# GloryyrolG/MHEntropy

Measured on AMD Instinct MI355X. Metric: hypotheses/sec (BxK) fwd+loss, 256x256, higher is better.
Workload: dtype bf16; 1 GPU; c2: MHEnt.get_loss forward+loss, resnet50 encoder (train-mode BN), 12-coupling RealNVP h=512, MANO joints, B=256/GPU, K=64, 256x256; images_per_gpu=256, hypotheses_per_image=64, global_batch=256, launch=hip-graph replay, base_noise=drawn on the device inside the step (Philox4x32-10, mhe_randn_f32), timing=one window of 452 steps, bracketed by barrier + synchronize, ranks=1, rccl_ranks=0

## Files before the change

include/mhe.h:

```cpp
#ifndef MHE_H
#define MHE_H

#include <stddef.h>
#include <stdint.h>

#ifdef __cplusplus
extern "C" {
#endif

#define MHE_OK 0
#define MHE_ERR_ARG 1
#define MHE_ERR_LAUNCH 2

enum { MHE_ACT_NONE = 0, MHE_ACT_RELU = 1 };
enum { MHE_F32 = 0, MHE_BF16 = 1 };
enum { MHE_FLOW_FORWARD = 0, MHE_FLOW_INVERSE = 1 };
enum { MHE_MODS_UV = 1, MHE_MODS_XYZ = 2 };

#define MHE_ABI_VERSION 4
int         mhe_abi_version(void);

typedef long long mhe_stat_t;
size_t mhe_stat_words(int C);
const char *mhe_last_error(void);
// ... 69 lines not shown
                        float image_size, int mm_mode, void *stream);

int mhe_mano_regress_joints_f32(const float *verts, const float *tables, float *joints, int R, void *stream);

int mhe_elbo_reduce_f32(const float *log_p_rows, const float *log_q_rows,
                        float *q_log_p, float *h, float *log_p, int N, int B, void *stream);

typedef struct mhe_conv_desc {
    int B, H, W, Cin, Cout, KH, KW, stride, pad;
    int dtype;
    int relu_in;
    int relu_out;
    int tile;
    int res_half;
} mhe_conv_desc;

int mhe_conv1x1_stats_nhwc(const mhe_conv_desc *d, const void *x, const void *w, const float *in_scale, const float *in_shift,
                           mhe_stat_t *stats, void *stream);
size_t mhe_gram_stats_words(int Cb);
size_t mhe_gram_stats_workspace_bytes(int Cb);
int mhe_conv1x1_gram_nhwc(const void *x, const float *in_scale, const float *in_shift, int relu_in, mhe_stat_t *gram, long pixels, int Cb,
                          void *stream);
int mhe_conv1x1_gram_store_nhwc(const void *x, const float *in_scale, const float *in_shift, int relu_in, mhe_stat_t *gram, void *a_out,
                                long pixels, int Cb, void *stream);
int mhe_gram_bn_finalize(mhe_stat_t *gram, void *workspace, const void *w, const float *gamma, const float *beta, float *running_mean,
                         float *running_var, float *scale, float *shift, float *mean_invstd, int C, int Cb, double count,
                         float momentum, float eps, long long *num_batches_tracked, void *stream);
int mhe_bottleneck_tail_supported(const mhe_conv_desc *d, int Cb);
int mhe_bottleneck_tail_nhwc(const mhe_conv_desc *d, int Cb, const void *y2, const float *bn2_scale, const float *bn2_shift,
                             const void *w3, const float *bn3_scale, const float *bn3_shift, const void *identity,
                             const float *id_scale, const float *id_shift, const void *w1, void *a_out, void *y1, mhe_stat_t *stats,
                             void *stream);

int mhe_conv2d_nhwc(const mhe_conv_desc *d, const void *x, const void *w, void *y,
                    const float *in_scale, const float *in_shift,
                    const float *out_scale, const float *out_shift, const void *residual,
                    mhe_stat_t *stats, void *stream);
int mhe_conv2d_f32out_nhwc(const mhe_conv_desc *d, const void *x, const void *w, float *y_f32, const float *out_shift, void *stream);
int mhe_conv2d_masked_nhwc(const mhe_conv_desc *d, const void *x, const void *w, void *y, const void *residual,
                           const void *mask, const void *bn_y0, const float *bn_mean_invstd0, mhe_stat_t *bn_stats0,
                           const void *bn_y1, const float *bn_mean_invstd1, mhe_stat_t *bn_stats1, void *stream);
int mhe_conv_stat_shards(void);
int mhe_conv1x1_residual_in_masked_nhwc(const mhe_conv_desc *d, const void *x, const void *x2, const void *w, void *y,
                                        const float *in_scale, const float *in_shift, const float *x2_scale, const float *x2_shift,
                                        void *a_out, const void *residual, const void *mask, const void *bn_y0,
                                        const float *bn_mean_invstd0, mhe_stat_t *bn_stats0, void *stream);

int mhe_conv3x3s2_dgrad_nhwc(int B, int Ho, int Wo, int Cout, int Cin, int dtype, const void *gy, const void *const *w4,
                             void *dx, const void *residual, const void *mask, const void *bn_y0,
                             const float *bn_mean_invstd0, mhe_stat_t *bn_stats0, const void *bn_y1,
                             const float *bn_mean_invstd1, mhe_stat_t *bn_stats1, int tile , void *stream);
int mhe_conv_tile(const mhe_conv_desc *d);
int mhe_conv_tile_mode(const mhe_conv_desc *d, int mode);

int mhe_conv1x1_residual_in_nhwc(const mhe_conv_desc *d, const void *x, const void *x2, const void *w, void *y,
                                 const float *in_scale, const float *in_shift, const float *x2_scale,
                                 const float *x2_shift, void *a_out, mhe_stat_t *stats, void *stream);

int mhe_stem_conv7x7s2(const float *x_nchw, const void *w, void *y, mhe_stat_t *stats, int B, int H, int W, int dtype,
                       void *stream);

int mhe_stem_pool_supported(int B, int H, int W, int dtype);
int mhe_stem_conv7x7s2_pool(const float *x_nchw, const void *w, const float *bn_gamma, void *pooled, mhe_stat_t *stats, int B, int H, int W,
                            void *stream);

int mhe_bn_finalize(const mhe_stat_t *stats, const float *gamma, const float *beta,
                    float *running_mean, float *running_var, float *scale, float *shift, float *mean_invstd,
                    int C, double count, float momentum, float eps, void *stream);
int mhe_bn_finalize_step(mhe_stat_t *stats, const float *gamma, const float *beta,
                         float *running_mean, float *running_var, float *scale, float *shift, float *mean_invstd,
                         int C, double count, float momentum, float eps, int clear_stats, long long *num_batches_tracked, void *stream);

int mhe_bn_act_nhwc(const void *x, const float *scale, const float *shift,
                    const void *res, const float *res_scale, const float *res_shift,
                    void *y, long P, int C, int relu, int dtype, void *stream);

int mhe_maxpool3x3s2_nhwc(const void *x, const float *scale, const float *shift, void *y,
                          int B, int H, int W, int C, int dtype, void *stream);

int mhe_avgpool_nhwc(const void *x, float *y, int B, int HW, int C, int dtype, void *stream);
int mhe_bn_act_avgpool_nhwc(const void *x, const float *scale, const float *shift, const void *res, const float *rscale,
                            const float *rshift, float *y, int B, int HW, int C, int relu, int dtype, void *stream);

int mhe_nchw_to_nhwc(const float *x, void *y, int B, int C, int H, int W, int dtype, void *stream);
int mhe_nchw_to_nhwc_pad(const float *x_nchw, void *y, int B, int C, int Cp, int H, int W, int dtype, void *stream);

int mhe_metrics_f32(const float *xyz, const float *uv, const float *pose3d, const float *scale,
                    const float *crop_uv, const float *vis, float *out, int N, int B, void *stream);

int mhe_metrics_split_f32(const float *xyz_err, const float *xyz_spread, const float *uv, const float *pose3d, const float *scale,
                          const float *crop_uv, const float *vis, float *out, int N, int B, void *stream);

size_t mhe_procrustes_workspace_floats(int B, int P);
int mhe_procrustes_align_f32(const float *pred, const float *target, float *out, float *R, float *s, float *ws, size_t ws_floats,
                             int N, int B, int P, void *stream);

int mhe_topk_gather_f32(const float *score, const float *rows, int *idx_out, float *rows_out,
                        int N, int B, int Q, int D, void *stream);

int mhe_mano_joints_bwd_f32(const float *th45, const float *det, const float *crop_uv, const float *vis,
                            const float *tables, const float *g_log_p, float *g_th45, float *g_det_rows,
                            int R, int B, float laplace_b, float th45_alpha, float row_weight, void *stream);
int mhe_mano_joints_mods_bwd_f32(const float *th45, const float *det, const float *crop_uv, const float *vis, const float *pose3d,
                                 const float *tables, const float *g_log_p, float *g_th45, float *g_det_rows,
                                 int R, int B, int mods, float laplace_b, float laplace_b_3d, float th45_alpha, float row_weight,
                                 void *stream);
int mhe_sum_over_hypotheses_f32(const float *rows, float *out, int N, int B, int C, int accumulate, long out_stride,
                                void *stream);

int mhe_conv_wgrad_nhwc(const mhe_conv_desc *d, const void *x, const void *gy, float *dw, int ldw, void *stream);
size_t mhe_conv_wgrad_workspace_floats(const mhe_conv_desc *d);
int mhe_conv_wgrad_ws_nhwc(const mhe_conv_desc *d, const void *x, const void *gy, float *dw, int ldw, float *workspace,
                           size_t workspace_floats, void *stream);
size_t mhe_conv_wgrad_batched_workspace_floats(const mhe_conv_desc *d, int nbatch);
int mhe_conv_wgrad_batched_nhwc(const mhe_conv_desc *d, int nbatch, const void *x, long x_batch_stride, const void *gy, long gy_batch_stride,
                                float *dw, long dw_batch_stride, int ldw, float *workspace, size_t workspace_floats, void *stream);
typedef struct mhe_wgrad_item {
    mhe_conv_desc d;
    const void *x, *gy;
    float *dw;
    int ldw;
} mhe_wgrad_item;
size_t mhe_conv_wgrad_multi_workspace_floats(const mhe_wgrad_item *items, int n);
int mhe_conv_wgrad_multi_nhwc(const mhe_wgrad_item *items, int n, float *workspace, size_t workspace_floats, void *stream);
int mhe_conv_wgrad_variant(const mhe_conv_desc *d, int Ho, int Wo, int nbatch);
size_t mhe_conv_wgrad_rect_workspace_floats(const mhe_conv_desc *d, int Ho, int Wo);
int mhe_conv_wgrad_rect_nhwc(const mhe_conv_desc *d, int stride_w, int pad_w, int Ho, int Wo, const void *x, const void *gy, float *dw,
                             int ldw, float *workspace, size_t workspace_floats, void *stream);
int mhe_colsum_f32(const void *rows, float *out, long R, int C, int dtype, void *stream);
size_t mhe_colsum_workspace_floats(long R, int C);
int mhe_colsum_ws_f32(const void *rows, float *out, long R, int C, int dtype, int out_group_width, long out_group_stride,
                      float *workspace, size_t workspace_floats, void *stream);
int mhe_gather_f32(const float *src, const int *idx, const int *idx2, void *dst, size_t n, int dst_dtype, void *stream);
int mhe_gather_affine8_bf16(const float *src, const int *base_stride, const unsigned char *mask, void *dst, size_t n, void *stream);

int mhe_flow_mask_pad_f32(const float *x, const float *mask, float *xp, long R, int dim, void *stream);
int mhe_flow_cond_lrelu_f32(float *P, const float *cond, long cond_stride, long R, int B, int H, void *stream);
int mhe_flow_lrelu_bwd_f32(float *G, const float *Hact, long n, float slope, void *stream);
int mhe_add_f32(const float *a, const float *b, float *out, long n, void *stream);
int mhe_flow_cond_lrelu_mixed(const void *pre, int pre_dtype, const float *cond, long cond_stride, float *out_f32,
                              void *out_bf16, long R, int B, int H, void *stream);
int mhe_flow_lrelu_bwd_mixed(const void *g, int g_dtype, const void *h, int h_dtype, float *out_f32, void *out_bf16,
                             long n, float slope, void *stream);
int mhe_flow_lrelu_bwd_sum(const void *g, int g_dtype, const void *h, int h_dtype, float *out_f32, void *out_bf16,
                           float *sum_out, long sum_stride, float *sum_out_t, int N, int B, int H, float slope, void *stream);
int mhe_flow_mask_pad_mixed(const float *x, const float *mask, float *xp, void *xp_bf16, long R, int dim, void *stream);
int mhe_conv2d_masked_bits_nhwc(const mhe_conv_desc *d, const void *x, const void *w, void *y, const void *residual,
                                const void *mask, const void *mask_bits, const void *bn_y0, const float *bn_mean_invstd0, mhe_stat_t *bn_stats0,
                                const void *bn_y1, const float *bn_mean_invstd1, mhe_stat_t *bn_stats1, void *stream);
int mhe_bottleneck_tail_bits_nhwc(const mhe_conv_desc *d, int Cb, const void *y2, const float *bn2_scale, const float *bn2_shift,
                                  const void *w3, const float *bn3_scale, const float *bn3_shift, const void *identity,
                                  const float *id_scale, const float *id_shift, const void *w1, void *a_out, void *a_bits, void *y1,
                                  mhe_stat_t *stats, void *stream);
int mhe_conv2d_masked_bias_nhwc(const mhe_conv_desc *d, const void *x, const void *xcat, int cin2, const void *w, void *y,
                                const void *residual, const void *mask, const float *bias, const void *bn_y0,
                                const float *bn_mean_invstd0, mhe_stat_t *bn_stats0, void *stream);
int mhe_conv1x1_cat_bias_nhwc(const mhe_conv_desc *d, const void *x, const void *xcat, int cin2, const void *w, void *y, const void *residual,
                              const float *bias, void *stream);
int mhe_conv3_bn_fold(float *D, const void *w_bf16, const double *gram_totals, const mhe_stat_t *rev_stats, const float *gamma,
                      const float *mean_invstd, double count, float *dgamma, float *dbeta, float *dW, void *w_dg_bf16, int ld_dg,
                      void *S_bf16, int ld_S, float *c0, float *coef_ws, int C, int Cb, void *stream);
int mhe_conv3x3_halo_supported(int B, int H, int W, int Cin, int Cout);
int mhe_conv3x3_halo_pack_bf16(const void *w, void *w_halo, int Cout, int Cin, void *stream);
int mhe_conv3x3_halo_nhwc(int B, int H, int W, int Cin, int Cout, const void *x, const void *w_halo, void *y, const float *in_scale,
                          const float *in_shift, int relu_in, void *a_out, mhe_stat_t *stats, const void *residual, const void *mask,
                          const void *bn_y0, const float *bn_mean_invstd0, mhe_stat_t *bn_stats0, void *stream);
int mhe_conv3x3_halo_dgrad_bn_nhwc(int B, int H, int W, int Cin, int Cout, const void *g, const void *y_raw, const float *coef, const void *w_halo,
                                   void *gx, void *gy_out, const void *residual, const void *mask, const void *bn_y0,
                                   const float *bn_mean_invstd0, mhe_stat_t *bn_stats0, void *stream);
int mhe_flow_reverse_chain_supported(int R, int B, int dim, int hidden, int ncoup);
int mhe_flow_couplings_frag_supported(int R, int B, int dim, int hidden, int ncoup);
int mhe_flow_couplings_frag_bf16(const float *in, float *out, const float *cond, int cond_stride, const void *w0F, const void *w1F,
                                 const void *w2F, long w_net_stride, const float *bias2, const float *mask, float *sum_s,
                                 float *log_prob, void *h1, void *h2, float *o, void *sign_bits, int R, int B, int dim, int hidden,
                                 int ncoup, int direction, void *stream);
int mhe_flow_reverse_chain_bf16(const float *x_out, const float *g_x, const float *g_logp, float q_weight, const float *mask,
                                const float *o_pre, const void *sign_bits, const void *w2F, const void *w1F,
                                const void *w0F, long w_net_stride, void *GO_bf16, void *G2_bf16, void *G1_bf16, void *XP_bf16,
                                float *Gc, int cond_stride, float *db2_rows, float *z0, int R, int B, int dim,
                                int hidden, int ncoup, void *stream);
int mhe_pack_transpose_bf16(const float *src, long src_stride, void *dst_bf16, void *dstT_bf16, int R, int C, void *stream);
int mhe_flow_couple_bwd_mixed(const float *x_out, const float *Os, const float *Ot, const float *mask,
                              const float *g_out, const float *g_log_p, float q_weight, float *x_in, float *GOs,
                              float *GOt, float *g_part, void *GOs_bf16, void *GOt_bf16,
                              float *db_s, float *db_t ,
                              long R, int B, int dim, void *stream);
int mhe_flow_couple_bwd_f32(const float *x_out, const float *Os, const float *Ot, const float *mask,
                            const float *g_out, const float *g_log_p, float q_weight, float *x_in, float *GOs,
                            float *GOt, float *g_part, long R, int B, int dim, void *stream);
int mhe_flow_couple_accum_f32(const float *g_part, const float *GXs, const float *GXt, const float *mask,
                              float *g_in, long R, int dim, void *stream);

int mhe_rot6d_to_rotmat_f32(const float *poses6, float *rotmats, long n, int robust, void *stream);
int mhe_rot6d_to_rotmat_bwd_f32(const float *poses6, const float *g_rotmats, float *g_poses6, long n, void *stream);
size_t mhe_lbs_workspace_floats(int R, int J, int nb);
int mhe_lbs_pose_f32(const float *rotmats, const float *betas, const float *j_template, const float *j_shapedirs,
                     const int *parents, float *workspace, float *joints, int R, int J, int nb, void *stream);
int mhe_lbs_skin_f32(const float *workspace, const float *v_template, const float *v_shapedirs, const float *v_posedirs,
                     const float *v_weights, float *verts, int R, int J, int nb, int NV, int VP, float scale, void *stream);
size_t mhe_lbs_split_floats(int J, int nb, int VP);
int mhe_lbs_split_tables_f32(const float *v_template, const float *v_shapedirs, const float *v_posedirs, const float *v_weights,
                             float *split, int J, int nb, int VP, void *stream);
int mhe_lbs_skin_mfma_supported(int R, int J, int nb, int NV, int VP);
int mhe_lbs_skin_mfma_f32(const float *workspace, const float *split, float *verts, int R, int J, int nb, int NV, int VP, float scale,
                          void *stream);

int mhe_bn_mean_invstd(const mhe_stat_t *stats, float *mean_invstd, int C, double count, float eps, void *stream);
int mhe_bn_bwd_reduce_nhwc(const void *g, const void *a, const void *y, const float *mean_invstd, mhe_stat_t *stats,
                           long P, int C, int dtype, void *stream);
int mhe_bn_bwd_finalize(const mhe_stat_t *stats, const float *gamma, const float *mean_invstd, float *dgamma,
                        float *dbeta, float *coef, int C, double count, void *stream);
int mhe_bn_bwd_apply_nhwc(const void *g, const void *a, const void *y, const float *coef, void *gy, void *g_masked,
                          long P, int C, int dtype, void *stream);
int mhe_maxpool3x3s2_idx_nhwc(const void *x, void *y, unsigned char *idx, int B, int H, int W, int C, int dtype, void *stream);
int mhe_maxpool3x3s2_bwd_nhwc(const void *gy, const unsigned char *idx, void *gx, int B, int H, int W, int C, int dtype, void *stream);
int mhe_maxpool3x3s2_idx_affine_nhwc(const void *x, const float *scale, const float *shift, void *y, unsigned char *idx, int B, int H, int W,
                                     int C, int dtype, void *stream);
int mhe_maxpool3x3s2_idx_affine_win_nhwc(const void *x, const float *scale, const float *shift, void *y, unsigned char *idx, void *xwin, int B,
                                         int H, int W, int C, int dtype, void *stream);
int mhe_pooled_bn_sums_nhwc(const void *g, const void *pooled, const void *xwin, const float *mean_invstd, mhe_stat_t *stats, long P, int C,
                            int dtype, void *stream);
int mhe_maxpool3x3s2_bwd_bn_nhwc(const void *gy, const unsigned char *idx, const void *y, const float *scale, const float *shift,
                                 const float *mean_invstd, mhe_stat_t *stats, void *gx, int B, int H, int W, int C, int dtype, void *stream);
int mhe_maxpool3x3s2_bwd_bn_apply_nhwc(const void *gy, const unsigned char *idx, const void *y, const float *scale, const float *shift,
                                       const float *mean_invstd, const float *coef, void *gy_out, int B, int H, int W, int C, int dtype,
                                       void *stream);
int mhe_avgpool_bwd_nhwc(const float *g, const void *mask, void *gx, int B, int HW, int C, int dtype, void *stream);
int mhe_upsample2_nhwc(const void *g, const void *base, void *out, int B, int H, int W, int C, int dtype, void *stream);
size_t mhe_sqnorm_workspace_floats(void);
int mhe_sqnorm_f32(const float *g, size_t n, float *workspace, float *out, void *stream);
int mhe_train_tick(int *step, float *sqnorm, void *stream);
int mhe_adam_step_f32(float *p, const float *g, float *m, float *v, size_t n, const float *sqnorm, const int *step,
                      float lr, float beta1, float beta2, float eps, float max_norm, float grad_scale, void *stream);

int mhe_glow_add_image_rows_f32(float *H, const float *img, long img_stride, long R, int C, int row_div, int n_img, void *stream);
int mhe_relu_copy_f32(const float *in, void *out, long n, int out_dtype, void *stream);
int mhe_glow_glu_residual_f32(float *H, const void *T, int t_dtype, const float *gate, long gate_stride, long R, int C,
                              int row_div, int n_img, void *stream);
int mhe_glow_coupling_f32(const float *u, const float *params, float *y, float *logdet, long R, int dim, int first,
                          int n_transform, int inverse, void *stream);
int mhe_pad64_f32(const float *x, float *xp, long R, int dim, void *stream);
int mhe_glow_coupling_inv_bwd_f32(const float *v, const float *params, const float *g_y, const float *g_log_p, float q_weight,
                                  float *g_v, float *g_params, long R, int B, int dim, int first, int n_transform, void *stream);
int mhe_glow_glu_bwd_f32(const float *g_h, const void *t3, const float *gate, long gate_stride, void *g_t3, float *g_gate_rows,
                         long R, int C, int row_div, int n_img, int t_dtype, void *stream);
int mhe_relu_bwd_add_f32(float *acc, const void *g, const float *h, long n, int g_dtype, void *stream);
int mhe_glow_finish_f32(const float *z_padded, const float *v_padded, const float *logdet, float *v_out, float *log_prob,
                        long R, int dim, float sign, float logdet_const, void *stream);
int mhe_glow_finish_dev_f32(const float *z_padded, const float *v_padded, const float *logdet, float *v_out, float *log_prob,
                            long R, int dim, float sign, const float *const_parts, int n_parts, void *stream);
int mhe_glow_glu_bwd_sum(const float *g_h, const void *t3, const float *gate, long gate_stride, void *g_t3, float *gct, long gct_stride,
                         float *bsum, long bsum_stride, int N, int B, int C, void *stream);
int mhe_glow_mask_scale_sum(void *g, const void *t2, float scale, float *bsum, long bsum_stride, int N, int B, int C, void *stream);
int mhe_relu_bwd_add_mixed(float *acc, const void *g, const void *h, long n, int g_dtype, int h_dtype, void *stream);
int mhe_dropout_bits(unsigned char *bits, long n, float p_drop, unsigned long long *state, void *stream);
int mhe_glow_layers_supported(int N, int B, int dim, int hidden, int layers, int blocks);
int mhe_glow_layers_bf16(const float *noise, const float *ctab, int ctab_stride, const void *wxF, const void *w0F, const void *w1F, const void *wsF,
                         const void *wuF, const float *b0, const float *b1, const float *bs, const float *bu, const float *ainvT,
                         const float *cinv, const float *const_parts, const unsigned char *drop_bits, float p_drop, float *out, float *log_q,
                         float *v_e, float *y_e, float *prm_e, void *tb_e, void *t2_e, void *t3_e, void *hf_e, float *prmc_e, void *vb_e,
                         void *bits_e, int N, int B, int dim, int hidden, int layers, int blocks, long row_n, long row_b, void *stream);
int mhe_glow_reverse_chain_supported(int R, int B, int dim, int hidden, int layers, int blocks);
int mhe_glow_reverse_chain_bf16(const float *g_x, const float *g_log_p, float q_weight, const float *v_e, const float *prmc_e, const void *t3_e,
                                const void *bits_e, const float *ctab, int ctab_stride, const void *wsT, const void *wuT, const void *w1T,
                                const void *w0T, const void *wxT, const float *ainv, float p_drop, float *gv_e, void *gpc_e, void *gt3_e,
                                void *gt2_e, void *gh0_e, float *gct, float *bsum, float *bfsum, int R, int B, int dim, int hidden, int layers,
                                int blocks, void *stream);
size_t mhe_glow_affine_workspace_doubles(int layers, int features);
int mhe_glow_affine_f64(const void *param_ptrs, int layers, int features, float eps, float *A, float *c, float *Ainv, float *AinvT,
                        float *cinv, float *const_parts, double *workspace, void *stream);
int mhe_glow_reparam_bwd_f64(const void *g_ainv_ptrs, const void *g_cinv_ptrs, const float *g_log_p, int n_log_p, float q_sign, int layers,
                             int features, const double *workspace, const void *grad_ptrs, void *stream);

size_t mhe_glow_affine_wide_workspace_doubles(int layers, int features);
size_t mhe_glow_affine_wide_grad_doubles(int layers, int features);
int mhe_glow_affine_wide_f64(const void *param_ptrs, int layers, int features, double eps, float *A, float *c, float *Ainv, float *AinvT,
                             float *cinv, float *const_parts, double *workspace, void *stream);
int mhe_glow_affine_wide_bwd_f64(const float *g_ainv, const float *g_cinv, const float *g_log_q, long n_log_q, int layers, int features,
                                 double *workspace, double *grads, void *stream);
int mhe_glow_coupling_inv_bwd_wide_f32(const float *v, const float *params, const float *g_y, const float *g_log_q, float *g_v,
                                       float *g_params, long R, int dim, int first, int n_transform, int ld, int ldp, void *stream);
int mhe_sum_row_blocks_f32(const float *rows, float *out, int groups, int N, int C, long out_stride, int accumulate, void *stream);
int mhe_lbs_pose_bwd_f32(const float *rotmats, const float *betas, const float *j_template, const float *j_shapedirs, const int *parents,
                         const float *g_joints, float *g_rotmats, float *g_betas, int R, int J, int nb, void *stream);
size_t mhe_lbs_bwd_tables_floats(int J, int nb, int VP);
int mhe_lbs_bwd_tables_f32(const float *v_shapedirs, const float *v_posedirs, const float *v_weights, float *tables, int J, int nb, int NV, int VP,
                           void *stream);
int mhe_lbs_skin_bwd_f32(const float *workspace, const float *v_template, const float *v_shapedirs, const float *v_posedirs, const float *v_weights,
                         const float *tables, const float *g_verts, float *g_transforms, float *g_posemap, float *g_betas, int R, int J, int nb, int NV,
                         int VP, float scale, void *stream);
int mhe_lbs_transforms_bwd_f32(const float *rotmats, const float *betas, const float *j_template, const float *j_shapedirs, const int *parents,
                               const float *g_joints, const float *g_transforms, const float *g_posemap, const float *g_betas_in, float *g_rotmats,
                               float *g_betas, int R, int J, int nb, void *stream);

#ifdef __cplusplus
}
#endif
#endif
```

mhentropy_amd/_lib.py:

```python
import ctypes as C
import os

_HERE = os.path.dirname(os.path.abspath(__file__))
LIB_PATH = os.path.join(_HERE, "csrc", "libmhe_hip.so")

_p, _i, _f, _sz, _l, _d = C.c_void_p, C.c_int, C.c_float, C.c_size_t, C.c_long, C.c_double


class ConvDesc(C.Structure):
    _fields_ = [(n, C.c_int) for n in
                ("B", "H", "W", "Cin", "Cout", "KH", "KW", "stride", "pad", "dtype", "relu_in", "relu_out", "tile", "res_half")]


class WgradItem(C.Structure):
    _fields_ = [("d", ConvDesc), ("x", C.c_void_p), ("gy", C.c_void_p), ("dw", C.c_void_p), ("ldw", C.c_int)]


SIGNATURES = {
    "mhe_abi_version": (_i, []),
    "mhe_last_error": (C.c_char_p, []),
    "mhe_linear_f32": (_i, [_p, _p, _p, _p, _i, _i, _i, _i, _p]),
    "mhe_linear_skinny_f32": (_i, [_p, _p, _p, _p, _i, _i, _i, _i, _p]),
    "mhe_linear_f32_bf16copy": (_i, [_p, _p, _p, _p, _p, _i, _i, _i, _i, _p]),
    "mhe_randn_f32": (_i, [_p, _l, _p, _f, _p]),
    "mhe_dropout": (_i, [_p, _i, _p, _l, _f, _p, _i, _p]),
    "mhe_reparam_f32": (_i, [_p, _p, _p, _p, _p, _l, _i, _i, _p]),
    "mhe_flow_packed_floats_per_net": (_sz, [_i, _i]),
    "mhe_flow_pack_net_host": (_i, [_p, _p, _p, _i, _i, _p]),
    "mhe_flow_couplings_f32": (_i, [_p, _p, _p, _p, _p, _p, _p, _p, _i, _i, _i, _i, _i, _i, _p]),
    "mhe_flow_packed_bytes_per_net_bf16": (_sz, [_i, _i]),
    "mhe_flow_pack_net_bf16_host": (_i, [_p, _p, _p, _i, _i, _p]),
    "mhe_flow_couplings_bf16": (_i, [_p, _p, _p, _p, _p, _p, _p, _p, _i, _i, _i, _i, _i, _i, _p]),
    "mhe_flow_couplings_bf16_emit": (_i, [_p, _p, _p, _p, _p, _p, _p, _p, _p, _p, _p, _i, _i, _i, _i, _i, _i, _p]),
    "mhe_mano_table_floats": (_sz, []),
    "mhe_mano_joints_f32": (_i, [_p] * 12 + [_i, _i, _f, _f, _i, _f, _p]),
    "mhe_mano_joints_mods_f32": (_i, [_p] * 13 + [_i, _i, _i, _f, _f, _f, _i, _f, _p]),
    "mhe_mano_verts_workspace_floats": (_sz, [_i]),
    "mhe_mano_verts_f32": (_i, [_p, _p, _p, _p, _i, _i, _p]),
    "mhe_mano_decode_f32": (_i, [_p] * 14 + [_i, _i, _f, _f, _i, _f, _i, _p]),
    "mhe_mano_joints_bwd_f32": (_i, [_p] * 8 + [_i, _i, _f, _f, _f, _p]),
    "mhe_mano_joints_mods_bwd_f32": (_i, [_p] * 9 + [_i, _i, _i, _f, _f, _f, _f, _p]),
    "mhe_sum_over_hypotheses_f32": (_i, [_p, _p, _i, _i, _i, _i, _l, _p]),
    "mhe_conv_wgrad_nhwc": (_i, [C.POINTER(ConvDesc), _p, _p, _p, _i, _p]),
    "mhe_conv_wgrad_workspace_floats": (_sz, [C.POINTER(ConvDesc)]),
    "mhe_conv_wgrad_variant": (_i, [_p, _i, _i, _i]),
    "mhe_conv_wgrad_ws_nhwc": (_i, [C.POINTER(ConvDesc), _p, _p, _p, _i, _p, _sz, _p]),
    "mhe_conv_wgrad_rect_workspace_floats": (_sz, [C.POINTER(ConvDesc), _i, _i]),
    "mhe_conv_wgrad_rect_nhwc": (_i, [C.POINTER(ConvDesc), _i, _i, _i, _i, _p, _p, _p, _i, _p, _sz, _p]),
    "mhe_colsum_f32": (_i, [_p, _p, _l, _i, _i, _p]),
    "mhe_colsum_workspace_floats": (_sz, [_l, _i]),
    "mhe_colsum_ws_f32": (_i, [_p, _p, _l, _i, _i, _i, _l, _p, _sz, _p]),
    "mhe_gather_f32": (_i, [_p, _p, _p, _p, _sz, _i, _p]),
    "mhe_gather_affine8_bf16": (_i, [_p, _p, _p, _p, _sz, _p]),
    "mhe_flow_mask_pad_f32": (_i, [_p, _p, _p, _l, _i, _p]),
    "mhe_flow_cond_lrelu_f32": (_i, [_p, _p, _l, _l, _i, _i, _p]),
    "mhe_flow_lrelu_bwd_f32": (_i, [_p, _p, _l, _f, _p]),
    "mhe_add_f32": (_i, [_p, _p, _p, _l, _p]),
    "mhe_flow_cond_lrelu_mixed": (_i, [_p, _i, _p, _l, _p, _p, _l, _i, _i, _p]),
    "mhe_flow_lrelu_bwd_mixed": (_i, [_p, _i, _p, _i, _p, _p, _l, _f, _p]),
    "mhe_flow_couple_bwd_f32": (_i, [_p] * 6 + [_f] + [_p] * 4 + [_l, _i, _i, _p]),
    "mhe_flow_lrelu_bwd_sum": (_i, [_p, _i, _p, _i, _p, _p, _p, _l, _p, _i, _i, _i, _f, _p]),
    "mhe_flow_mask_pad_mixed": (_i, [_p, _p, _p, _p, _l, _i, _p]),
    "mhe_flow_couple_bwd_mixed": (_i, [_p] * 6 + [_f] + [_p] * 8 + [_l, _i, _i, _p]),
    "mhe_flow_couple_accum_f32": (_i, [_p] * 5 + [_l, _i, _p]),
    "mhe_bn_mean_invstd": (_i, [_p, _p, _i, _d, _f, _p]),
    "mhe_bn_bwd_reduce_nhwc": (_i, [_p] * 5 + [_l, _i, _i, _p]),
    "mhe_bn_bwd_finalize": (_i, [_p] * 6 + [_i, _d, _p]),
    "mhe_bn_bwd_apply_nhwc": (_i, [_p] * 6 + [_l, _i, _i, _p]),
    "mhe_maxpool3x3s2_idx_nhwc": (_i, [_p, _p, _p, _i, _i, _i, _i, _i, _p]),
    "mhe_maxpool3x3s2_bwd_nhwc": (_i, [_p, _p, _p, _i, _i, _i, _i, _i, _p]),
    "mhe_maxpool3x3s2_idx_affine_nhwc": (_i, [_p] * 5 + [_i] * 5 + [_p]),
    "mhe_maxpool3x3s2_idx_affine_win_nhwc": (_i, [_p] * 6 + [_i] * 5 + [_p]),
    "mhe_pooled_bn_sums_nhwc": (_i, [_p] * 5 + [_l, _i, _i, _p]),
    "mhe_maxpool3x3s2_bwd_bn_nhwc": (_i, [_p] * 8 + [_i] * 5 + [_p]),
    "mhe_maxpool3x3s2_bwd_bn_apply_nhwc": (_i, [_p] * 8 + [_i] * 5 + [_p]),
    "mhe_avgpool_bwd_nhwc": (_i, [_p, _p, _p, _i, _i, _i, _i, _p]),
    "mhe_upsample2_nhwc": (_i, [_p, _p, _p, _i, _i, _i, _i, _i, _p]),
    "mhe_sqnorm_workspace_floats": (_sz, []),
    "mhe_sqnorm_f32": (_i, [_p, _sz, _p, _p, _p]),
    "mhe_train_tick": (_i, [_p, _p, _p]),
    "mhe_adam_step_f32": (_i, [_p] * 4 + [_sz, _p, _p] + [_f] * 6 + [_p]),
    "mhe_glow_add_image_rows_f32": (_i, [_p, _p, _l, _l, _i, _i, _i, _p]),
    "mhe_relu_copy_f32": (_i, [_p, _p, _l, _i, _p]),
    "mhe_glow_glu_residual_f32": (_i, [_p, _p, _i, _p, _l, _l, _i, _i, _i, _p]),
    "mhe_glow_coupling_f32": (_i, [_p, _p, _p, _p, _l, _i, _i, _i, _i, _p]),
    "mhe_pad64_f32": (_i, [_p, _p, _l, _i, _p]),
    "mhe_glow_coupling_inv_bwd_f32": (_i, [_p, _p, _p, _p, _f, _p, _p, _l, _i, _i, _i, _i, _p]),
    "mhe_glow_glu_bwd_f32": (_i, [_p, _p, _p, _l, _p, _p, _l, _i, _i, _i, _i, _p]),
    "mhe_relu_bwd_add_f32": (_i, [_p, _p, _p, _l, _i, _p]),
    "mhe_glow_finish_f32": (_i, [_p, _p, _p, _p, _p, _l, _i, _f, _f, _p]),
    "mhe_conv_wgrad_multi_workspace_floats": (_sz, [_p, _i]),
    "mhe_conv_wgrad_multi_nhwc": (_i, [_p, _i, _p, _sz, _p]),
    "mhe_glow_glu_bwd_sum": (_i, [_p, _p, _p, _l, _p, _p, _l, _p, _l, _i, _i, _i, _p]),
    "mhe_glow_mask_scale_sum": (_i, [_p, _p, _f, _p, _l, _i, _i, _i, _p]),
    "mhe_relu_bwd_add_mixed": (_i, [_p, _p, _p, _l, _i, _i, _p]),
    "mhe_dropout_bits": (_i, [_p, _l, _f, _p, _p]),
    "mhe_glow_layers_supported": (_i, [_i] * 6),
    "mhe_glow_layers_bf16": (_i, [_p, _p, _i] + [_p] * 13 + [_f] + [_p] * 12 + [_i] * 6 + [_l, _l, _p]),
    "mhe_glow_reverse_chain_supported": (_i, [_i] * 6),
    "mhe_glow_reverse_chain_bf16": (_i, [_p, _p, _f, _p, _p, _p, _p, _p, _i] + [_p] * 6 + [_f] + [_p] * 8 + [_i] * 6 + [_p]),
    "mhe_glow_finish_dev_f32": (_i, [_p, _p, _p, _p, _p, _l, _i, _f, _p, _i, _p]),
    "mhe_glow_affine_workspace_doubles": (_sz, [_i, _i]),
    "mhe_glow_affine_f64": (_i, [_p, _i, _i, _f] + [_p] * 7 + [_p]),
    "mhe_glow_reparam_bwd_f64": (_i, [_p, _p, _p, _i, _f, _i, _i, _p, _p, _p]),
    "mhe_glow_affine_wide_workspace_doubles": (_sz, [_i, _i]),
    "mhe_glow_affine_wide_grad_doubles": (_sz, [_i, _i]),
    "mhe_glow_affine_wide_f64": (_i, [_p, _i, _i, _d] + [_p] * 7 + [_p]),
    "mhe_glow_affine_wide_bwd_f64": (_i, [_p, _p, _p, _l, _i, _i, _p, _p, _p]),
    "mhe_glow_coupling_inv_bwd_wide_f32": (_i, [_p] * 6 + [_l, _i, _i, _i, _i, _i, _p]),
    "mhe_sum_row_blocks_f32": (_i, [_p, _p, _i, _i, _i, _l, _i, _p]),
    "mhe_mano_regress_joints_f32": (_i, [_p, _p, _p, _i, _p]),
    "mhe_elbo_reduce_f32": (_i, [_p, _p, _p, _p, _p, _i, _i, _p]),
    "mhe_conv2d_nhwc": (_i, [C.POINTER(ConvDesc), _p, _p, _p, _p, _p, _p, _p, _p, _p, _p]),
    "mhe_conv2d_masked_nhwc": (_i, [_p] * 13),
    "mhe_conv2d_f32out_nhwc": (_i, [C.POINTER(ConvDesc), _p, _p, _p, _p, _p]),
    "mhe_conv_stat_shards": (_i, []),
    "mhe_conv1x1_residual_in_masked_nhwc": (_i, [C.POINTER(ConvDesc)] + [_p] * 15),
    "mhe_conv3x3s2_dgrad_nhwc": (_i, [_i, _i, _i, _i, _i, _i, _p, C.POINTER(C.c_void_p), _p, _p, _p, _p, _p, _p, _p, _p, _p, _i, _p]),
    "mhe_ho3d_geom_doubles": (_i, []),
    "mhe_ho3d_targets": (_i, [_p] * 7 + [_i] + [_p] * 18 + [_i, _p]),
    "mhe_ho3d_images": (_i, [_p] * 9 + [_i, _p]),
    "mhe_conv_tile": (_i, [C.POINTER(ConvDesc)]),
    "mhe_conv_tile_mode": (_i, [C.POINTER(ConvDesc), _i]),
    "mhe_conv1x1_residual_in_nhwc": (_i, [C.POINTER(ConvDesc)] + [_p] * 11),
    "mhe_stem_conv7x7s2": (_i, [_p, _p, _p, _p, _i, _i, _i, _i, _p]),
    "mhe_conv1x1_stats_nhwc": (_i, [_p, _p, _p, _p, _p, _p, _p]),
    "mhe_conv_wgrad_batched_workspace_floats": (_sz, [_p, _i]),
    "mhe_conv_wgrad_batched_nhwc": (_i, [_p, _i, _p, _l, _p, _l, _p, _l, _i, _p, _sz, _p]),
    "mhe_conv2d_masked_bits_nhwc": (_i, [_p] * 14),
    "mhe_bottleneck_tail_bits_nhwc": (_i, [_p, _i] + [_p] * 15),
    "mhe_conv2d_masked_bias_nhwc": (_i, [_p, _p, _p, _i] + [_p] * 9),
    "mhe_conv3x3_halo_supported": (_i, [_i] * 5),
    "mhe_conv3x3_halo_pack_bf16": (_i, [_p, _p, _i, _i, _p]),
    "mhe_conv3x3_halo_dgrad_bn_nhwc": (_i, [_i] * 5 + [_p] * 12),
    "mhe_conv3x3_halo_nhwc": (_i, [_i] * 5 + [_p] * 5 + [_i] + [_p] * 8),
    "mhe_conv1x1_cat_bias_nhwc": (_i, [_p, _p, _p, _i, _p, _p, _p, _p, _p]),
    "mhe_conv3_bn_fold": (_i, [_p] * 6 + [_d] + [_p] * 4 + [_i, _p, _i] + [_p] * 2 + [_i, _i, _p]),
    "mhe_flow_reverse_chain_supported": (_i, [_i, _i, _i, _i, _i]),
    "mhe_flow_couplings_frag_supported": (_i, [_i, _i, _i, _i, _i]),
    "mhe_flow_couplings_frag_bf16": (_i, [_p, _p, _p, _i, _p, _p, _p, _l, _p, _p, _p, _p, _p, _p, _p, _p, _i, _i, _i, _i, _i, _i, _p]),
    "mhe_flow_reverse_chain_bf16": (_i, [_p, _p, _p, _f, _p, _p, _p, _p, _p, _p, _l, _p, _p, _p, _p, _p, _i, _p, _p, _i, _i, _i, _i, _i, _p]),
    "mhe_pack_transpose_bf16": (_i, [_p, _l, _p, _p, _i, _i, _p]),
    "mhe_gram_stats_words": (_sz, [_i]),
    "mhe_stat_words": (_sz, [_i]),
    "mhe_gram_stats_workspace_bytes": (_sz, [_i]),
    "mhe_conv1x1_gram_nhwc": (_i, [_p, _p, _p, _i, _p, _l, _i, _p]),
    "mhe_conv1x1_gram_store_nhwc": (_i, [_p, _p, _p, _i, _p, _p, _l, _i, _p]),
    "mhe_gram_bn_finalize": (_i, [_p] * 10 + [_i, _i, _d, _f, _f, _p, _p]),
    "mhe_bottleneck_tail_supported": (_i, [_p, _i]),
    "mhe_bottleneck_tail_nhwc": (_i, [_p, _i] + [_p] * 14),
    "mhe_stem_pool_supported": (_i, [_i, _i, _i, _i]),
    "mhe_stem_conv7x7s2_pool": (_i, [_p, _p, _p, _p, _p, _i, _i, _i, _p]),
    "mhe_bn_finalize": (_i, [_p] * 8 + [_i, _d, _f, _f, _p]),
    "mhe_bn_finalize_step": (_i, [_p] * 8 + [_i, _d, _f, _f, _i, _p, _p]),
    "mhe_bn_act_nhwc": (_i, [_p] * 7 + [_l, _i, _i, _i, _p]),
    "mhe_maxpool3x3s2_nhwc": (_i, [_p, _p, _p, _p, _i, _i, _i, _i, _i, _p]),
    "mhe_avgpool_nhwc": (_i, [_p, _p, _i, _i, _i, _i, _p]),
    "mhe_bn_act_avgpool_nhwc": (_i, [_p] * 7 + [_i, _i, _i, _i, _i, _p]),
    "mhe_nchw_to_nhwc": (_i, [_p, _p, _i, _i, _i, _i, _i, _p]),
    "mhe_nchw_to_nhwc_pad": (_i, [_p, _p, _i, _i, _i, _i, _i, _i, _p]),
    "mhe_rot6d_to_rotmat_f32": (_i, [_p, _p, _l, _i, _p]),
    "mhe_rot6d_to_rotmat_bwd_f32": (_i, [_p, _p, _p, _l, _p]),
    "mhe_lbs_workspace_floats": (_sz, [_i, _i, _i]),
    "mhe_lbs_pose_f32": (_i, [_p] * 7 + [_i, _i, _i, _p]),
    "mhe_lbs_pose_bwd_f32": (_i, [_p] * 8 + [_i, _i, _i, _p]),
    "mhe_lbs_skin_f32": (_i, [_p] * 6 + [_i, _i, _i, _i, _i, _f, _p]),
    "mhe_lbs_split_floats": (_sz, [_i, _i, _i]),
    "mhe_lbs_split_tables_f32": (_i, [_p, _p, _p, _p, _p, _i, _i, _i, _p]),
    "mhe_lbs_skin_mfma_supported": (_i, [_i, _i, _i, _i, _i]),
    "mhe_lbs_skin_mfma_f32": (_i, [_p, _p, _p, _i, _i, _i, _i, _i, _f, _p]),
    "mhe_lbs_bwd_tables_floats": (_sz, [_i, _i, _i]),
    "mhe_lbs_bwd_tables_f32": (_i, [_p] * 4 + [_i, _i, _i, _i, _p]),
    "mhe_lbs_skin_bwd_f32": (_i, [_p] * 10 + [_i, _i, _i, _i, _i, _f, _p]),
    "mhe_lbs_transforms_bwd_f32": (_i, [_p] * 11 + [_i, _i, _i, _p]),
    "mhe_topk_gather_f32": (_i, [_p, _p, _p, _p, _i, _i, _i, _i, _p]),
    "mhe_metrics_f32": (_i, [_p] * 7 + [_i, _i, _p]),
    "mhe_metrics_split_f32": (_i, [_p] * 8 + [_i, _i, _p]),
    "mhe_procrustes_workspace_floats": (_sz, [_i, _i]),
    "mhe_procrustes_align_f32": (_i, [_p] * 6 + [_sz, _i, _i, _i, _p]),
}

_lib = None
ABI_VERSION = 4


class MheError(RuntimeError):
    pass


def lib():
    global _lib
    if _lib is None:
        if not os.path.exists(LIB_PATH):
            raise MheError(
                f"{LIB_PATH} is missing: build it with `python -m mhentropy_amd.build` "
                "(hipcc --offload-arch=gfx950). There is no CPU fallback.")
        import torch
        L = C.CDLL(LIB_PATH)
        for name, (res, args) in SIGNATURES.items():
            fn = getattr(L, name)
            fn.restype, fn.argtypes = res, args
        if L.mhe_abi_version() != ABI_VERSION:
            raise MheError(f"{LIB_PATH} has ABI version {L.mhe_abi_version()}, these bindings are for {ABI_VERSION}: rebuild "
                           "(`python -m mhentropy_amd.build`)")
        _lib = L
    return _lib


def check(status, what):
    if status != 0:
        raise MheError(f"{what} failed ({status}): {lib().mhe_last_error().decode()}")
```

mhentropy_amd/csrc/conv.hip:

```cpp
#include "conv_shared.h"
#include <cstdlib>

namespace mhe { namespace conv {

template <typename T, int BM, int BN, int WM, int WN, bool FAST, int MODE, bool DG = false>
__global__ __launch_bounds__(64 * WM * WN, WM * WN == 4 ? 2 : 1) void conv_kernel(const Params p) {
    constexpr int NTH = 64 * WM * WN;
    constexpr int CE = El<T>::CE, BKE = 8 * CE;
    constexpr int RSTEP = NTH / 8;
    constexpr int NJ_A = BM / RSTEP, NJ_B = BN / RSTEP;
    constexpr int MTW = BM / WM / 16, NTW = BN / WN / 16;
    __shared__ uint4 lds[2][(BM + BN) * 8];
    constexpr bool AFFM = MODE == 1 || MODE == 2;
    __shared__ __attribute__((aligned(16))) float aff[2][AFFM ? MAXC : 4];

    const int tid = threadIdx.x, wave = tid >> 6, lane = tid & 63;
    const int q = lane >> 4, l15 = lane & 15;
    const int wr = wave / WN, wc = wave % WN;
    int mtile, ntile;
    tile_of_block(mtile, ntile);
    const int m0 = mtile * BM, n0 = ntile * BN;
    const int s = tid & 7, rbase = tid >> 3;
    const T *xg = reinterpret_cast<const T *>(p.x);
    const T *wg = reinterpret_cast<const T *>(p.w);
// ... 386 lines not shown
    const int b = blockIdx.y, l = threadIdx.x & 63, g = threadIdx.x >> 6, c = blockIdx.x * 256 + l * 4;
    float a[4] = {0.f, 0.f, 0.f, 0.f};
    if (c < C) {
        const float4 s = *reinterpret_cast<const float4 *>(scale + c), t = *reinterpret_cast<const float4 *>(shift + c);
        float4 rs = make_float4(1.f, 1.f, 1.f, 1.f), rt = make_float4(0.f, 0.f, 0.f, 0.f);
        if (rscale) { rs = *reinterpret_cast<const float4 *>(rscale + c); rt = *reinterpret_cast<const float4 *>(rshift + c); }
        for (int p = g; p < HW; p += 4) {
            const size_t e = ((size_t)b * HW + p) * C + c;
            float v[4], r[4];
            load4<T>(x + e, v);
            v[0] = fmaf(v[0], s.x, t.x); v[1] = fmaf(v[1], s.y, t.y); v[2] = fmaf(v[2], s.z, t.z); v[3] = fmaf(v[3], s.w, t.w);
            if (res) {
                load4<T>(res + e, r);
                if (rscale) { r[0] = fmaf(r[0], rs.x, rt.x); r[1] = fmaf(r[1], rs.y, rt.y); r[2] = fmaf(r[2], rs.z, rt.z); r[3] = fmaf(r[3], rs.w, rt.w); }
#pragma unroll
                for (int k = 0; k < 4; ++k) v[k] += r[k];
            }
#pragma unroll
            for (int k = 0; k < 4; ++k) {
                if (relu) v[k] = fmaxf(v[k], 0.f);
                if constexpr (sizeof(T) == 2) v[k] = bf16_to_f32(f32_to_bf16(v[k]));
                a[k] += v[k];
            }
        }
    }
#pragma unroll
    for (int k = 0; k < 4; ++k) part[g][l * 4 + k] = a[k];
    __syncthreads();
    const int cc = blockIdx.x * 256 + threadIdx.x;
    if (cc < C) y[(size_t)b * C + cc] = (part[0][threadIdx.x] + part[1][threadIdx.x] + part[2][threadIdx.x] + part[3][threadIdx.x]) / (float)HW;
}

template <typename T>
__global__ void nchw_to_nhwc_kernel(const float *__restrict__ x, T *__restrict__ y, int B, int C, int HW, int Cp) {
    const size_t n = (size_t)B * HW;
    for (size_t i = (size_t)blockIdx.x * blockDim.x + threadIdx.x; i < n; i += (size_t)gridDim.x * blockDim.x) {
        const size_t b = i / HW, p = i % HW;
        for (int c = 0; c < Cp; ++c) {
            const float v = c < C ? x[(b * C + c) * HW + p] : 0.f;
            if constexpr (sizeof(T) == 4) y[i * Cp + c] = v;
            else y[i * Cp + c] = f32_to_bf16(v);
        }
    }
}

__global__ void nchw3_to_nhwc4_bf16_kernel(const float *__restrict__ x, uint2 *__restrict__ y, int B, int HW) {
    const size_t n = (size_t)B * HW;
    for (size_t i = (size_t)blockIdx.x * blockDim.x + threadIdx.x; i < n; i += (size_t)gridDim.x * blockDim.x) {
        const size_t b = i / HW, p = i % HW;
        const float *src = x + b * 3 * HW + p;
        const float c0 = src[0], c1 = src[HW], c2 = src[2 * (size_t)HW];
        y[i] = make_uint2((unsigned)f32_to_bf16(c0) | ((unsigned)f32_to_bf16(c1) << 16), (unsigned)f32_to_bf16(c2));
    }
}

template <typename T, int BM, int BN, int WM, int WN, bool FAST>
static void launch_mode(const Params &p, hipStream_t s) {
    const dim3 grid((p.M + BM - 1) / BM, (p.Cout + BN - 1) / BN), block(64 * WM * WN);
    if (p.x2) {
        if constexpr (FAST) {
            if constexpr (BM == 128) { if (p.mask) { hipLaunchKernelGGL((conv_kernel<T, BM, BN, WM, WN, true, 2, true>), grid, block, 0, s, p); return; } }
            hipLaunchKernelGGL((conv_kernel<T, BM, BN, WM, WN, true, 2>), grid, block, 0, s, p);
        }
    } else if (p.in_scale) {
        hipLaunchKernelGGL((conv_kernel<T, BM, BN, WM, WN, FAST, 1>), grid, block, 0, s, p);
    } else if (p.xcat) {
        if constexpr (FAST && BM == 128 && sizeof(T) == 2) {
            if (p.mask) hipLaunchKernelGGL((conv_kernel<T, BM, BN, WM, WN, true, 3, true>), grid, block, 0, s, p);
            else hipLaunchKernelGGL((conv_kernel<T, BM, BN, WM, WN, true, 3>), grid, block, 0, s, p);
        }
    } else if (p.mask) {
        hipLaunchKernelGGL((conv_kernel<T, BM, BN, WM, WN, FAST, 0, true>), grid, block, 0, s, p);
    } else {
        hipLaunchKernelGGL((conv_kernel<T, BM, BN, WM, WN, FAST, 0>), grid, block, 0, s, p);
    }
}

bool p8_supports(const Params &p);
int launch_p8(const Params &p, hipStream_t s);
int launch_p8h(const Params &p, hipStream_t s);
bool stream_supports(const Params &p);
int launch_stream(const Params &p, hipStream_t s);
bool stream3_supports(const Params &p);
int launch_stream3(const Params &p, hipStream_t s);
bool wide_supports(const Params &p);
int launch_wide(const Params &p, hipStream_t s);
bool fuse_supports(const Params &p, int cb);
int launch_fuse(const Params &p, int cb, hipStream_t s);
bool tail_supports(const Params &p);
int launch_tail(const Params &p, hipStream_t s);

static int choose_tile(const Params &p, bool fast, bool bf16) {
    static const int env_force = getenv("MHE_CONV_TILE") ? atoi(getenv("MHE_CONV_TILE")) : -1;
    const int force = p.force >= 0 ? p.force : env_force;
    if ((p.mask && p.out_shift) || p.xcat) return force == 0 || (force < 0 && p.Cout <= 64) ? 0 : 1;
    static const int env_stream = getenv("MHE_CONV_STREAM") ? atoi(getenv("MHE_CONV_STREAM")) : 1;
    if (bf16 && (force == 8 || (force < 0 && env_stream && !(p.mask && p.Cin == 256))) && stream_supports(p)) return 8;
    if (bf16 && (force == 9 || (force < 0 && env_stream)) && stream3_supports(p)) return 9;
    static const int env_wide = getenv("MHE_CONV_WIDE") ? atoi(getenv("MHE_CONV_WIDE")) : 1;
    if (bf16 && (force == 11 || (force < 0 && env_wide && p.Cin == 256)) && wide_supports(p)) return 11;
    static const int env_tail = getenv("MHE_CONV_TAIL") ? atoi(getenv("MHE_CONV_TAIL")) : 1;
    if (bf16 && (force == 10 || (force < 0 && env_tail)) && tail_supports(p)) return 10;
    if ((force & 15) == 7 && bf16 && p8_supports(p)) return 7;
    if (force == 13 && bf16 && p8_supports(p)) return 13;
    if (p.x2 && p.mask) return force == 0 ? 0 : 1;
    if (force >= 0 && force <= 4 && (force < 2 || (fast && bf16))) return force;
    if (p.Cout <= 64) return 0;
    if (fast && bf16 && p.Cout >= 256) {
        const long tiles = (long)((p.M + 255) / 256) * ((p.Cout + 255) / 256);
        if (p.x2) return 1;
        if (tiles >= 192) return p8_supports(p) && force < 0 ? 7 : 2;
    }
    static const int env_p8h = getenv("MHE_CONV_P8H") ? atoi(getenv("MHE_CONV_P8H")) : 1;
    if (fast && bf16 && env_p8h && force < 0 && !p.x2 && p.KH * p.KW > 1 && p.KH * p.KW * p.Cin >= 2304 && p.Cout % 128 == 0 && p8_supports(p) &&
        (long)((p.M + 255) / 256) * (p.Cout / 128) >= 192)
        return 13;
    return 1;
}

template <typename T>
static int launch_conv(const Params &p, hipStream_t s) {
    constexpr int BKE = 8 * El<T>::CE;
    const bool fast = (p.Cin % BKE) == 0;
    if constexpr (sizeof(T) == 2) {
        const int t0 = choose_tile(p, fast, true);
        if (t0 == 8) return launch_stream(p, s);
        if (t0 == 9) return launch_stream3(p, s);
        if (t0 == 10) return launch_tail(p, s);
        if (t0 == 11) return launch_wide(p, s);
        if (t0 == 7) return launch_p8(p, s);
        if (t0 == 13) return launch_p8h(p, s);
    }
    if (p.x2 && !fast) { set_error("residual-tail prologue needs Cin %% %d == 0", BKE); return MHE_ERR_ARG; }
    switch (choose_tile(p, fast, sizeof(T) == 2)) {
        case 0: if (fast) launch_mode<T, 128, 64, 2, 2, true>(p, s); else launch_mode<T, 128, 64, 2, 2, false>(p, s); break;
        case 2: if constexpr (sizeof(T) == 2) launch_mode<T, 256, 256, 2, 4, true>(p, s); break;
        case 3: if constexpr (sizeof(T) == 2) launch_mode<T, 256, 128, 4, 2, true>(p, s); break;
        case 4: if constexpr (sizeof(T) == 2) launch_mode<T, 256, 64, 4, 2, true>(p, s); break;
        default: if (fast) launch_mode<T, 128, 128, 2, 2, true>(p, s); else launch_mode<T, 128, 128, 2, 2, false>(p, s); break;
    }
    return check_launch("conv_kernel");
}

}}

using namespace mhe;

static inline int elem_chunk(int dtype) { return dtype == MHE_F32 ? 4 : 8; }

static int conv_entry(const mhe_conv_desc *d, const void *x, const void *w, void *y, const float *in_scale,
                      const float *in_shift, const float *out_scale, const float *out_shift, const void *residual,
                      mhe_stat_t *stats, const void *x2, const float *x2_scale, const float *x2_shift, void *a_out, void *stream,
                      const void *mask = nullptr, const struct BnRev *bn = nullptr, float *y32 = nullptr, const int *scatter = nullptr,
                      const void *xcat = nullptr, int cin2 = 0, const void *mask_bits = nullptr);
struct BnRev { const void *y[2]; const float *mi[2]; mhe_stat_t *stats[2]; };

extern "C" int mhe_conv2d_nhwc(const mhe_conv_desc *d, const void *x, const void *w, void *y, const float *in_scale,
                               const float *in_shift, const float *out_scale, const float *out_shift,
                               const void *residual, mhe_stat_t *stats, void *stream) {
    return conv_entry(d, x, w, y, in_scale, in_shift, out_scale, out_shift, residual, stats, nullptr, nullptr, nullptr,
                      nullptr, stream);
}

extern "C" int mhe_conv2d_f32out_nhwc(const mhe_conv_desc *d, const void *x, const void *w, float *y_f32, const float *out_shift, void *stream) {
    MHE_REQUIRE(y_f32, "mhe_conv2d_f32out_nhwc: null output");
    return conv_entry(d, x, w, nullptr, nullptr, nullptr, nullptr, out_shift, nullptr, nullptr, nullptr, nullptr, nullptr, nullptr, stream, nullptr,
                      nullptr, y_f32);
}

extern "C" int mhe_conv1x1_residual_in_nhwc(const mhe_conv_desc *d, const void *x, const void *x2, const void *w, void *y,
                                            const float *in_scale, const float *in_shift, const float *x2_scale,
                                            const float *x2_shift, void *a_out, mhe_stat_t *stats, void *stream) {
    MHE_REQUIRE(d && x2 && in_scale && in_shift, "mhe_conv1x1_residual_in_nhwc: x2, in_scale and in_shift are required");
    MHE_REQUIRE(d->KH == 1 && d->KW == 1 && d->stride == 1 && d->pad == 0, "mhe_conv1x1_residual_in_nhwc: 1x1 stride-1 only");
    MHE_REQUIRE((x2_scale == nullptr) == (x2_shift == nullptr), "mhe_conv1x1_residual_in_nhwc: x2_scale/x2_shift must come together");
    return conv_entry(d, x, w, y, in_scale, in_shift, nullptr, nullptr, nullptr, stats, x2, x2_scale, x2_shift, a_out, stream);
}

extern "C" int mhe_conv1x1_cat_bias_nhwc(const mhe_conv_desc *d, const void *x, const void *xcat, int cin2, const void *w, void *y, const void *residual,
                                         const float *bias, void *stream) {
    MHE_REQUIRE(d && xcat && d->dtype == MHE_BF16 && d->KH == 1 && d->KW == 1 && d->stride == 1 && d->pad == 0 && cin2 > 0 && cin2 % 64 == 0 && d->Cin % 64 == 0,
                "mhe_conv1x1_cat_bias_nhwc: a bf16 1x1 stride-1 launch on two operand tensors with Cin and cin2 multiples of 64");
    MHE_REQUIRE(d->tile == 0 || d->tile == 1 || d->tile == 2, "mhe_conv1x1_cat_bias_nhwc: 128-row register-staged tiles only (tile 0, 1 or 2)");
    return conv_entry(d, x, w, y, nullptr, nullptr, nullptr, bias, residual, nullptr, nullptr, nullptr, nullptr, nullptr, stream, nullptr, nullptr, nullptr,
                      nullptr, xcat, cin2);
}

extern "C" int mhe_conv1x1_residual_in_masked_nhwc(const mhe_conv_desc *d, const void *x, const void *x2, const void *w, void *y,
                                                   const float *in_scale, const float *in_shift, const float *x2_scale,
                                                   const float *x2_shift, void *a_out, const void *residual, const void *mask,
                                                   const void *bn_y0, const float *bn_mean_invstd0, mhe_stat_t *bn_stats0, void *stream) {
    MHE_REQUIRE(d && x2 && in_scale && in_shift && mask, "mhe_conv1x1_residual_in_masked_nhwc: x2, in_scale, in_shift and mask are required");
    MHE_REQUIRE(d->KH == 1 && d->KW == 1 && d->stride == 1 && d->pad == 0, "mhe_conv1x1_residual_in_masked_nhwc: 1x1 stride-1 only");
    MHE_REQUIRE((x2_scale == nullptr) == (x2_shift == nullptr), "mhe_conv1x1_residual_in_masked_nhwc: x2_scale/x2_shift must come together");
    MHE_REQUIRE(!bn_y0 || (bn_mean_invstd0 && bn_stats0), "mhe_conv1x1_residual_in_masked_nhwc: bn_y needs its mean_invstd and stats");
    MHE_REQUIRE(d->tile == 0 || d->tile == 1 || d->tile == 2 || d->tile == 11,
                "mhe_conv1x1_residual_in_masked_nhwc: 128-row tiles only (tile 0, 1, 2, or 11 = the transfer-wave kernel)");
    const BnRev bn = {{bn_y0, nullptr}, {bn_mean_invstd0, nullptr}, {bn_stats0, nullptr}};
    return conv_entry(d, x, w, y, in_scale, in_shift, nullptr, nullptr, residual, nullptr, x2, x2_scale, x2_shift, a_out, stream, mask, &bn);
}

extern "C" int mhe_conv2d_masked_nhwc(const mhe_conv_desc *d, const void *x, const void *w, void *y, const void *residual,
                                      const void *mask, const void *bn_y0, const float *bn_mean_invstd0, mhe_stat_t *bn_stats0,
                                      const void *bn_y1, const float *bn_mean_invstd1, mhe_stat_t *bn_stats1, void *stream) {
    MHE_REQUIRE(mask, "mhe_conv2d_masked_nhwc: mask is required");
    MHE_REQUIRE((!bn_y0 || (bn_mean_invstd0 && bn_stats0)) && (!bn_y1 || (bn_y0 && bn_mean_invstd1 && bn_stats1)),
                "mhe_conv2d_masked_nhwc: each bn_y needs its mean_invstd and stats (and bn_y1 needs bn_y0)");
    const BnRev bn = {{bn_y0, bn_y1}, {bn_mean_invstd0, bn_mean_invstd1}, {bn_stats0, bn_stats1}};
    return conv_entry(d, x, w, y, nullptr, nullptr, nullptr, nullptr, residual, nullptr, nullptr, nullptr, nullptr, nullptr, stream, mask, &bn);
}

extern "C" int mhe_conv2d_masked_bits_nhwc(const mhe_conv_desc *d, const void *x, const void *w, void *y, const void *residual,
                                           const void *mask, const void *mask_bits, const void *bn_y0, const float *bn_mean_invstd0, mhe_stat_t *bn_stats0,
                                           const void *bn_y1, const float *bn_mean_invstd1, mhe_stat_t *bn_stats1, void *stream) {
    MHE_REQUIRE(mask, "mhe_conv2d_masked_bits_nhwc: mask is required (kernels without the bit path read it)");
    MHE_REQUIRE((!bn_y0 || (bn_mean_invstd0 && bn_stats0)) && (!bn_y1 || (bn_y0 && bn_mean_invstd1 && bn_stats1)),
                "mhe_conv2d_masked_bits_nhwc: each bn_y needs its mean_invstd and stats (and bn_y1 needs bn_y0)");
    MHE_REQUIRE(!mask_bits || (d && d->Cout % 8 == 0), "mhe_conv2d_masked_bits_nhwc: Cout must be a multiple of 8");
    const BnRev bn = {{bn_y0, bn_y1}, {bn_mean_invstd0, bn_mean_invstd1}, {bn_stats0, bn_stats1}};
    return conv_entry(d, x, w, y, nullptr, nullptr, nullptr, nullptr, residual, nullptr, nullptr, nullptr, nullptr, nullptr, stream, mask, &bn, nullptr,
                      nullptr, nullptr, 0, mask_bits);
}

extern "C" int mhe_conv2d_masked_bias_nhwc(const mhe_conv_desc *d, const void *x, const void *xcat, int cin2, const void *w, void *y,
                                           const void *residual, const void *mask, const float *bias, const void *bn_y0,
                                           const float *bn_mean_invstd0, mhe_stat_t *bn_stats0, void *stream) {
    MHE_REQUIRE(mask && bias, "mhe_conv2d_masked_bias_nhwc: mask and bias are required");
    MHE_REQUIRE(!xcat || (d && d->dtype == MHE_BF16 && d->KH == 1 && d->KW == 1 && d->stride == 1 && d->pad == 0 && cin2 > 0 && cin2 % 64 == 0 && d->Cin % 64 == 0),
                "mhe_conv2d_masked_bias_nhwc: a concatenated operand needs a bf16 1x1 stride-1 launch with Cin and cin2 multiples of 64");
    MHE_REQUIRE(!bn_y0 || (bn_mean_invstd0 && bn_stats0), "mhe_conv2d_masked_bias_nhwc: bn_y needs its mean_invstd and stats");
    MHE_REQUIRE(d && (d->tile == 0 || d->tile == 1 || d->tile == 2), "mhe_conv2d_masked_bias_nhwc: 128-row register-staged tiles only (tile 0, 1 or 2)");
    const BnRev bn = {{bn_y0, nullptr}, {bn_mean_invstd0, nullptr}, {bn_stats0, nullptr}};
    return conv_entry(d, x, w, y, nullptr, nullptr, nullptr, bias, residual, nullptr, nullptr, nullptr, nullptr, nullptr, stream, mask, &bn, nullptr,
                      nullptr, xcat, xcat ? cin2 : 0);
}

extern "C" int mhe_conv3x3s2_dgrad_nhwc(int B, int Ho, int Wo, int Cout, int Cin, int dtype, const void *gy, const void *const *w4,
                                        void *dx, const void *residual, const void *mask, const void *bn_y0,
                                        const float *bn_mean_invstd0, mhe_stat_t *bn_stats0, const void *bn_y1,
                                        const float *bn_mean_invstd1, mhe_stat_t *bn_stats1, int tile, void *stream) {
    MHE_REQUIRE(gy && w4 && dx && w4[0] && w4[1] && w4[2] && w4[3], "mhe_conv3x3s2_dgrad_nhwc: null pointer");
    MHE_REQUIRE((!bn_y0 || (bn_mean_invstd0 && bn_stats0 && mask)) && (!bn_y1 || (bn_y0 && bn_mean_invstd1 && bn_stats1)),
                "mhe_conv3x3s2_dgrad_nhwc: each bn_y needs its mean_invstd and stats (and the gate)");
    const BnRev bn = {{bn_y0, bn_y1}, {bn_mean_invstd0, bn_mean_invstd1}, {bn_stats0, bn_stats1}};
    for (int py = 0; py < 2; ++py)
        for (int px = 0; px < 2; ++px) {
            mhe_conv_desc d = {B, Ho, Wo, Cout, Cin, 1 + py, 1 + px, 1, 0, dtype, 0, 0, tile};
            const int sc[2] = {py, px};
            const int rc = conv_entry(&d, gy, w4[2 * py + px], dx, nullptr, nullptr, nullptr, nullptr, residual, nullptr, nullptr, nullptr,
                                      nullptr, nullptr, stream, mask, mask ? &bn : nullptr, nullptr, sc);
            if (rc) return rc;
        }
    return MHE_OK;
}

static int conv_entry(const mhe_conv_desc *d, const void *x, const void *w, void *y, const float *in_scale,
                      const float *in_shift, const float *out_scale, const float *out_shift, const void *residual,
                      mhe_stat_t *stats, const void *x2, const float *x2_scale, const float *x2_shift, void *a_out, void *stream,
                      const void *mask, const BnRev *bn, float *y32, const int *scatter, const void *xcat, int cin2, const void *mask_bits) {
    MHE_REQUIRE(d && x && w && (y || y32), "mhe_conv2d_nhwc: null pointer");
    MHE_REQUIRE(d->dtype == MHE_F32 || d->dtype == MHE_BF16, "mhe_conv2d_nhwc: dtype=%d", d->dtype);
    const int ce = elem_chunk(d->dtype), bke = 8 * ce;
    MHE_REQUIRE(d->B > 0 && d->H > 0 && d->W > 0 && d->KH > 0 && d->KW > 0 && d->stride > 0 && d->pad >= 0,
                "mhe_conv2d_nhwc: bad geometry");
    MHE_REQUIRE(d->Cin % ce == 0, "mhe_conv2d_nhwc: Cin=%d must be a multiple of %d (pad channels)", d->Cin, ce);
    MHE_REQUIRE(d->Cout % ce == 0, "mhe_conv2d_nhwc: Cout=%d must be a multiple of %d", d->Cout, ce);
    MHE_REQUIRE((in_scale == nullptr) == (in_shift == nullptr), "mhe_conv2d_nhwc: in_scale/in_shift must come together");
    MHE_REQUIRE(!in_scale || d->Cin <= conv::MAXC, "mhe_conv2d_nhwc: fused input affine supports Cin <= %d", conv::MAXC);
    conv::Params p{};
    p.x = x; p.w = w; p.y = y; p.in_scale = in_scale; p.in_shift = in_shift; p.out_scale = out_scale;
    p.out_shift = out_shift; p.residual = residual; p.stats = stats; p.mask = mask;
    for (int u = 0; u < 2; ++u) { p.bn_y[u] = bn ? bn->y[u] : nullptr; p.bn_mi[u] = bn ? bn->mi[u] : nullptr; p.bn_stats[u] = bn ? bn->stats[u] : nullptr; }
    p.x2 = x2; p.x2_scale = x2_scale; p.x2_shift = x2_shift; p.a_out = a_out;
    p.B = d->B; p.H = d->H; p.W = d->W; p.Cin = d->Cin; p.Cout = d->Cout; p.KH = d->KH; p.KW = d->KW;
    p.stride = d->stride; p.pad = d->pad;
    p.Ho = (d->H + 2 * d->pad - d->KH) / d->stride + 1;
    p.Wo = (d->W + 2 * d->pad - d->KW) / d->stride + 1;
    p.os2 = 0; p.os_py = p.os_px = 0;
    p.res_s2 = d->res_half ? 1 : 0;
    MHE_REQUIRE(!p.res_s2 || (residual && !scatter && !y32), "mhe_conv2d_nhwc: res_half needs a residual (and no output scatter)");
    if (scatter) {
        p.Ho = d->H; p.Wo = d->W; p.os2 = 1; p.os_py = scatter[0]; p.os_px = scatter[1];
    }
    MHE_REQUIRE(p.Ho > 0 && p.Wo > 0, "mhe_conv2d_nhwc: empty output");
    const long long M = (long long)p.B * p.Ho * p.Wo;
    MHE_REQUIRE(M < (1ll << 31), "mhe_conv2d_nhwc: too many output pixels");
    p.M = (int)M;
    p.xcat = xcat; p.Cin2 = cin2; p.mask_bits = (const unsigned char *)mask_bits;
    const int ktot = d->KH * d->KW * d->Cin + cin2;
    p.Kpad = (ktot + bke - 1) / bke * bke;
    p.relu_in = d->relu_in; p.relu_out = d->relu_out;
    p.force = d->tile - 1;
    p.y32 = nullptr;
    if (y32) {
        MHE_REQUIRE(d->dtype == MHE_BF16 && !in_scale && !out_scale && !residual && !stats && !x2 && !mask && !d->relu_out && d->Cout % 4 == 0,
                    "mhe_conv2d_f32out_nhwc: bf16 operands, optional out_shift only");
        p.y32 = y32;
        if (p.force < 0 || p.force > 4) p.force = p.Cout <= 64 ? 0 : 1;
    }
    if (d->dtype == MHE_F32) return conv::launch_conv<float>(p, (hipStream_t)stream);
    return conv::launch_conv<u16>(p, (hipStream_t)stream);
}

extern "C" int mhe_conv1x1_stats_nhwc(const mhe_conv_desc *d, const void *x, const void *w, const float *in_scale, const float *in_shift,
                                      mhe_stat_t *stats, void *stream) {
    MHE_REQUIRE(d && x && w && stats, "mhe_conv1x1_stats_nhwc: null pointer");
    MHE_REQUIRE(d->dtype == MHE_BF16 && d->KH == 1 && d->KW == 1 && d->stride == 1 && d->pad == 0 && (d->Cin == 64 || d->Cin == 128 || d->Cin == 256) && d->Cout % 256 == 0,
                "mhe_conv1x1_stats_nhwc: bf16 1x1 stride-1 with 64 / 128 / 256 input channels and a multiple of 256 output channels");
    MHE_REQUIRE((in_scale == nullptr) == (in_shift == nullptr), "mhe_conv1x1_stats_nhwc: in_scale/in_shift must come together");
    conv::Params p{};
    p.x = x; p.w = w; p.y = nullptr; p.in_scale = in_scale; p.in_shift = in_shift; p.stats = stats;
    p.B = d->B; p.H = d->H; p.W = d->W; p.Cin = d->Cin; p.Cout = d->Cout; p.KH = 1; p.KW = 1; p.stride = 1; p.pad = 0; p.Ho = d->H; p.Wo = d->W;
    const long long M = (long long)d->B * d->H * d->W;
    MHE_REQUIRE(M > 0 && M < (1ll << 31), "mhe_conv1x1_stats_nhwc: bad pixel count");
    p.M = (int)M; p.Kpad = d->Cin; p.relu_in = d->relu_in; p.force = 8; p.stats_only = 1;
    if (d->Cin == 256) {
        p.force = 11;
        MHE_REQUIRE(conv::wide_supports(p), "mhe_conv1x1_stats_nhwc: geometry not taken by the resident-slab kernel (M=%lld Cout=%d)", M, d->Cout);
        return conv::launch_wide(p, (hipStream_t)stream);
    }
    MHE_REQUIRE(conv::stream_supports(p), "mhe_conv1x1_stats_nhwc: geometry not taken by the streaming kernel");
    return conv::launch_stream(p, (hipStream_t)stream);
}

extern "C" int mhe_bottleneck_tail_supported(const mhe_conv_desc *d, int Cb) {
    if (!d || d->dtype != MHE_BF16) return 0;
    static const float dummy = 0.f;
    conv::Params p{};
    p.x = p.x2 = p.w = p.w3 = p.y = p.a_out = (void *)&dummy; p.in_scale = p.in_shift = p.mid_scale = p.mid_shift = &dummy;
    p.Cin = d->Cin; p.Cout = d->Cout; p.KH = d->KH; p.KW = d->KW; p.stride = d->stride; p.pad = d->pad; p.Kpad = d->Cin;
    const long long M = (long long)d->B * d->H * d->W;
    if (M <= 0 || M >= (1ll << 31)) return 0;
    p.M = (int)M;
    return conv::fuse_supports(p, Cb) ? 1 : 0;
}

extern "C" int mhe_bottleneck_tail_nhwc(const mhe_conv_desc *d, int Cb, const void *y2, const float *bn2_scale, const float *bn2_shift,
                                        const void *w3, const float *bn3_scale, const float *bn3_shift, const void *identity,
                                        const float *id_scale, const float *id_shift, const void *w1, void *a_out, void *y1, mhe_stat_t *stats,
                                        void *stream) {
    return mhe_bottleneck_tail_bits_nhwc(d, Cb, y2, bn2_scale, bn2_shift, w3, bn3_scale, bn3_shift, identity, id_scale, id_shift, w1, a_out, nullptr, y1, stats, stream);
}

extern "C" int mhe_bottleneck_tail_bits_nhwc(const mhe_conv_desc *d, int Cb, const void *y2, const float *bn2_scale, const float *bn2_shift,
                                             const void *w3, const float *bn3_scale, const float *bn3_shift, const void *identity,
                                             const float *id_scale, const float *id_shift, const void *w1, void *a_out, void *a_bits, void *y1,
                                             mhe_stat_t *stats, void *stream) {
    MHE_REQUIRE(d && y2 && bn2_scale && bn2_shift && w3 && bn3_scale && bn3_shift && identity && w1 && a_out && y1, "mhe_bottleneck_tail_nhwc: null pointer");
    MHE_REQUIRE(d->dtype == MHE_BF16, "mhe_bottleneck_tail_nhwc: bf16 storage only");
    MHE_REQUIRE((id_scale == nullptr) == (id_shift == nullptr), "mhe_bottleneck_tail_nhwc: id_scale/id_shift must come together");
    conv::Params p{};
    p.x = y2; p.in_scale = bn2_scale; p.in_shift = bn2_shift; p.w3 = w3; p.mid_scale = bn3_scale; p.mid_shift = bn3_shift;
    p.x2 = identity; p.x2_scale = id_scale; p.x2_shift = id_shift; p.w = w1; p.a_out = a_out; p.y = y1; p.stats = stats;
    p.a_bits = (unsigned char *)a_bits;
    p.B = d->B; p.H = d->H; p.W = d->W; p.Cin = d->Cin; p.Cout = d->Cout; p.KH = d->KH; p.KW = d->KW; p.stride = d->stride; p.pad = d->pad;
    p.Ho = d->H; p.Wo = d->W; p.Kpad = d->Cin; p.relu_in = 1; p.force = -1;
    const long long M = (long long)d->B * d->H * d->W;
    MHE_REQUIRE(M > 0 && M < (1ll << 31), "mhe_bottleneck_tail_nhwc: bad pixel count");
    p.M = (int)M;
    MHE_REQUIRE(conv::fuse_supports(p, Cb), "mhe_bottleneck_tail_nhwc: needs Cin = 4 Cb, Cb 64 / 128, Cout 64 / 128, pixels %% 128 == 0 (Cin=%d Cb=%d Cout=%d M=%lld)",
                d->Cin, Cb, d->Cout, M);
    return conv::launch_fuse(p, Cb, (hipStream_t)stream);
}

extern "C" int mhe_conv_stat_shards(void) { return conv::NSH; }
extern "C" size_t mhe_stat_words(int C) { return C > 0 ? (size_t)2 * conv::NSH * 2 * (size_t)C : 0; }

extern "C" int mhe_conv_tile(const mhe_conv_desc *d) {
    if (!d) return -1;
    conv::Params p{};
    p.B = d->B; p.H = d->H; p.W = d->W; p.Cin = d->Cin; p.Cout = d->Cout; p.KH = d->KH; p.KW = d->KW; p.stride = d->stride; p.pad = d->pad;
    const int Ho = (d->H + 2 * d->pad - d->KH) / d->stride + 1, Wo = (d->W + 2 * d->pad - d->KW) / d->stride + 1;
    p.M = d->B * Ho * Wo;
    p.force = d->tile - 1;
    const int bke = d->dtype == MHE_F32 ? 32 : 64;
    p.Kpad = (d->KH * d->KW * d->Cin + bke - 1) / bke * bke;
    return conv::choose_tile(p, d->Cin % bke == 0, d->dtype == MHE_BF16);
}

extern "C" int mhe_conv_tile_mode(const mhe_conv_desc *d, int mode) {
    if (!d || mode < 0 || mode > 3) return -1;
    static const float dummy = 0.f;
    conv::Params p{};
    p.B = d->B; p.H = d->H; p.W = d->W; p.Cin = d->Cin; p.Cout = d->Cout; p.KH = d->KH; p.KW = d->KW; p.stride = d->stride; p.pad = d->pad;
    const int Ho = (d->H + 2 * d->pad - d->KH) / d->stride + 1, Wo = (d->W + 2 * d->pad - d->KW) / d->stride + 1;
    p.M = d->B * Ho * Wo;
    p.force = d->tile - 1;
    const int bke = d->dtype == MHE_F32 ? 32 : 64;
    p.Kpad = (d->KH * d->KW * d->Cin + bke - 1) / bke * bke;
    if (mode == 1 || mode == 2) p.in_scale = &dummy;
    if (mode == 2) p.x2 = &dummy;
    if (mode == 3) p.residual = &dummy;
    return conv::choose_tile(p, d->Cin % bke == 0, d->dtype == MHE_BF16);
}

extern "C" int mhe_stem_conv7x7s2(const float *x_nchw, const void *w, void *y, mhe_stat_t *stats, int B, int H, int W, int dtype,
                                  void *stream) {
    MHE_REQUIRE(x_nchw && w && y, "mhe_stem_conv7x7s2: null pointer");
    MHE_REQUIRE(B > 0 && H > 0 && W > 0, "mhe_stem_conv7x7s2: bad geometry");
    MHE_REQUIRE(dtype == MHE_F32 || dtype == MHE_BF16, "mhe_stem_conv7x7s2: dtype=%d", dtype);
    conv::Params p{};
    p.force = -1;
    p.w = w; p.y = y; p.stats = stats;
    p.B = B; p.H = H; p.W = W; p.Cin = 3; p.Cout = 64; p.KH = p.KW = 7; p.stride = 2; p.pad = 3;
    p.Ho = (H + 6 - 7) / 2 + 1; p.Wo = (W + 6 - 7) / 2 + 1;
    p.M = B * p.Ho * p.Wo;
    const int tx = (p.Wo + 15) / 16, ty = (p.Ho + 7) / 8;
    const dim3 grid((unsigned)(tx * ty * B));
    if (dtype == MHE_F32) hipLaunchKernelGGL(conv::stem_kernel<float>, grid, dim3(256), 0, (hipStream_t)stream, x_nchw, p, tx, ty);
    else hipLaunchKernelGGL(conv::stem_kernel<u16>, grid, dim3(256), 0, (hipStream_t)stream, x_nchw, p, tx, ty);
    return check_launch("stem_kernel");
}

extern "C" int mhe_linear_skinny_f32(const float *X, const float *W, const float *bias, float *Y, int M, int N, int K,
                                     int act, void *stream);

extern "C" int mhe_linear_f32(const float *X, const float *W, const float *bias, float *Y, int M, int N, int K, int act,
                              void *stream) {
    MHE_REQUIRE(X && W && Y && M > 0 && N > 0 && K > 0, "mhe_linear_f32: bad arguments");
    MHE_REQUIRE(K % 32 == 0, "mhe_linear_f32: K=%d must be a multiple of 32", K);
    MHE_REQUIRE(N % 4 == 0, "mhe_linear_f32: N=%d must be a multiple of 4", N);
    if (M <= 256 && K % 64 == 0) return mhe_linear_skinny_f32(X, W, bias, Y, M, N, K, act, stream);
    mhe_conv_desc d = {M, 1, 1, K, N, 1, 1, 1, 0, MHE_F32, 0, act == MHE_ACT_RELU};
    return mhe_conv2d_nhwc(&d, X, W, Y, nullptr, nullptr, nullptr, bias, nullptr, nullptr, stream);
}

extern "C" int mhe_bn_finalize(const mhe_stat_t *stats, const float *gamma, const float *beta, float *running_mean,
                               float *running_var, float *scale, float *shift, float *mean_invstd, int C, double count,
                               float momentum, float eps, void *stream) {
    MHE_REQUIRE(stats && gamma && beta && scale && shift && C > 0 && count > 1.f, "mhe_bn_finalize: bad arguments");
    hipLaunchKernelGGL(conv::bn_finalize_kernel, dim3((C + 3) / 4), dim3(256), 0, (hipStream_t)stream, const_cast<mhe_stat_t *>(stats), gamma,
                       beta, running_mean, running_var, scale, shift, mean_invstd, C, count, momentum, eps, 0, (long long *)nullptr);
    return check_launch("bn_finalize_kernel");
}

extern "C" int mhe_bn_finalize_step(mhe_stat_t *stats, const float *gamma, const float *beta, float *running_mean,
                                    float *running_var, float *scale, float *shift, float *mean_invstd, int C, double count,
                                    float momentum, float eps, int clear_stats, long long *num_batches_tracked, void *stream) {
    MHE_REQUIRE(stats && gamma && beta && scale && shift && C > 0 && count > 1.f, "mhe_bn_finalize_step: bad arguments");
    hipLaunchKernelGGL(conv::bn_finalize_kernel, dim3((C + 3) / 4), dim3(256), 0, (hipStream_t)stream, stats, gamma,
                       beta, running_mean, running_var, scale, shift, mean_invstd, C, count, momentum, eps, clear_stats,
                       num_batches_tracked);
    return check_launch("bn_finalize_kernel");
}

static inline int ew_blocks(size_t n) { size_t b = (n + 255) / 256; return (int)(b < 4096 ? (b ? b : 1) : 4096); }

extern "C" int mhe_bn_act_nhwc(const void *x, const float *scale, const float *shift, const void *res,
                               const float *res_scale, const float *res_shift, void *y, long P, int C, int relu,
                               int dtype, void *stream) {
    MHE_REQUIRE(x && scale && shift && y && P > 0 && C > 0 && C % 4 == 0, "mhe_bn_act_nhwc: bad arguments");
    const size_t n4 = (size_t)P * C / 4;
    if (dtype == MHE_F32)
        hipLaunchKernelGGL(conv::bn_act_kernel<float>, dim3(ew_blocks(n4)), dim3(256), 0, (hipStream_t)stream,
                           (const float *)x, scale, shift, (const float *)res, res_scale, res_shift, (float *)y, n4, C, relu);
    else
        hipLaunchKernelGGL(conv::bn_act_kernel<u16>, dim3(ew_blocks(n4)), dim3(256), 0, (hipStream_t)stream,
                           (const u16 *)x, scale, shift, (const u16 *)res, res_scale, res_shift, (u16 *)y, n4, C, relu);
    return check_launch("bn_act_kernel");
}

extern "C" int mhe_maxpool3x3s2_nhwc(const void *x, const float *scale, const float *shift, void *y, int B, int H, int W,
                                     int C, int dtype, void *stream) {
    MHE_REQUIRE(x && y && B > 0 && H > 0 && W > 0 && C % 4 == 0, "mhe_maxpool3x3s2_nhwc: bad arguments");
    const int Ho = (H + 2 - 3) / 2 + 1, Wo = (W + 2 - 3) / 2 + 1;
    const size_t n4 = (size_t)B * Ho * Wo * C / 4;
    if (dtype == MHE_F32)
        hipLaunchKernelGGL(conv::maxpool_kernel<float>, dim3(ew_blocks(n4)), dim3(256), 0, (hipStream_t)stream,
                           (const float *)x, scale, shift, (float *)y, B, H, W, C, Ho, Wo);
    else if (C % 8 == 0)
        hipLaunchKernelGGL(conv::maxpool8_kernel, dim3(ew_blocks(n4 / 2)), dim3(256), 0, (hipStream_t)stream,
                           (const u16 *)x, scale, shift, (u16 *)y, B, H, W, C, Ho, Wo);
    else
        hipLaunchKernelGGL(conv::maxpool_kernel<u16>, dim3(ew_blocks(n4)), dim3(256), 0, (hipStream_t)stream,
                           (const u16 *)x, scale, shift, (u16 *)y, B, H, W, C, Ho, Wo);
    return check_launch("maxpool_kernel");
}

extern "C" int mhe_avgpool_nhwc(const void *x, float *y, int B, int HW, int C, int dtype, void *stream) {
    MHE_REQUIRE(x && y && B > 0 && HW > 0 && C > 0, "mhe_avgpool_nhwc: bad arguments");
    dim3 grid((C + 63) / 64, B);
    if (dtype == MHE_F32)
        hipLaunchKernelGGL(conv::avgpool_kernel<float>, grid, dim3(256), 0, (hipStream_t)stream, (const float *)x, y, HW, C);
    else
        hipLaunchKernelGGL(conv::avgpool_kernel<u16>, grid, dim3(256), 0, (hipStream_t)stream, (const u16 *)x, y, HW, C);
    return check_launch("avgpool_kernel");
}

extern "C" int mhe_bn_act_avgpool_nhwc(const void *x, const float *scale, const float *shift, const void *res, const float *rscale,
                                       const float *rshift, float *y, int B, int HW, int C, int relu, int dtype, void *stream) {
    MHE_REQUIRE(x && scale && shift && y && B > 0 && HW > 0 && C > 0 && C % 4 == 0, "mhe_bn_act_avgpool_nhwc: bad arguments (C=%d must be a multiple of 4)", C);
    MHE_REQUIRE((rscale == nullptr) == (rshift == nullptr) && (res || !rscale), "mhe_bn_act_avgpool_nhwc: the residual's affine needs both tables and the residual");
    MHE_REQUIRE(dtype == MHE_F32 || dtype == MHE_BF16, "mhe_bn_act_avgpool_nhwc: dtype=%d", dtype);
    const dim3 grid((C + 255) / 256, B);
    if (dtype == MHE_F32)
        hipLaunchKernelGGL(conv::bn_act_avgpool_kernel<float>, grid, dim3(256), 0, (hipStream_t)stream, (const float *)x, scale, shift, (const float *)res,
                           rscale, rshift, y, HW, C, relu);
    else
        hipLaunchKernelGGL(conv::bn_act_avgpool_kernel<u16>, grid, dim3(256), 0, (hipStream_t)stream, (const u16 *)x, scale, shift, (const u16 *)res,
                           rscale, rshift, y, HW, C, relu);
    return check_launch("bn_act_avgpool_kernel");
}

extern "C" int mhe_nchw_to_nhwc(const float *x, void *y, int B, int C, int H, int W, int dtype, void *stream) {
    MHE_REQUIRE(x && y && B > 0 && C > 0 && H > 0 && W > 0, "mhe_nchw_to_nhwc: bad arguments");
    const int Cp = (C + elem_chunk(dtype) - 1) / elem_chunk(dtype) * elem_chunk(dtype);
    const size_t n = (size_t)B * H * W;
    if (dtype == MHE_F32)
        hipLaunchKernelGGL(conv::nchw_to_nhwc_kernel<float>, dim3(ew_blocks(n)), dim3(256), 0, (hipStream_t)stream, x,
                           (float *)y, B, C, H * W, Cp);
    else
        hipLaunchKernelGGL(conv::nchw_to_nhwc_kernel<u16>, dim3(ew_blocks(n)), dim3(256), 0, (hipStream_t)stream, x,
// ... 110 lines not shown
```

mhentropy_amd/csrc/conv_fuse.hip:

```cpp
#include "conv_shared.h"

namespace mhe { namespace conv {

namespace {
constexpr int FPIX = 128;
constexpr int FT = FPIX * 8;
typedef unsigned int u32x4 __attribute__((ext_vector_type(4)));
__device__ __forceinline__ __amdgpu_buffer_rsrc_t rsrc_of(const void *p, size_t bytes) {
    return __builtin_amdgcn_make_buffer_rsrc(const_cast<void *>(p), 0, (int)bytes, 0x00020000);
}
__device__ __forceinline__ uint4 bld(__amdgpu_buffer_rsrc_t r, unsigned toff, unsigned uoff) {
    const u32x4 v = __builtin_amdgcn_raw_buffer_load_b128(r, (int)toff, (int)uoff, 0);
    return make_uint4(v[0], v[1], v[2], v[3]);
}
__device__ __forceinline__ u32x4 bldv(__amdgpu_buffer_rsrc_t r, unsigned toff, unsigned uoff) {
    return __builtin_amdgcn_raw_buffer_load_b128(r, (int)toff, (int)uoff, 0);
}
__device__ __forceinline__ void bst(__amdgpu_buffer_rsrc_t r, unsigned toff, unsigned uoff, uint4 v) {
    const u32x4 t = {v.x, v.y, v.z, v.w};
    __builtin_amdgcn_raw_buffer_store_b128(t, r, (int)toff, (int)uoff, 0);
}
}

template <int CB, int N2>
__global__ __launch_bounds__(512) void bottleneck_tail_kernel(const Params p) {
    using T = u16;
    constexpr int C = 4 * CB, NT = C / 64, KT1 = CB / 64;
    constexpr int R3S = KT1 * 64 * 8, R1S = N2 * 8;
    constexpr int CPR2 = N2 * 2 / 16, RPP = 256 / CPR2, NJ2 = FPIX / RPP;
    static_assert(NT % 2 == 0 && KT1 >= 1 && KT1 <= 2 && (N2 == 64 || N2 == 128), "geometry");
    static_assert(FPIX * CPR2 <= 2 * FT, "the output tile is staged over Tbuf");
    __shared__ uint4 lds[4 * FT + 2 * R3S + 2 * R1S];
    __shared__ float aff[4 * C + 2 * CB];
    uint4 *Tbuf = lds, *Abuf = lds + 2 * FT, *R3 = lds + 4 * FT, *R1 = R3 + 2 * R3S;
    const int tid = threadIdx.x, wave = __builtin_amdgcn_readfirstlane(tid >> 6), lane = tid & 63, q = lane >> 4, l15 = lane & 15;
    const bool mult = wave < 4;
    const int t2 = tid & 255, s8 = t2 & 7, rbase = t2 >> 3;
    const int ntiles = p.M / FPIX;
    const bool idaff = p.x2_scale != nullptr;
    for (int i = tid; i < C; i += 512) {
        aff[i] = p.mid_scale[i]; aff[C + i] = p.mid_shift[i];
        aff[2 * C + i] = idaff ? p.x2_scale[i] : 1.f; aff[3 * C + i] = idaff ? p.x2_shift[i] : 0.f;
    }
    for (int i = tid; i < CB; i += 512) { aff[4 * C + i] = p.in_scale[i]; aff[4 * C + CB + i] = p.in_shift[i]; }
    __syncthreads();
    const __amdgpu_buffer_rsrc_t y2g = rsrc_of(p.x, (size_t)p.M * CB * 2), idg = rsrc_of(p.x2, (size_t)p.M * C * 2);
    const __amdgpu_buffer_rsrc_t w3g = rsrc_of(p.w3, (size_t)C * CB * 2), w1g = rsrc_of(p.w, (size_t)N2 * C * 2);
    const __amdgpu_buffer_rsrc_t ag = rsrc_of(p.a_out, (size_t)p.M * C * 2), yg = rsrc_of(p.y, (size_t)p.M * N2 * 2);
    const __amdgpu_buffer_rsrc_t abg = rsrc_of(p.a_bits, (size_t)p.M * (C / 8));
    const int cc = t2 % CPR2, r0 = t2 / CPR2;
    const unsigned toffC = (unsigned)(rbase * C + s8 * 8) * 2u, toffB = (unsigned)(rbase * CB + s8 * 8) * 2u, toffY = (unsigned)(r0 * N2 + cc * 8) * 2u;
    const bool st_on = p.stats != nullptr;
    float ss1[8], ss2[8];
#pragma unroll
    for (int i = 0; i < 8; ++i) ss1[i] = ss2[i] = 0.f;
    auto store_outputs = [&](int m0) __attribute__((always_inline)) {
        const unsigned char *ot = reinterpret_cast<const unsigned char *>(Tbuf);
        uint4 raw[NJ2];
#pragma unroll
        for (int j = 0; j < NJ2; ++j) {
            const int row = r0 + RPP * j;
            raw[j] = *reinterpret_cast<const uint4 *>(ot + ((size_t)row * CPR2 + (cc ^ (row & (CPR2 - 1)))) * 16);
        }
#pragma unroll
        for (int j = 0; j < NJ2; ++j) {
            if (st_on) {
                float f[8];
                Chunk<T>::unpack(raw[j], f);
#pragma unroll
                for (int i = 0; i < 8; ++i) { ss1[i] += f[i]; ss2[i] = fmaf(f[i], f[i], ss2[i]); }
            }
            bst(yg, toffY, (unsigned)(m0 + RPP * j) * (N2 * 2), raw[j]);
        }
    };

    if (mult) {
        for (int L = blockIdx.x; L < ntiles; L += (int)gridDim.x) {
            __syncthreads();
            uint4 fa[2][KT1 * 2];
#pragma unroll
            for (int m = 0; m < 2; ++m)
#pragma unroll
                for (int k = 0; k < KT1 * 2; ++k) fa[m][k] = Abuf[(k >> 1) * FT + swz(wave * 32 + m * 16 + l15, (k & 1) * 4 + q)];
            v4f acc2[N2 / 16][2];
#pragma unroll
            for (int a = 0; a < N2 / 16; ++a) { acc2[a][0] = v4f{0.f, 0.f, 0.f, 0.f}; acc2[a][1] = v4f{0.f, 0.f, 0.f, 0.f}; }
#pragma unroll
            for (int s = 0; s < NT + 2; ++s) {
                if (s > 0) __syncthreads();
                if (s < NT) {
                    const uint4 *W3s = R3 + (s & 1) * R3S;
                    v4f acc1[4][2];
#pragma unroll
                    for (int a = 0; a < 4; ++a) { acc1[a][0] = v4f{0.f, 0.f, 0.f, 0.f}; acc1[a][1] = v4f{0.f, 0.f, 0.f, 0.f}; }
#pragma unroll
                    for (int k = 0; k < KT1 * 2; ++k) {
                        uint4 fb[4];
#pragma unroll
                        for (int nt = 0; nt < 4; ++nt) fb[nt] = W3s[(k >> 1) * 512 + swz(nt * 16 + l15, (k & 1) * 4 + q)];
#pragma unroll
                        for (int nt = 0; nt < 4; ++nt)
#pragma unroll
                            for (int m = 0; m < 2; ++m)
                                acc1[nt][m] = __builtin_amdgcn_mfma_f32_16x16x32_bf16(
                                    __builtin_bit_cast(__attribute__((ext_vector_type(8))) __bf16, fb[nt]),
                                    __builtin_bit_cast(__attribute__((ext_vector_type(8))) __bf16, fa[m][k]), acc1[nt][m], 0, 0, 0);
                    }
                    unsigned char *tb = reinterpret_cast<unsigned char *>(Tbuf + (s & 1) * FT);
#pragma unroll
                    for (int nt = 0; nt < 4; ++nt)
#pragma unroll
                        for (int m = 0; m < 2; ++m) {
                            const int row = wave * 32 + m * 16 + l15, chunk = nt * 2 + (q >> 1);
                            const v4f v = acc1[nt][m];
                            uint2 o;
                            o.x = (unsigned)f32_to_bf16(v[0]) | ((unsigned)f32_to_bf16(v[1]) << 16);
                            o.y = (unsigned)f32_to_bf16(v[2]) | ((unsigned)f32_to_bf16(v[3]) << 16);
                            *reinterpret_cast<uint2 *>(tb + (size_t)swz(row, chunk) * 16 + (q & 1) * 8) = o;
                        }
                }
                if (s >= 2) {
                    const int t = s - 2;
                    const uint4 *As = Abuf + (t & 1) * FT, *W1s = R1 + (t & 1) * R1S;
#pragma unroll
                    for (int kk = 0; kk < 2; ++kk) {
                        uint4 fa2[2], fb2[N2 / 16];
#pragma unroll
                        for (int m = 0; m < 2; ++m) fa2[m] = As[swz(wave * 32 + m * 16 + l15, kk * 4 + q)];
#pragma unroll
                        for (int nt = 0; nt < N2 / 16; ++nt) fb2[nt] = W1s[swz(nt * 16 + l15, kk * 4 + q)];
#pragma unroll
                        for (int nt = 0; nt < N2 / 16; ++nt)
#pragma unroll
                            for (int m = 0; m < 2; ++m)
                                acc2[nt][m] = __builtin_amdgcn_mfma_f32_16x16x32_bf16(
                                    __builtin_bit_cast(__attribute__((ext_vector_type(8))) __bf16, fb2[nt]),
                                    __builtin_bit_cast(__attribute__((ext_vector_type(8))) __bf16, fa2[m]), acc2[nt][m], 0, 0, 0);
                    }
                }
            }
            __syncthreads();
            unsigned char *ot = reinterpret_cast<unsigned char *>(Tbuf);
#pragma unroll
            for (int nt = 0; nt < N2 / 16; ++nt)
#pragma unroll
                for (int m = 0; m < 2; ++m) {
                    const int row = wave * 32 + m * 16 + l15, boff = (nt * 16 + 4 * q) * 2;
                    const int chunk = (boff >> 4) ^ (row & (CPR2 - 1));
                    const v4f v = acc2[nt][m];
                    uint2 o;
                    o.x = (unsigned)f32_to_bf16(v[0]) | ((unsigned)f32_to_bf16(v[1]) << 16);
                    o.y = (unsigned)f32_to_bf16(v[2]) | ((unsigned)f32_to_bf16(v[3]) << 16);
                    *reinterpret_cast<uint2 *>(ot + ((size_t)row * CPR2 + chunk) * 16 + (boff & 15)) = o;
                }
            __syncthreads();
        }
    } else {
        struct IdSet { uint4 v[4]; };
        IdSet id0, id1;
        uint4 a2r[KT1 * 4];
        u32x4 w3r[KT1 * 2], w1r[N2 / 32];
        auto load_id = [&](int m0, int t, IdSet &st) __attribute__((always_inline)) {
#pragma unroll
            for (int j = 0; j < 4; ++j) st.v[j] = bld(idg, toffC, (unsigned)(m0 + 32 * j) * (C * 2) + t * 128);
        };
        auto load_a2 = [&](int m0) __attribute__((always_inline)) {
#pragma unroll
            for (int kt = 0; kt < KT1; ++kt)
#pragma unroll
                for (int j = 0; j < 4; ++j) a2r[kt * 4 + j] = bld(y2g, toffB, (unsigned)(m0 + 32 * j) * (CB * 2) + kt * 128);
        };
        auto load_w3 = [&](int t) __attribute__((always_inline)) {
#pragma unroll
            for (int kt = 0; kt < KT1; ++kt)
#pragma unroll
                for (int j = 0; j < 2; ++j) w3r[kt * 2 + j] = bldv(w3g, toffB, (unsigned)(t * 64 + 32 * j) * (CB * 2) + kt * 128);
        };
        auto store_w3 = [&](int t) __attribute__((always_inline)) {
            uint4 *dst = R3 + (t & 1) * R3S;
#pragma unroll
            for (int kt = 0; kt < KT1; ++kt)
#pragma unroll
                for (int j = 0; j < 2; ++j) *reinterpret_cast<u32x4 *>(dst + kt * 512 + swz(rbase + 32 * j, s8)) = w3r[kt * 2 + j];
        };
        auto load_w1 = [&](int t) __attribute__((always_inline)) {
#pragma unroll
            for (int j = 0; j < N2 / 32; ++j) w1r[j] = bldv(w1g, toffC, (unsigned)(32 * j) * (C * 2) + t * 128);
        };
        auto store_w1 = [&](int t) __attribute__((always_inline)) {
            uint4 *dst = R1 + (t & 1) * R1S;
#pragma unroll
            for (int j = 0; j < N2 / 32; ++j) *reinterpret_cast<u32x4 *>(dst + swz(rbase + 32 * j, s8)) = w1r[j];
        };
        auto xform = [&](int m0, int t, const IdSet &st) __attribute__((always_inline)) {
            const uint4 *Ts = Tbuf + (t & 1) * FT;
            uint4 *As = Abuf + (t & 1) * FT;
            const int kc = t * 64 + s8 * 8;
            float sc[8], sh[8], s2[8], h2[8];
#pragma unroll
            for (int h = 0; h < 2; ++h) {
                const float4 a0 = *reinterpret_cast<const float4 *>(aff + kc + 4 * h), a1 = *reinterpret_cast<const float4 *>(aff + C + kc + 4 * h);
                const float4 b0 = *reinterpret_cast<const float4 *>(aff + 2 * C + kc + 4 * h), b1 = *reinterpret_cast<const float4 *>(aff + 3 * C + kc + 4 * h);
                sc[4 * h] = a0.x; sc[4 * h + 1] = a0.y; sc[4 * h + 2] = a0.z; sc[4 * h + 3] = a0.w;
                sh[4 * h] = a1.x; sh[4 * h + 1] = a1.y; sh[4 * h + 2] = a1.z; sh[4 * h + 3] = a1.w;
                s2[4 * h] = b0.x; s2[4 * h + 1] = b0.y; s2[4 * h + 2] = b0.z; s2[4 * h + 3] = b0.w;
                h2[4 * h] = b1.x; h2[4 * h + 1] = b1.y; h2[4 * h + 2] = b1.z; h2[4 * h + 3] = b1.w;
            }
#pragma unroll
            for (int j = 0; j < 4; ++j) {
                const int row = rbase + 32 * j;
                float v[8], w[8];
                Chunk<T>::unpack(Ts[swz(row, s8)], v);
                Chunk<T>::unpack(st.v[j], w);
#pragma unroll
                for (int i = 0; i < 8; ++i) {
                    v[i] = fmaf(v[i], sc[i], sh[i]);
                    if (idaff) w[i] = fmaf(w[i], s2[i], h2[i]);
                    v[i] = fmaxf(v[i] + w[i], 0.f);
                }
                const uint4 o = Chunk<T>::pack(v);
                As[swz(row, s8)] = o;
                bst(ag, toffC, (unsigned)(m0 + 32 * j) * (C * 2) + t * 128, o);
                const unsigned wds[4] = {o.x, o.y, o.z, o.w};
                unsigned gb = 0;
#pragma unroll
                for (int i = 0; i < 4; ++i)
                    gb |= ((unsigned)((wds[i] & 0x8000u) == 0 && (wds[i] & 0x7fffu) != 0) << (2 * i)) |
                          ((unsigned)((wds[i] & 0x80000000u) == 0 && (wds[i] & 0x7fff0000u) != 0) << (2 * i + 1));
                if (p.a_bits) __builtin_amdgcn_raw_buffer_store_b8((unsigned char)gb, abg, (int)((rbase * (C / 8)) + s8), (int)((unsigned)(m0 + 32 * j) * (C / 8) + t * 8), 0);
            }
        };
        auto stage_a2 = [&]() __attribute__((always_inline)) {
#pragma unroll
            for (int kt = 0; kt < KT1; ++kt) {
                float sc[8], sh[8];
#pragma unroll
                for (int h = 0; h < 2; ++h) {
                    const float4 a0 = *reinterpret_cast<const float4 *>(aff + 4 * C + kt * 64 + s8 * 8 + 4 * h);
                    const float4 a1 = *reinterpret_cast<const float4 *>(aff + 4 * C + CB + kt * 64 + s8 * 8 + 4 * h);
                    sc[4 * h] = a0.x; sc[4 * h + 1] = a0.y; sc[4 * h + 2] = a0.z; sc[4 * h + 3] = a0.w;
                    sh[4 * h] = a1.x; sh[4 * h + 1] = a1.y; sh[4 * h + 2] = a1.z; sh[4 * h + 3] = a1.w;
                }
#pragma unroll
                for (int j = 0; j < 4; ++j) {
                    float v[8];
                    Chunk<T>::unpack(a2r[kt * 4 + j], v);
#pragma unroll
                    for (int i = 0; i < 8; ++i) v[i] = fmaxf(fmaf(v[i], sc[i], sh[i]), 0.f);
                    Abuf[kt * FT + swz(rbase + 32 * j, s8)] = Chunk<T>::pack(v);
                }
            }
        };
        {
            const int m0 = (int)blockIdx.x * FPIX;
            load_a2(m0); load_w3(0);
            load_id(m0, 0, id0); load_id(m0, 1, id1);
            load_w1(0);
        }
        for (int L = blockIdx.x; L < ntiles; L += (int)gridDim.x) {
            const int m0 = L * FPIX;
            const int Ln = L + (int)gridDim.x;
            const bool more = Ln < ntiles;
            const int m0n = more ? Ln * FPIX : m0;
            stage_a2();
            store_w3(0);
            load_w3(1);
            __syncthreads();
#pragma unroll
            for (int s = 0; s < NT + 2; ++s) {
                if (s > 0) __syncthreads();
                if (s >= 1 && s <= NT) {
                    const int t = s - 1;
                    if (t & 1) { xform(m0, t, id1); if (t + 2 < NT) load_id(m0, t + 2, id1); else load_id(m0n, t + 2 - NT, id1); }
                    else       { xform(m0, t, id0); if (t + 2 < NT) load_id(m0, t + 2, id0); else load_id(m0n, t + 2 - NT, id0); }
                    store_w1(t);
                    load_w1((t + 1) % NT);
                }
                if (s + 1 < NT) {
                    store_w3(s + 1);
                    load_w3((s + 2) % NT);
                }
                if (s == 1) load_a2(m0n);
            }
            __syncthreads();
            __syncthreads();
            store_outputs(m0);
        }
    }
    if (st_on) {
        float *red = reinterpret_cast<float *>(lds);
        __syncthreads();
        if (!mult) {
#pragma unroll
            for (int i = 0; i < 8; ++i) { red[t2 * 16 + i] = ss1[i]; red[t2 * 16 + 8 + i] = ss2[i]; }
        }
        __syncthreads();
        if (tid < N2) {
            const int ch = tid >> 3, e = tid & 7;
            float a = 0.f, b = 0.f;
            for (int k = 0; k < RPP; ++k) { a += red[(ch + CPR2 * k) * 16 + e]; b += red[(ch + CPR2 * k) * 16 + 8 + e]; }
            fx::add(p.stats, (int)blockIdx.x % NSH, 0, N2, tid, a);
            fx::add(p.stats, (int)blockIdx.x % NSH, 1, N2, tid, b);
        }
    }
}

bool fuse_supports(const Params &p, int cb) {
    return p.x && p.x2 && p.w && p.w3 && p.y && p.a_out && p.in_scale && p.in_shift && p.mid_scale && p.mid_shift &&
           (cb == 64 || cb == 128) && p.Cin == 4 * cb && (p.Cout == 64 || p.Cout == 128) && p.Kpad == p.Cin &&
           p.KH == 1 && p.KW == 1 && p.stride == 1 && p.pad == 0 && p.M % FPIX == 0 && p.M > 0;
}

int launch_fuse(const Params &p, int cb, hipStream_t s) {
    const int ntiles = p.M / FPIX;
    const dim3 grid((unsigned)(ntiles < 256 ? ntiles : 256)), block(512);
    if (cb == 64 && p.Cout == 64) hipLaunchKernelGGL((bottleneck_tail_kernel<64, 64>), grid, block, 0, s, p);
    else if (cb == 64 && p.Cout == 128) hipLaunchKernelGGL((bottleneck_tail_kernel<64, 128>), grid, block, 0, s, p);
    else if (cb == 128 && p.Cout == 64) hipLaunchKernelGGL((bottleneck_tail_kernel<128, 64>), grid, block, 0, s, p);
    else hipLaunchKernelGGL((bottleneck_tail_kernel<128, 128>), grid, block, 0, s, p);
    return check_launch("bottleneck_tail_kernel");
}

}}
```

mhentropy_amd/csrc/conv_shared.h:

```cpp
#pragma once
#include "common.h"
#include <type_traits>

namespace mhe { namespace conv {

struct Params {
    const void *x; const void *w; void *y;
    const float *in_scale, *in_shift, *out_scale, *out_shift;
    const void *residual;
    const void *mask;
    const void *bn_y[2]; const float *bn_mi[2]; fx::acc_t *bn_stats[2];
    fx::acc_t *stats;
    const void *x2; const float *x2_scale, *x2_shift; void *a_out;
    int B, H, W, Cin, Cout, KH, KW, stride, pad, Ho, Wo, M, Kpad, relu_in, relu_out;
    float *y32;
    int force;
    int os2, os_py, os_px;
    int res_s2;
    const void *w3; const float *mid_scale, *mid_shift;
    int stats_only;
    const void *xcat; int Cin2;
    unsigned char *a_bits; const unsigned char *mask_bits;
    const float *rev_coef;
};

__device__ __forceinline__ long out_pixel(const Params &p, int m) {
    if (m >= p.M) return -1l;
    if (!p.os2) return (long)m;
    const int j = m % p.Wo, t = m / p.Wo, i = t % p.Ho, b = t / p.Ho;
    return ((long)(b * 2 * p.Ho + 2 * i + p.os_py)) * (2 * p.Wo) + 2 * j + p.os_px;
}

constexpr int NSH = fx::NSH;
constexpr int MAXC = 2048;

template <typename T> struct El;
template <> struct El<float> { static constexpr int CE = 4; };
template <> struct El<u16>   { static constexpr int CE = 8; };

__device__ __forceinline__ int swz(int row, int slot) { return row * 8 + (slot ^ ((row >> 1) & 7)); }

template <typename T> struct Chunk;
template <> struct Chunk<float> {
    static constexpr int N = 4;
    static __device__ __forceinline__ void unpack(uint4 r, float *v) {
        v[0] = __uint_as_float(r.x); v[1] = __uint_as_float(r.y); v[2] = __uint_as_float(r.z); v[3] = __uint_as_float(r.w);
    }
    static __device__ __forceinline__ uint4 pack(const float *v) {
        return make_uint4(__float_as_uint(v[0]), __float_as_uint(v[1]), __float_as_uint(v[2]), __float_as_uint(v[3]));
    }
};
template <> struct Chunk<u16> {
    static constexpr int N = 8;
    static __device__ __forceinline__ void unpack(uint4 r, float *v) {
        const unsigned in[4] = {r.x, r.y, r.z, r.w};
#pragma unroll
        for (int i = 0; i < 4; ++i) { v[2 * i] = __uint_as_float(in[i] << 16); v[2 * i + 1] = __uint_as_float(in[i] & 0xffff0000u); }
    }
    static __device__ __forceinline__ uint4 pack(const float *v) {
        unsigned o[4];
#pragma unroll
        for (int i = 0; i < 4; ++i) o[i] = (unsigned)f32_to_bf16(v[2 * i]) | ((unsigned)f32_to_bf16(v[2 * i + 1]) << 16);
        return make_uint4(o[0], o[1], o[2], o[3]);
    }
};

template <typename T>
__device__ __forceinline__ uint4 in_transform(uint4 raw, const float *sc, const float *sh, int c, int relu,
                                              bool dual, uint4 raw2, const float *sc2, const float *sh2) {
    constexpr int N = Chunk<T>::N;
    float v[N], ss[N], tt[N];
    Chunk<T>::unpack(raw, v);
#pragma unroll
    for (int i = 0; i < N; i += 4) {
        const float4 a = *reinterpret_cast<const float4 *>(sc + c + i), b = *reinterpret_cast<const float4 *>(sh + c + i);
        ss[i] = a.x; ss[i + 1] = a.y; ss[i + 2] = a.z; ss[i + 3] = a.w;
        tt[i] = b.x; tt[i + 1] = b.y; tt[i + 2] = b.z; tt[i + 3] = b.w;
    }
#pragma unroll
    for (int i = 0; i < N; ++i) v[i] = fmaf(v[i], ss[i], tt[i]);
    if (dual) {
        float w[N];
        Chunk<T>::unpack(raw2, w);
        if (sc2) {
#pragma unroll
            for (int i = 0; i < N; i += 4) {
                const float4 a = *reinterpret_cast<const float4 *>(sc2 + c + i), b = *reinterpret_cast<const float4 *>(sh2 + c + i);
                w[i] = fmaf(w[i], a.x, b.x); w[i + 1] = fmaf(w[i + 1], a.y, b.y);
                w[i + 2] = fmaf(w[i + 2], a.z, b.z); w[i + 3] = fmaf(w[i + 3], a.w, b.w);
            }
        }
#pragma unroll
        for (int i = 0; i < N; ++i) v[i] += w[i];
    }
    if (relu) {
#pragma unroll
        for (int i = 0; i < N; ++i) v[i] = fmaxf(v[i], 0.f);
    }
    return Chunk<T>::pack(v);
}

#ifndef MHE_CONV_XCD_ORDER
#define MHE_CONV_XCD_ORDER 1
#endif
constexpr bool XCD_ORDER = MHE_CONV_XCD_ORDER;
#ifndef MHE_CONV_BN_EPILOGUE
#define MHE_CONV_BN_EPILOGUE 1
#endif
constexpr bool BN_EPILOGUE = MHE_CONV_BN_EPILOGUE;
__device__ __forceinline__ void tile_of_block(int &mt, int &nt) {
    const int gm = gridDim.x, gn = gridDim.y;
    mt = blockIdx.x; nt = blockIdx.y;
    if (XCD_ORDER && gn > 1 && (gm & 7) == 0) {
        const int L = blockIdx.x + gm * blockIdx.y, slot = L >> 3;
        nt = slot % gn;
        mt = (slot / gn) * 8 + (L & 7);
    }
}

__device__ __forceinline__ long res_half_row(const Params &p, long m) {
    const int j = (int)(m % p.Wo), t = (int)(m / p.Wo), i = t % p.Ho, b = t / p.Ho;
    if ((i | j) & 1) return -1l;
    const int Hh = (p.Ho + 1) >> 1, Wh = (p.Wo + 1) >> 1;
    return ((long)(b * Hh + (i >> 1))) * Wh + (j >> 1);
}

template <typename T, int BM, int BN, int NTH, bool DG, int GROWS = (NTH >= 512 ? 4 : 2), int MAXU = 2, typename PixF>
__device__ __forceinline__ void epilogue_store(const Params &p, unsigned char *ot, int shard, int n0, PixF pix) {
    const int tid = threadIdx.x;
    constexpr int CPR = BN * (int)sizeof(T) / 16;
    constexpr int CMASK = (CPR - 1) & 15;
    constexpr int EPC = 16 / (int)sizeof(T);
    float *const lds = reinterpret_cast<float *>(ot);
    {
        T *yg = reinterpret_cast<T *>(p.y);
        const T *rg = reinterpret_cast<const T *>(p.residual);
        const T *mk = DG ? reinterpret_cast<const T *>(p.mask) : nullptr;
        const bool bnr = DG && BN_EPILOGUE && p.bn_y[0] != nullptr;
        const bool plain = !p.out_scale && !p.out_shift && !rg && !p.relu_out && !mk && !bnr;
        static_assert(NTH % CPR == 0, "a thread keeps one 16-byte column chunk across its rows");
        float bs1[DG ? MAXU : 1][EPC], bs2[DG ? MAXU : 1][EPC], bmu[DG ? MAXU : 1][EPC], biv[DG ? MAXU : 1][EPC];
        const int cfix = tid % CPR;
        float bsh[DG ? EPC : 1];
        if constexpr (DG) {
#pragma unroll
            for (int i = 0; i < EPC; ++i) bsh[i] = p.out_shift && n0 + cfix * EPC + i < p.Cout ? p.out_shift[n0 + cfix * EPC + i] : 0.f;
        }
        if constexpr (DG) if (bnr) {
#pragma unroll
            for (int u = 0; u < MAXU; ++u)
#pragma unroll
                for (int i = 0; i < EPC; ++i) {
                    const int n = n0 + cfix * EPC + i;
                    const bool ok = p.bn_y[u] && n < p.Cout;
                    bs1[u][i] = bs2[u][i] = 0.f;
                    bmu[u][i] = ok ? p.bn_mi[u][n] : 0.f;
                    biv[u][i] = ok ? p.bn_mi[u][p.Cout + n] : 0.f;
                }
        }
        const bool st_on = !DG && p.stats != nullptr;
        float ss1[EPC], ss2[EPC];
#pragma unroll
        for (int i = 0; i < EPC; ++i) ss1[i] = ss2[i] = 0.f;
        bool done = false;
        if constexpr (DG) {
            if (mk && pix(0) >= 0 && pix(BM - 1) >= 0 && n0 + BN <= p.Cout && !p.out_scale && !p.relu_out) {
                done = true;
                const int nbn = bnr ? (MAXU == 2 && p.bn_y[1] ? 2 : 1) : 0;
                const T *y0g = reinterpret_cast<const T *>(p.bn_y[0]), *y1g = reinterpret_cast<const T *>(MAXU == 2 ? p.bn_y[1] : nullptr);
                auto run = [&](auto RES, auto NB) {
                    constexpr bool HAS_RES = decltype(RES)::value;
                    constexpr int NBN = decltype(NB)::value, NJ = BM * CPR / NTH;
                    constexpr int G = GROWS;
                    static_assert(NJ % G == 0, "rows per thread");
#pragma unroll 1
                    for (int j0 = 0; j0 < NJ; j0 += G) {
                        uint4 raw[G], gm[G], rr[HAS_RES ? G : 1], ya[NBN >= 1 ? G : 1], yb[NBN == 2 ? G : 1];
// ... 210 lines not shown
```

mhentropy_amd/csrc/conv_tail.hip:

```cpp
#include "conv_shared.h"

namespace mhe { namespace conv {

namespace {

constexpr int TBM = 128, TBN = 256, TBK = 64, TMAXK = 2048;
constexpr int T_A = TBM * 8, T_W = TBN * 8, T_STAGE = T_A + T_W;

}

template <bool DG>
__global__ __launch_bounds__(512) void conv_tail_kernel(const Params p) {
    using T = u16;
    __shared__ uint4 lds[2 * T_STAGE];
    __shared__ float aff[4 * TMAXK];
    const int tid = threadIdx.x, wave = __builtin_amdgcn_readfirstlane(tid >> 6), lane = tid & 63, q = lane >> 4, l15 = lane & 15;
    const bool mult = wave < 4;
    const int t2 = tid & 255, s = t2 & 7, rbase = t2 >> 3;
    const int K = p.Cin, nk = K / TBK;
    const int gm = p.M / TBM, gn = p.Cout / TBN, ntiles = gm * gn;
    auto tile_at = [&](int L, int &mt, int &nt) __attribute__((always_inline)) {
        if (gn > 1 && (gm & 7) == 0) {
            const int slot = L >> 3;
            nt = slot % gn;
            mt = (slot / gn) * 8 + (L & 7);
        } else { mt = L % gm; nt = L / gm; }
    };
    const bool aff2 = p.x2_scale != nullptr;
    for (int i = tid; i < K; i += 512) {
        aff[i] = p.in_scale[i]; aff[K + i] = p.in_shift[i];
        aff[2 * K + i] = aff2 ? p.x2_scale[i] : 1.f; aff[3 * K + i] = aff2 ? p.x2_shift[i] : 0.f;
    }
    const T *xg = reinterpret_cast<const T *>(p.x), *x2g = reinterpret_cast<const T *>(p.x2), *wg = reinterpret_cast<const T *>(p.w);
    T *yg = reinterpret_cast<T *>(p.y);
    struct Set { uint4 a[4], b[4], w[8]; };
    Set st0, st1;
    auto load_tile = [&](int t, Set &st, int m0, int n0) __attribute__((always_inline)) {
        const int kc = t * TBK + s * 8;
#pragma unroll
        for (int j = 0; j < 4; ++j) {
            const size_t off = (size_t)(m0 + rbase + 32 * j) * K + kc;
            st.a[j] = *reinterpret_cast<const uint4 *>(xg + off);
            st.b[j] = *reinterpret_cast<const uint4 *>(x2g + off);
        }
#pragma unroll
        for (int j = 0; j < 8; ++j) st.w[j] = *reinterpret_cast<const uint4 *>(wg + (size_t)(n0 + rbase + 32 * j) * p.Kpad + kc);
    };
    auto store_tile = [&](int t, const Set &st, int m0, T *ag) __attribute__((always_inline)) {
        uint4 *At = lds + (t & 1) * T_STAGE, *Wt = At + T_A;
        const int kc = t * TBK + s * 8;
        float sc[8], sh[8], s2[8], h2[8];
#pragma unroll
        for (int h = 0; h < 2; ++h) {
            const float4 a0 = *reinterpret_cast<const float4 *>(aff + kc + 4 * h), a1 = *reinterpret_cast<const float4 *>(aff + K + kc + 4 * h);
            const float4 b0 = *reinterpret_cast<const float4 *>(aff + 2 * K + kc + 4 * h), b1 = *reinterpret_cast<const float4 *>(aff + 3 * K + kc + 4 * h);
            sc[4 * h] = a0.x; sc[4 * h + 1] = a0.y; sc[4 * h + 2] = a0.z; sc[4 * h + 3] = a0.w;
            sh[4 * h] = a1.x; sh[4 * h + 1] = a1.y; sh[4 * h + 2] = a1.z; sh[4 * h + 3] = a1.w;
            s2[4 * h] = b0.x; s2[4 * h + 1] = b0.y; s2[4 * h + 2] = b0.z; s2[4 * h + 3] = b0.w;
            h2[4 * h] = b1.x; h2[4 * h + 1] = b1.y; h2[4 * h + 2] = b1.z; h2[4 * h + 3] = b1.w;
        }
#pragma unroll
        for (int j = 0; j < 4; ++j) {
            float v[8], w[8];
            Chunk<T>::unpack(st.a[j], v);
            Chunk<T>::unpack(st.b[j], w);
#pragma unroll
            for (int i = 0; i < 8; ++i) {
                v[i] = fmaf(v[i], sc[i], sh[i]);
                if (aff2) w[i] = fmaf(w[i], s2[i], h2[i]);
                v[i] += w[i];
                if (p.relu_in) v[i] = fmaxf(v[i], 0.f);
            }
            const uint4 o = Chunk<T>::pack(v);
            At[swz(rbase + 32 * j, s)] = o;
            if (ag) *reinterpret_cast<uint4 *>(ag + (size_t)(m0 + rbase + 32 * j) * K + kc) = o;
        }
#pragma unroll
        for (int j = 0; j < 8; ++j) Wt[swz(rbase + 32 * j, s)] = st.w[j];
    };
    const bool st_on = p.stats != nullptr;
    auto store_outputs = [&](int mt, int m0, int n0) __attribute__((always_inline)) {
        const unsigned char *ot = reinterpret_cast<const unsigned char *>(lds);
        const int cc = tid & 31, r0 = tid >> 5;
        float *red = reinterpret_cast<float *>(lds);
        auto fold = [&](const float *a8, const float *b8, fx::acc_t *dst) __attribute__((always_inline)) {
            __syncthreads();
#pragma unroll
            for (int i = 0; i < 8; ++i) { red[tid * 16 + i] = a8[i]; red[tid * 16 + 8 + i] = b8[i]; }
            __syncthreads();
            if (tid < 256) {
                const int ch = tid >> 3, e = tid & 7;
                float a = 0.f, b = 0.f;
                for (int k = 0; k < 16; ++k) { a += red[(ch + 32 * k) * 16 + e]; b += red[(ch + 32 * k) * 16 + 8 + e]; }
                fx::add(dst, mt % NSH, 0, p.Cout, n0 + tid, a);
                fx::add(dst, mt % NSH, 1, p.Cout, n0 + tid, b);
            }
        };
        if constexpr (DG) {
            const T *mk = reinterpret_cast<const T *>(p.mask), *rg = reinterpret_cast<const T *>(p.residual);
            const T *y0g = reinterpret_cast<const T *>(p.bn_y[0]), *y1g = reinterpret_cast<const T *>(p.bn_y[1]);
            const int ccol = n0 + cc * 8;
            float bs1[2][8], bs2[2][8], bmu[2][8], biv[2][8];
#pragma unroll
            for (int u = 0; u < 2; ++u)
#pragma unroll
                for (int i = 0; i < 8; ++i) {
                    const bool ok = p.bn_y[u] != nullptr;
                    bs1[u][i] = bs2[u][i] = 0.f;
                    bmu[u][i] = ok ? p.bn_mi[u][ccol + i] : 0.f;
                    biv[u][i] = ok ? p.bn_mi[u][p.Cout + ccol + i] : 0.f;
                }
#pragma unroll 1
            for (int j0 = 0; j0 < 8; j0 += 4) {
                uint4 raw[4], gm[4], rr[4], ya[4], yb[4];
#pragma unroll
                for (int j = 0; j < 4; ++j) {
                    const int row = r0 + 16 * (j0 + j);
                    const size_t off = (size_t)(m0 + row) * p.Cout + ccol;
                    gm[j] = *reinterpret_cast<const uint4 *>(mk + off);
                    rr[j] = rg ? *reinterpret_cast<const uint4 *>(rg + off) : make_uint4(0, 0, 0, 0);
                    if (y0g) ya[j] = *reinterpret_cast<const uint4 *>(y0g + off);
                    if (y1g) yb[j] = *reinterpret_cast<const uint4 *>(y1g + off);
                    raw[j] = *reinterpret_cast<const uint4 *>(ot + ((size_t)row * 32 + (cc ^ (row & 31))) * 16);
                }
#pragma unroll
                for (int j = 0; j < 4; ++j) {
                    const int row = r0 + 16 * (j0 + j);
                    float v[8], t[8];
                    Chunk<T>::unpack(raw[j], v);
                    if (rg) {
                        Chunk<T>::unpack(rr[j], t);
#pragma unroll
                        for (int i = 0; i < 8; ++i) v[i] += t[i];
                    }
                    Chunk<T>::unpack(gm[j], t);
#pragma unroll
                    for (int i = 0; i < 8; ++i) v[i] = t[i] > 0.f ? v[i] : 0.f;
                    if (y0g) {
                        Chunk<T>::unpack(ya[j], t);
#pragma unroll
                        for (int i = 0; i < 8; ++i) { bs1[0][i] += v[i]; bs2[0][i] = fmaf(v[i], (t[i] - bmu[0][i]) * biv[0][i], bs2[0][i]); }
                    }
                    if (y1g) {
                        Chunk<T>::unpack(yb[j], t);
#pragma unroll
                        for (int i = 0; i < 8; ++i) { bs1[1][i] += v[i]; bs2[1][i] = fmaf(v[i], (t[i] - bmu[1][i]) * biv[1][i], bs2[1][i]); }
                    }
                    *reinterpret_cast<uint4 *>(yg + (size_t)(m0 + row) * p.Cout + ccol) = Chunk<T>::pack(v);
                }
            }
#pragma unroll
            for (int u = 0; u < 2; ++u)
                if (p.bn_y[u]) fold(bs1[u], bs2[u], p.bn_stats[u]);
        } else {
            float ss1[8], ss2[8];
#pragma unroll
            for (int i = 0; i < 8; ++i) ss1[i] = ss2[i] = 0.f;
            uint4 raw[8];
#pragma unroll
            for (int j = 0; j < 8; ++j) {
                const int row = r0 + 16 * j;
                raw[j] = *reinterpret_cast<const uint4 *>(ot + ((size_t)row * 32 + (cc ^ (row & 31))) * 16);
            }
#pragma unroll
            for (int j = 0; j < 8; ++j) {
                const int row = r0 + 16 * j;
                if (st_on) {
                    float f[8];
                    Chunk<T>::unpack(raw[j], f);
#pragma unroll
                    for (int i = 0; i < 8; ++i) { ss1[i] += f[i]; ss2[i] = fmaf(f[i], f[i], ss2[i]); }
                }
                *reinterpret_cast<uint4 *>(yg + (size_t)(m0 + row) * p.Cout + n0 + cc * 8) = raw[j];
            }
            if (st_on) fold(ss1, ss2, p.stats);
        }
    };
    if (mult) {
        for (int L = blockIdx.x; L < ntiles; L += (int)gridDim.x) {
            int mt, ntile;
            tile_at(L, mt, ntile);
            __syncthreads();
            v4f acc[4][8];
#pragma unroll
            for (int a = 0; a < 4; ++a)
#pragma unroll
                for (int b = 0; b < 8; ++b) acc[a][b] = v4f{0.f, 0.f, 0.f, 0.f};
            for (int t = 0; t < nk; ++t) {
                __syncthreads();
                const uint4 *At = lds + (t & 1) * T_STAGE, *Wt = At + T_A + wave * 64 * 8;
#pragma unroll
                for (int kk = 0; kk < 2; ++kk) {
                    uint4 fa[8], fb[4];
#pragma unroll
                    for (int nt = 0; nt < 4; ++nt) fb[nt] = Wt[swz(nt * 16 + l15, kk * 4 + q)];
#pragma unroll
                    for (int m = 0; m < 8; ++m) fa[m] = At[swz(m * 16 + l15, kk * 4 + q)];
#pragma unroll
                    for (int m = 0; m < 8; ++m)
#pragma unroll
                        for (int nt = 0; nt < 4; ++nt)
                            acc[nt][m] = __builtin_amdgcn_mfma_f32_16x16x32_bf16(
                                __builtin_bit_cast(__attribute__((ext_vector_type(8))) __bf16, fb[nt]),
                                __builtin_bit_cast(__attribute__((ext_vector_type(8))) __bf16, fa[m]), acc[nt][m], 0, 0, 0);
                }
            }
            __syncthreads();
            unsigned char *ot = reinterpret_cast<unsigned char *>(lds);
#pragma unroll
            for (int nt = 0; nt < 4; ++nt)
#pragma unroll
                for (int m = 0; m < 8; ++m) {
                    const int row = m * 16 + l15, boff = (wave * 64 + nt * 16 + 4 * q) * 2;
                    const int chunk = (boff >> 4) ^ (row & 31);
                    const v4f v = acc[nt][m];
                    uint2 o;
                    o.x = (unsigned)f32_to_bf16(v[0]) | ((unsigned)f32_to_bf16(v[1]) << 16);
                    o.y = (unsigned)f32_to_bf16(v[2]) | ((unsigned)f32_to_bf16(v[3]) << 16);
                    *reinterpret_cast<uint2 *>(ot + ((size_t)row * 32 + chunk) * 16 + (boff & 15)) = o;
                }
            __syncthreads();
            store_outputs(mt, mt * TBM, ntile * TBN);
        }
    } else {
        int mt, ntile;
        tile_at(blockIdx.x, mt, ntile);
        load_tile(0, st0, mt * TBM, ntile * TBN);
        if (1 < nk) load_tile(1, st1, mt * TBM, ntile * TBN);
        for (int L = blockIdx.x; L < ntiles; L += (int)gridDim.x) {
            tile_at(L, mt, ntile);
            const int m0 = mt * TBM, n0 = ntile * TBN;
            T *ag = p.a_out && ntile == 0 ? reinterpret_cast<T *>(p.a_out) : nullptr;
            __syncthreads();
            store_tile(0, st0, m0, ag);
            if (2 < nk) load_tile(2, st0, m0, n0);
            auto tick = [&](int t, Set &st) __attribute__((always_inline)) {
                __syncthreads();
                if (t + 1 < nk) store_tile(t + 1, st, m0, ag);
                if (t + 3 < nk) load_tile(t + 3, st, m0, n0);
            };
            for (int t = 0; t < nk; t += 2) {
                tick(t, st1);
                if (t + 1 < nk) tick(t + 1, st0);
            }
            __syncthreads();
            if constexpr (!DG) {
                if (L + (int)gridDim.x < ntiles) {
                    int mt2, nt2;
                    tile_at(L + (int)gridDim.x, mt2, nt2);
                    load_tile(0, st0, mt2 * TBM, nt2 * TBN);
                    if (1 < nk) load_tile(1, st1, mt2 * TBM, nt2 * TBN);
                }
            }
            __syncthreads();
            store_outputs(mt, m0, n0);
            if constexpr (DG) {
                if (L + (int)gridDim.x < ntiles) {
                    int mt2, nt2;
                    tile_at(L + (int)gridDim.x, mt2, nt2);
                    load_tile(0, st0, mt2 * TBM, nt2 * TBN);
                    if (1 < nk) load_tile(1, st1, mt2 * TBM, nt2 * TBN);
                }
            }
        }
    }
}


bool tail_supports(const Params &p) {
    if (p.mask ? (p.stats != nullptr) : (p.residual != nullptr)) return false;
    return p.x2 && p.in_scale && !p.out_scale && !p.out_shift && !p.relu_out && !p.y32 && !p.os2 && !p.res_s2 &&
           p.KH == 1 && p.KW == 1 && p.stride == 1 && p.pad == 0 && p.Kpad == p.Cin && p.Cin % TBK == 0 && p.Cin >= 2 * TBK && p.Cin <= TMAXK &&
           p.Cout % TBN == 0 && p.M % TBM == 0;
}

int launch_tail(const Params &p, hipStream_t s) {
    const int ntiles = (p.M / TBM) * (p.Cout / TBN);
    const dim3 grid((unsigned)(ntiles < 256 ? ntiles : 256));
    if (p.mask) hipLaunchKernelGGL(conv_tail_kernel<true>, grid, dim3(512), 0, s, p);
    else hipLaunchKernelGGL(conv_tail_kernel<false>, grid, dim3(512), 0, s, p);
    return check_launch("conv_tail_kernel");
}

}}
```

mhentropy_amd/ops.py:

```python
import ctypes as C
import os

import numpy as np
import torch

from . import _lib
from ._lib import ConvDesc, check

F32, BF16 = 0, 1
FLOW_FORWARD, FLOW_INVERSE = 0, 1

TIMING = False
TIMING_DG = False
KERNEL_TIMES = []


def _stream():
    return C.c_void_p(torch.cuda.current_stream().cuda_stream)


def _ptr(t):
    return C.c_void_p(0 if t is None else t.data_ptr())


# ... 507 lines not shown
    check(_lib.lib().mhe_conv2d_nhwc(C.byref(d), _ptr(x), _ptr(w), _ptr(y), _ptr(in_scale), _ptr(in_shift),
                                     _ptr(out_scale), _ptr(out_shift), _ptr(residual), _ptr(stats), _stream()),
          "mhe_conv2d_nhwc")
    if TIMING:
        ev1.record()
        es = x.element_size()
        nbytes = es * (x.numel() + y.numel() + w.numel() + (residual.numel() if residual is not None else 0))
        KERNEL_TIMES.append((_conv_kernel_name(d, dt, 1 if in_scale is not None else 3 if residual is not None else 0),
                             2.0 * B * Ho * Wo * Cout * KH * KW * Cin, ev0, ev1, nbytes))
    return y


def conv1x1_stats(x, w, in_scale, in_shift, stats):
    B, H, W, Cin = x.shape
    Cout = w.shape[0]
    _chk(x, torch.bfloat16, "conv_stats.x"); _chk(w, torch.bfloat16, "conv_stats.w", (Cout, Cin))
    _chk(in_scale, torch.float32, "conv_stats.in_scale", (Cin,)); _chk(in_shift, torch.float32, "conv_stats.in_shift", (Cin,))
    _chk_stats(stats, "conv_stats.stats", Cout)
    d = ConvDesc(B, H, W, Cin, Cout, 1, 1, 1, 0, BF16, 1, 0, 0, 0)
    if TIMING:
        ev0, ev1 = torch.cuda.Event(enable_timing=True), torch.cuda.Event(enable_timing=True)
        ev0.record()
    check(_lib.lib().mhe_conv1x1_stats_nhwc(C.byref(d), _ptr(x), _ptr(w), _ptr(in_scale), _ptr(in_shift), _ptr(stats), _stream()), "mhe_conv1x1_stats_nhwc")
    if TIMING:
        ev1.record()
        name = "mhe::conv::conv_wide_kernel<128, 4, true>" if Cin == 256 else "mhe::conv::conv1x1_stream_kernel<%d, 256, true, false>" % (Cin // 64)
        KERNEL_TIMES.append((name, 2.0 * B * H * W * Cout * Cin, ev0, ev1, 2 * (x.numel() + w.numel())))
    return stats


def gram_buffers(Cb, device):
    L = _lib.lib()
    return (torch.zeros(L.mhe_gram_stats_words(Cb), device=device, dtype=STAT_DTYPE),
            torch.empty(L.mhe_gram_stats_workspace_bytes(Cb) // 8, device=device, dtype=torch.float64))


def conv1x1_gram_bn(x, in_scale, in_shift, w, bn_weight, bn_bias, running_mean, running_var, bufs, momentum=0.1, eps=1e-5, num_batches_tracked=None,
                    want_mean_invstd=False, a_out=None):
    B, H, W, Cb = x.shape
    Cn = w.shape[0]
    _chk(x, torch.bfloat16, "gram.x"); _chk(w, torch.bfloat16, "gram.w", (Cn, Cb))
    _chk(in_scale, torch.float32, "gram.in_scale", (Cb,)); _chk(in_shift, torch.float32, "gram.in_shift", (Cb,))
    gram, ws = bufs
    L = _lib.lib()
    _chk(gram, STAT_DTYPE, "gram.accumulators", (L.mhe_gram_stats_words(Cb),))
    if TIMING:
        ev0, ev1 = torch.cuda.Event(enable_timing=True), torch.cuda.Event(enable_timing=True)
        ev0.record()
    if a_out is not None:
        _chk(a_out, torch.bfloat16, "gram.a_out", (B, H, W, Cb))
    check(L.mhe_conv1x1_gram_store_nhwc(_ptr(x), _ptr(in_scale), _ptr(in_shift), 1, _ptr(gram), _ptr(a_out), B * H * W, Cb, _stream()), "mhe_conv1x1_gram_store_nhwc")
    if TIMING:
        ev1.record()
        KERNEL_TIMES.append(("mhe::conv::gram_kernel<%d>" % Cb, 2.0 * B * H * W * Cb * Cb, ev0, ev1, 2 * x.numel()))
    scale = torch.empty(Cn, device=x.device, dtype=torch.float32)
    shift = torch.empty_like(scale)
    mi = torch.empty(2, Cn, device=x.device, dtype=torch.float32) if want_mean_invstd else None
    check(L.mhe_gram_bn_finalize(_ptr(gram), _ptr(ws), _ptr(w), _ptr(bn_weight), _ptr(bn_bias), _ptr(running_mean), _ptr(running_var), _ptr(scale),
                                 _ptr(shift), _ptr(mi), Cn, Cb, float(B * H * W), float(momentum), float(eps), _ptr(num_batches_tracked), _stream()),
          "mhe_gram_bn_finalize")
    return (scale, shift, mi) if want_mean_invstd else (scale, shift)


def gram_workspace(Cb, device):
    return torch.empty(_lib.lib().mhe_gram_stats_workspace_bytes(Cb) // 8, device=device, dtype=torch.float64)


def conv3_bn_fold(D, w, gram_totals, rev_stats, gamma, mean_invstd, count, dgamma, dbeta, dW, w_dg, S, c0, coef_ws):
    Cn, Cb = w.shape
    if S is None:
        _chk(w_dg, torch.bfloat16, "fold.w_cat", (Cb, Cn + Cb))
        s_ptr, ld_s = C.c_void_p(w_dg.data_ptr() + 2 * Cn), Cn + Cb
    else:
        _chk(S, torch.bfloat16, "fold.S", (Cb, Cb))
        s_ptr, ld_s = _ptr(S), Cb
    _chk(D, torch.float32, "fold.D", (Cn, Cb)); _chk(w, torch.bfloat16, "fold.w", (Cn, Cb)); _chk(gram_totals, torch.float64, "fold.gram")
    _chk_stats(rev_stats, "fold.rev_stats", Cn); _chk(gamma, torch.float32, "fold.gamma", (Cn,))
    _chk(mean_invstd, torch.float32, "fold.mean_invstd", (2, Cn)); _chk(dgamma, torch.float32, "fold.dgamma", (Cn,)); _chk(dbeta, torch.float32, "fold.dbeta", (Cn,))
    _chk(dW, torch.float32, "fold.dW"); _chk(w_dg, torch.bfloat16, "fold.w_dg")
    _chk(c0, torch.float32, "fold.c0", (Cb,)); _chk(coef_ws, torch.float32, "fold.coef_ws")
    if gram_totals.numel() < Cb * Cb + Cb or dW.numel() < Cn * Cb or w_dg.shape[0] != Cb or w_dg.shape[1] < Cn or coef_ws.numel() < 2 * Cn:
        raise ValueError("conv3_bn_fold: operand sizes")
    check(_lib.lib().mhe_conv3_bn_fold(_ptr(D), _ptr(w), _ptr(gram_totals), _ptr(rev_stats), _ptr(gamma), _ptr(mean_invstd), float(count), _ptr(dgamma),
                                       _ptr(dbeta), _ptr(dW), _ptr(w_dg), int(w_dg.shape[1]), s_ptr, int(ld_s), _ptr(c0), _ptr(coef_ws), Cn, Cb, _stream()),
          "mhe_conv3_bn_fold")


def conv3x3_halo_supported(B, H, W, Cin, Cout):
    return bool(_lib.lib().mhe_conv3x3_halo_supported(int(B), int(H), int(W), int(Cin), int(Cout)))


def conv3x3_halo_pack(w):
    _chk(w, torch.bfloat16, "halo_pack.w")
    Cout, K = w.shape
    if K % 9 or (K // 9) % 64 or Cout % 128:
        raise ValueError(f"conv3x3_halo_pack: weight rows [{Cout}][{K}] are not 9 x (a multiple of 64) wide / a multiple of 128 many")
    out = torch.empty_like(w)
    check(_lib.lib().mhe_conv3x3_halo_pack_bf16(_ptr(w), _ptr(out), int(Cout), int(K // 9), _stream()), "mhe_conv3x3_halo_pack_bf16")
    return out


def conv3x3_halo(x, w_halo, in_scale=None, in_shift=None, relu_in=False, a_out=None, stats=None, residual=None, mask=None, bn=None):
    B, H, W, Cin = x.shape
    Cout = w_halo.shape[0]
    _chk(x, torch.bfloat16, "halo.x"); _chk(w_halo, torch.bfloat16, "halo.w", (Cout, 9 * Cin))
    y = torch.empty(B, H, W, Cout, device=x.device, dtype=torch.bfloat16)
    for t, name, shape in ((in_scale, "in_scale", (Cin,)), (in_shift, "in_shift", (Cin,))):
        if t is not None:
            _chk(t, torch.float32, "halo." + name, shape)
    if stats is not None:
        _chk_stats(stats, "halo.stats", Cout)
    for t, name, shape in ((a_out, "a_out", tuple(x.shape)), (residual, "residual", tuple(y.shape)), (mask, "mask", tuple(y.shape))):
        if t is not None:
            _chk(t, torch.bfloat16, "halo." + name, shape)
    by, bmi, bst = (None, None, None) if bn is None else bn
    if by is not None:
        _chk(by, torch.bfloat16, "halo.bn_y", tuple(y.shape)); _chk(bmi, torch.float32, "halo.bn_mi", (2, Cout)); _chk_stats(bst, "halo.bn_stats", Cout)
    if TIMING:
        ev0, ev1 = torch.cuda.Event(enable_timing=True), torch.cuda.Event(enable_timing=True)
        ev0.record()
    check(_lib.lib().mhe_conv3x3_halo_nhwc(B, H, W, Cin, Cout, _ptr(x), _ptr(w_halo), _ptr(y), _ptr(in_scale), _ptr(in_shift), int(bool(relu_in)),
                                           _ptr(a_out), _ptr(stats), _ptr(residual), _ptr(mask), _ptr(by), _ptr(bmi), _ptr(bst), _stream()),
          "mhe_conv3x3_halo_nhwc")
    if TIMING:
        ev1.record()
        KERNEL_TIMES.append(("mhe::conv::conv_halo_kernel<%d, %s>" % (W, "true" if mask is not None else "false"), 2.0 * B * H * W * Cout * 9 * Cin, ev0, ev1,
                             2 * (x.numel() + y.numel() + w_halo.numel())))
    return y


def conv3x3_halo_dgrad_bn(g, y_raw, coef, w_halo, mask, gy_out=None, residual=None, bn=None):
    B, H, W, Cin = g.shape
    Cout = w_halo.shape[0]
    _chk(g, torch.bfloat16, "halo_dg.g"); _chk(y_raw, torch.bfloat16, "halo_dg.y", tuple(g.shape)); _chk(coef, torch.float32, "halo_dg.coef", (3, Cin))
    _chk(w_halo, torch.bfloat16, "halo_dg.w", (Cout, 9 * Cin)); _chk(mask, torch.bfloat16, "halo_dg.mask", (B, H, W, Cout))
    gx = torch.empty(B, H, W, Cout, device=g.device, dtype=torch.bfloat16)
    if gy_out is not None:
        _chk(gy_out, torch.bfloat16, "halo_dg.gy_out", tuple(g.shape))
    if residual is not None:
        _chk(residual, torch.bfloat16, "halo_dg.residual", tuple(gx.shape))
    by, bmi, bst = (None, None, None) if bn is None else bn
    if by is not None:
        _chk(by, torch.bfloat16, "halo_dg.bn_y", tuple(gx.shape)); _chk(bmi, torch.float32, "halo_dg.bn_mi", (2, Cout)); _chk_stats(bst, "halo_dg.bn_stats", Cout)
    check(_lib.lib().mhe_conv3x3_halo_dgrad_bn_nhwc(B, H, W, Cin, Cout, _ptr(g), _ptr(y_raw), _ptr(coef), _ptr(w_halo), _ptr(gx), _ptr(gy_out), _ptr(residual),
                                                    _ptr(mask), _ptr(by), _ptr(bmi), _ptr(bst), _stream()), "mhe_conv3x3_halo_dgrad_bn_nhwc")
    return gx


def bottleneck_tail_supported(B, H, W, Cb, Cout):
    d = ConvDesc(B, H, W, 4 * Cb, Cout, 1, 1, 1, 0, BF16, 1, 0, 0, 0)
    return bool(_lib.lib().mhe_bottleneck_tail_supported(C.byref(d), int(Cb)))


def bottleneck_tail(y2, bn2, w3, bn3, identity, id_aff, w1, stats=None, want_bits=False):
    B, H, W, Cb = y2.shape
    Cw, Cout = w3.shape[0], w1.shape[0]
    _chk(y2, torch.bfloat16, "tail.y2"); _chk(w3, torch.bfloat16, "tail.w3", (Cw, Cb)); _chk(w1, torch.bfloat16, "tail.w1", (Cout, Cw))
    _chk(identity, torch.bfloat16, "tail.identity", (B, H, W, Cw))
    for (sc, sh), n, c in ((bn2, "bn2", Cb), (bn3, "bn3", Cw)) + (((id_aff, "id", Cw),) if id_aff is not None else ()):
        _chk(sc, torch.float32, f"tail.{n}_scale", (c,)); _chk(sh, torch.float32, f"tail.{n}_shift", (c,))
    if stats is not None:
        _chk_stats(stats, "tail.stats", Cout)
    a = torch.empty(B, H, W, Cw, device=y2.device, dtype=torch.bfloat16)
    y1 = torch.empty(B, H, W, Cout, device=y2.device, dtype=torch.bfloat16)
    bits = torch.empty(B, H, W, Cw // 8, device=y2.device, dtype=torch.uint8) if want_bits else None
    d = ConvDesc(B, H, W, Cw, Cout, 1, 1, 1, 0, BF16, 1, 0, 0, 0)
    if TIMING:
        ev0, ev1 = torch.cuda.Event(enable_timing=True), torch.cuda.Event(enable_timing=True)
        ev0.record()
    check(_lib.lib().mhe_bottleneck_tail_bits_nhwc(C.byref(d), Cb, _ptr(y2), _ptr(bn2[0]), _ptr(bn2[1]), _ptr(w3), _ptr(bn3[0]), _ptr(bn3[1]), _ptr(identity),
                                                   _ptr(id_aff[0] if id_aff is not None else None), _ptr(id_aff[1] if id_aff is not None else None),
                                                   _ptr(w1), _ptr(a), _ptr(bits), _ptr(y1), _ptr(stats), _stream()), "mhe_bottleneck_tail_bits_nhwc")
    if TIMING:
        ev1.record()
        nbytes = 2 * (y2.numel() + identity.numel() + a.numel() + y1.numel() + w3.numel() + w1.numel())
        KERNEL_TIMES.append(("mhe::conv::bottleneck_tail_kernel<%d, %d>" % (Cb, Cout), 2.0 * B * H * W * Cw * (Cb + Cout), ev0, ev1, nbytes))
    return (a, y1, bits) if want_bits else (a, y1)


def linear_bf16_f32out(x, w, bias=None, out=None):
    R, K = x.shape
    N = w.shape[0]
    _chk(x, torch.bfloat16, "linear_bf16.x"); _chk(w, torch.bfloat16, "linear_bf16.w", (N, K))
    if bias is not None:
        _chk(bias, torch.float32, "linear_bf16.bias", (N,))
    y = out if out is not None else torch.empty(R, N, device=x.device, dtype=torch.float32)
    _chk(y, torch.float32, "linear_bf16.out", (R, N))
    d = ConvDesc(R, 1, 1, K, N, 1, 1, 1, 0, BF16, 0, 0, 0)
    check(_lib.lib().mhe_conv2d_f32out_nhwc(C.byref(d), _ptr(x), _ptr(w), _ptr(y), _ptr(bias), _stream()), "mhe_conv2d_f32out_nhwc")
    return y


def conv3x3s2_dgrad(gy, w4, residual=None, mask=None, bn=None, tile=0):
    B, Ho, Wo, Cout = gy.shape
    dt = gy.dtype
    Cin = w4[0].shape[0]
    _chk(gy, dt, "dgrad_s2.gy")
    for i, w in enumerate(w4):
        _chk(w, dt, f"dgrad_s2.w{i}")
    dx = torch.empty(B, 2 * Ho, 2 * Wo, Cin, device=gy.device, dtype=dt)
    for t, name in ((residual, "residual"), (mask, "mask")):
        if t is not None:
            _chk(t, dt, "dgrad_s2." + name, dx.shape)
    ext = []
    for by, bmi, bst in (list(bn or []) + [(None, None, None)] * 2)[:2]:
        if by is not None:
            _chk(by, dt, "dgrad_s2.bn_y", dx.shape); _chk(bmi, torch.float32, "dgrad_s2.bn_mean_invstd", (2, Cin))
            _chk_stats(bst, "dgrad_s2.bn_stats", Cin)
        ext += [_ptr(by), _ptr(bmi), _ptr(bst)]
    wp = (C.c_void_p * 4)(*[w.data_ptr() for w in w4])
    check(_lib.lib().mhe_conv3x3s2_dgrad_nhwc(B, Ho, Wo, Cout, Cin, dtype_code(dt), _ptr(gy), wp, _ptr(dx), _ptr(residual), _ptr(mask), *ext, int(tile), _stream()),
          "mhe_conv3x3s2_dgrad_nhwc")
    return dx


def conv1x1_residual_in(x, x2, w, in_scale, in_shift, x2_scale=None, x2_shift=None, a_out=None, stats=None, tile=0):
    B, H, W, Cin = x.shape
    Cout = w.shape[0]
    dt = x.dtype
    _chk(x, dt, "conv_res.x"); _chk(x2, dt, "conv_res.x2", x.shape); _chk(w, dt, "conv_res.w")
    _chk(in_scale, torch.float32, "conv_res.in_scale", (Cin,)); _chk(in_shift, torch.float32, "conv_res.in_shift", (Cin,))
    if x2_scale is not None:
        _chk(x2_scale, torch.float32, "conv_res.x2_scale", (Cin,)); _chk(x2_shift, torch.float32, "conv_res.x2_shift", (Cin,))
    if a_out is not None:
        _chk(a_out, dt, "conv_res.a_out", x.shape)
    if stats is not None:
        _chk_stats(stats, "conv_res.stats", Cout)
    y = torch.empty(B, H, W, Cout, device=x.device, dtype=dt)
    d = ConvDesc(B, H, W, Cin, Cout, 1, 1, 1, 0, dtype_code(dt), 1, 0, int(tile))
    if TIMING:
        ev0, ev1 = torch.cuda.Event(enable_timing=True), torch.cuda.Event(enable_timing=True)
        ev0.record()
    check(_lib.lib().mhe_conv1x1_residual_in_nhwc(C.byref(d), _ptr(x), _ptr(x2), _ptr(w), _ptr(y), _ptr(in_scale), _ptr(in_shift),
                                                  _ptr(x2_scale), _ptr(x2_shift), _ptr(a_out), _ptr(stats), _stream()),
          "mhe_conv1x1_residual_in_nhwc")
    if TIMING:
        ev1.record()
        es = x.element_size()
        nbytes = es * (2 * x.numel() + y.numel() + w.numel() + (a_out.numel() if a_out is not None else 0))
        name = _conv_kernel_name(d, dt, 2)
        KERNEL_TIMES.append((name, 2.0 * B * H * W * Cout * Cin, ev0, ev1, nbytes))
    return y


def conv1x1_dgrad_bn_apply(g, y_raw, coef, w_dg, a_out, mask, bn=None, zeros=None, tile=0):
    B, H, W, Cin = g.shape
    Cout = w_dg.shape[0]
    dt = g.dtype
    _chk(g, dt, "dgrad_apply.g"); _chk(y_raw, dt, "dgrad_apply.y", g.shape); _chk(w_dg, dt, "dgrad_apply.w"); _chk(a_out, dt, "dgrad_apply.a_out", g.shape)
    _chk(coef, torch.float32, "dgrad_apply.coef", (3, Cin)); _chk(mask, dt, "dgrad_apply.mask", (B, H, W, Cout))
    if zeros is None:
        zeros = torch.zeros(Cin, device=g.device, dtype=torch.float32)
    _chk(zeros, torch.float32, "dgrad_apply.zeros", (Cin,))
    out = torch.empty(B, H, W, Cout, device=g.device, dtype=dt)
    by, bmi, bst = bn[0] if bn else (None, None, None)
    if by is not None:
        _chk(by, dt, "dgrad_apply.bn_y", out.shape); _chk(bmi, torch.float32, "dgrad_apply.bn_mean_invstd", (2, Cout))
        _chk_stats(bst, "dgrad_apply.bn_stats", Cout)
    d = ConvDesc(B, H, W, Cin, Cout, 1, 1, 1, 0, dtype_code(dt), 0, 0, int(tile))
    check(_lib.lib().mhe_conv1x1_residual_in_masked_nhwc(C.byref(d), _ptr(g), _ptr(y_raw), _ptr(w_dg), _ptr(out), _ptr(coef[0]), _ptr(coef[2]),
                                                         _ptr(coef[1]), _ptr(zeros), _ptr(a_out), None, _ptr(mask), _ptr(by), _ptr(bmi), _ptr(bst),
                                                         _stream()), "mhe_conv1x1_residual_in_masked_nhwc")
    return out


def stem_conv7x7s2(x, w, dtype, stats=None):
    B, Cn, H, W = x.shape
    _chk(x, torch.float32, "stem.x"); _chk(w, dtype, "stem.w", (64, 192))
    if Cn != 3:
        raise _lib.MheError("stem.x: expected 3 input channels")
    Ho, Wo = (H - 1) // 2 + 1, (W - 1) // 2 + 1
    y = torch.empty(B, Ho, Wo, 64, device=x.device, dtype=dtype)
    if stats is not None:
        _chk_stats(stats, "stem.stats", 64)
    if TIMING:
        ev0, ev1 = torch.cuda.Event(enable_timing=True), torch.cuda.Event(enable_timing=True)
        ev0.record()
    check(_lib.lib().mhe_stem_conv7x7s2(_ptr(x), _ptr(w), _ptr(y), _ptr(stats), B, H, W, dtype_code(dtype), _stream()),
          "mhe_stem_conv7x7s2")
    if TIMING:
        ev1.record()
        KERNEL_TIMES.append(("mhe::conv::stem_kernel<%s>" % ("float" if dtype == torch.float32 else "unsigned short"),
                             2.0 * B * Ho * Wo * 64 * 147, ev0, ev1, 4 * x.numel() + y.element_size() * y.numel()))
    return y


def stem_pool_supported(B, H, W, dtype):
    return bool(_lib.lib().mhe_stem_pool_supported(B, H, W, dtype_code(dtype)))


def stem_conv7x7s2_pool(x, w, bn_gamma, stats=None):
    B, Cn, H, W = x.shape
    _chk(x, torch.float32, "stem_pool.x"); _chk(w, torch.bfloat16, "stem_pool.w", (64, 192)); _chk(bn_gamma, torch.float32, "stem_pool.gamma", (64,))
    if Cn != 3:
        raise _lib.MheError("stem_pool.x: expected 3 input channels")
    if stats is not None:
        _chk_stats(stats, "stem_pool.stats", 64)
    y = torch.empty(B, 64, 64, 64, device=x.device, dtype=torch.bfloat16)
    if TIMING:
        ev0, ev1 = torch.cuda.Event(enable_timing=True), torch.cuda.Event(enable_timing=True)
        ev0.record()
    check(_lib.lib().mhe_stem_conv7x7s2_pool(_ptr(x), _ptr(w), _ptr(bn_gamma), _ptr(y), _ptr(stats), B, H, W, _stream()), "mhe_stem_conv7x7s2_pool")
    if TIMING:
        ev1.record()
        KERNEL_TIMES.append(("mhe::conv::stem_pool_kernel", 2.0 * B * 128 * 128 * 64 * 147, ev0, ev1, 4 * x.numel() + 2 * y.numel()))
    return y


def bn_finalize(stats, gamma, beta, running_mean, running_var, count, momentum=0.1, eps=1e-5, want_mean_invstd=False, clear=False,
                num_batches_tracked=None):
    Cn = gamma.shape[0]
    _chk_stats(stats, "bn_finalize.stats", Cn)
    scale = torch.empty(Cn, device=gamma.device, dtype=torch.float32)
    shift = torch.empty_like(scale)
    mi = torch.empty(2, Cn, device=gamma.device, dtype=torch.float32) if want_mean_invstd else None
    if clear or num_batches_tracked is not None:
        if num_batches_tracked is not None and (num_batches_tracked.dtype != torch.int64 or not num_batches_tracked.is_cuda):
            raise _lib.MheError("bn_finalize.num_batches_tracked: int64 device tensor expected")
        check(_lib.lib().mhe_bn_finalize_step(_ptr(stats), _ptr(gamma), _ptr(beta), _ptr(running_mean), _ptr(running_var), _ptr(scale), _ptr(shift),
                                              _ptr(mi), Cn, float(count), float(momentum), float(eps), int(clear), _ptr(num_batches_tracked), _stream()),
              "mhe_bn_finalize_step")
    else:
        check(_lib.lib().mhe_bn_finalize(_ptr(stats), _ptr(gamma), _ptr(beta), _ptr(running_mean), _ptr(running_var),
                                         _ptr(scale), _ptr(shift), _ptr(mi), Cn, float(count), float(momentum), float(eps), _stream()),
              "mhe_bn_finalize")
    return (scale, shift, mi) if want_mean_invstd else (scale, shift)


def bn_act(x, scale, shift, res=None, res_scale=None, res_shift=None, relu=True, out=None):
    Cn = x.shape[-1]
    P = x.numel() // Cn
    y = out if out is not None else torch.empty_like(x)
    with _Timed(lambda: "mhe::conv::bn_act_kernel<%s>" % ("float" if x.dtype == torch.float32 else "unsigned short"), 0.0, x.element_size() * x.numel() * (2 + (res is not None))):
        check(_lib.lib().mhe_bn_act_nhwc(_ptr(x), _ptr(scale), _ptr(shift), _ptr(res), _ptr(res_scale), _ptr(res_shift),
                                         _ptr(y), P, Cn, int(relu), dtype_code(x.dtype), _stream()), "mhe_bn_act_nhwc")
    return y


def maxpool3x3s2(x, scale=None, shift=None):
    B, H, W, Cn = x.shape
    Ho, Wo = (H - 1) // 2 + 1, (W - 1) // 2 + 1
    y = torch.empty(B, Ho, Wo, Cn, device=x.device, dtype=x.dtype)
    check(_lib.lib().mhe_maxpool3x3s2_nhwc(_ptr(x), _ptr(scale), _ptr(shift), _ptr(y), B, H, W, Cn, dtype_code(x.dtype),
                                           _stream()), "mhe_maxpool3x3s2_nhwc")
    return y


def avgpool(x):
    B, H, W, Cn = x.shape
    y = torch.empty(B, Cn, device=x.device, dtype=torch.float32)
    check(_lib.lib().mhe_avgpool_nhwc(_ptr(x), _ptr(y), B, H * W, Cn, dtype_code(x.dtype), _stream()), "mhe_avgpool_nhwc")
    return y


def bn_act_avgpool(x, scale, shift, res=None, rscale=None, rshift=None, relu=True):
    B, H, W, Cn = x.shape
    _chk(x, x.dtype, "bn_act_avgpool.x"); _chk(scale, torch.float32, "bn_act_avgpool.scale", (Cn,)); _chk(shift, torch.float32, "bn_act_avgpool.shift", (Cn,))
    if res is not None:
        _chk(res, x.dtype, "bn_act_avgpool.res", x.shape)
    if rscale is not None:
        _chk(rscale, torch.float32, "bn_act_avgpool.rscale", (Cn,)); _chk(rshift, torch.float32, "bn_act_avgpool.rshift", (Cn,))
    y = torch.empty(B, Cn, device=x.device, dtype=torch.float32)
    check(_lib.lib().mhe_bn_act_avgpool_nhwc(_ptr(x), _ptr(scale), _ptr(shift), _ptr(res), _ptr(rscale), _ptr(rshift), _ptr(y), B, H * W, Cn, int(relu),
                                             dtype_code(x.dtype), _stream()), "mhe_bn_act_avgpool_nhwc")
    return y


def nchw_to_nhwc(x, dtype=torch.float32, cpad=None):
    B, Cn, H, W = x.shape
    _chk(x, torch.float32, "nchw_to_nhwc.x")
    ce = 4 if dtype == torch.float32 else 8
    Cp = (Cn + ce - 1) // ce * ce if cpad is None else int(cpad)
    y = torch.empty(B, H, W, Cp, device=x.device, dtype=dtype)
    if cpad is None:
        check(_lib.lib().mhe_nchw_to_nhwc(_ptr(x), _ptr(y), B, Cn, H, W, dtype_code(dtype), _stream()), "mhe_nchw_to_nhwc")
    else:
        check(_lib.lib().mhe_nchw_to_nhwc_pad(_ptr(x), _ptr(y), B, Cn, Cp, H, W, dtype_code(dtype), _stream()), "mhe_nchw_to_nhwc_pad")
    return y


_WGRAD_WS = {}
_WGRAD_WS_RETIRED = []


def _wgrad_ws(device, need):
    ws = _WGRAD_WS.get(device)
    if ws is None or ws.numel() < need:
        if ws is not None:
            _WGRAD_WS_RETIRED.append(ws)
        ws = _WGRAD_WS[device] = torch.empty(need, device=device, dtype=torch.float32)
    return ws
WGRAD_SLABS = True

# ... 688 lines not shown
```

mhentropy_amd/resnet.py:

```python
import torch
from torch import nn

from . import ops

CFG = {
    "resnet18": ("basic", (2, 2, 2, 2), 512),
    "resnet50": ("bottleneck", (3, 4, 6, 3), 2048),
}
BN_EPS, BN_MOMENTUM = 1e-5, 0.1


def pack_conv_weight(w, dtype, cin_pad=None):
    Cout, Cin, KH, KW = w.shape
    cin_pad = cin_pad or Cin
    bke = 32 if dtype == torch.float32 else 64
    wp = torch.zeros(Cout, KH, KW, cin_pad, dtype=torch.float32, device=w.device)
    wp[..., :Cin] = w.detach().float().permute(0, 2, 3, 1)
    k = KH * KW * cin_pad
    kpad = (k + bke - 1) // bke * bke
    out = torch.zeros(Cout, kpad, dtype=torch.float32, device=w.device)
    out[:, :k] = wp.reshape(Cout, k)
    return out.to(dtype).contiguous()


def pack_stem_weight(w, dtype):
    wp = torch.zeros(64, 8, 24, dtype=torch.float32, device=w.device)
    wp[:, :7, :21] = w.detach().float().permute(0, 2, 3, 1).reshape(64, 7, 21)
    return wp.reshape(64, 192).to(dtype).contiguous()


class _Block(nn.Module):
    def __init__(self, kind, inplanes, planes, stride):
        super().__init__()
        self.kind, self.stride = kind, stride
        exp = 4 if kind == "bottleneck" else 1
        if kind == "bottleneck":
            self.conv1 = nn.Conv2d(inplanes, planes, 1, bias=False); self.bn1 = nn.BatchNorm2d(planes)
            self.conv2 = nn.Conv2d(planes, planes, 3, stride, 1, bias=False); self.bn2 = nn.BatchNorm2d(planes)
            self.conv3 = nn.Conv2d(planes, planes * 4, 1, bias=False); self.bn3 = nn.BatchNorm2d(planes * 4)
        else:
            self.conv1 = nn.Conv2d(inplanes, planes, 3, stride, 1, bias=False); self.bn1 = nn.BatchNorm2d(planes)
            self.conv2 = nn.Conv2d(planes, planes, 3, 1, 1, bias=False); self.bn2 = nn.BatchNorm2d(planes)
        if stride != 1 or inplanes != planes * exp:
            self.downsample = nn.Sequential(nn.Conv2d(inplanes, planes * exp, 1, stride, bias=False),
                                            nn.BatchNorm2d(planes * exp))
        else:
            self.downsample = None


class ResNetTrunk(nn.Module):
    def __init__(self, arch="resnet50", compute_dtype=torch.float32):
        super().__init__()
        kind, blocks, self.feat_dim = CFG[arch]
        self.arch, self.kind = arch, kind
        self.compute_dtype = compute_dtype
        self.conv1 = nn.Conv2d(3, 64, 7, 2, 3, bias=False)
        self.bn1 = nn.BatchNorm2d(64)
        inplanes, exp = 64, (4 if kind == "bottleneck" else 1)
        for li, (planes, nb) in enumerate(zip((64, 128, 256, 512), blocks)):
            layer = []
            for bi in range(nb):
                layer.append(_Block(kind, inplanes, planes, 2 if (bi == 0 and li > 0) else 1))
                inplanes = planes * exp
            setattr(self, f"layer{li + 1}", nn.Sequential(*layer))
        self.fc = nn.Identity()
        self._wcache = {}
        import os
        self.bn_apply = os.environ.get("MHE_BN_APPLY", "pass")
        self.bn_apply_1x1 = os.environ.get("MHE_BN_APPLY_1X1", "auto")
        self.bn_apply_3x3 = os.environ.get("MHE_BN_APPLY_3X3", "auto")
        self.bn_load_s2 = int(os.environ.get("MHE_BN_LOAD_S2", "256"))
        self.conv_halo = os.environ.get("MHE_CONV_HALO", "1") == "1"
        self.fuse_tail = os.environ.get("MHE_FUSE_TAIL", "1") == "1"
        self.fuse_recompute = os.environ.get("MHE_FUSE_RECOMPUTE", "1") == "1"
        self.recompute_stats = os.environ.get("MHE_RECOMPUTE_STATS", "gram")
        self.stem_pool_fused = os.environ.get("MHE_STEM_POOL", "1") == "1"
        self.fuse_pool = os.environ.get("MHE_FUSE_POOL", "1") == "1"

    def _w(self, conv, cin_pad=None, stem=False):
        p = conv.weight
        ext = getattr(self, "_external_w", None)
        if ext is not None and id(p) in ext:
            return ext[id(p)]
        key = (id(p), p._version, self.compute_dtype, p.device)
        hit = self._wcache.get(id(p))
        if hit is None or hit[0] != key:
            hit = (key, pack_stem_weight(p, self.compute_dtype) if stem else pack_conv_weight(p, self.compute_dtype, cin_pad))
            self._wcache[id(p)] = hit
        return hit[1]

    def _w_halo(self, conv):
        if getattr(self, "_external_w", None) is not None:
            return None
        p = conv.weight
        key = (id(p), p._version, "halo", p.device)
        hit = self._wcache.get(("halo", id(p)))
        if hit is None or hit[0] != key:
            hit = (key, ops.conv3x3_halo_pack(self._w(conv)))
            self._wcache[("halo", id(p))] = hit
        return hit[1]

    def _bn_affine(self, y, bn, st, count=None):
        if self.training:
            count = count if count is not None else y.numel() // y.shape[-1]
            return ops.bn_finalize(st, bn.weight, bn.bias, bn.running_mean, bn.running_var, count, BN_MOMENTUM, BN_EPS, clear=True,
                                   num_batches_tracked=bn.num_batches_tracked)
        sc = bn.weight.detach() / torch.sqrt(bn.running_var + BN_EPS)
        return sc.contiguous(), (bn.bias.detach() - bn.running_mean * sc).contiguous()

    def _conv_bn(self, x, conv, bn, stats_pool, in_aff=None, stride=1, pad=0, k=1, cin_pad=None, apply=None):
        w = self._w(conv, cin_pad)
        if in_aff is not None and (apply or self.bn_apply) == "pass":
            x = ops.bn_act(x, in_aff[0], in_aff[1], relu=True, out=x)
            in_aff = None
        isc, ish = in_aff if in_aff is not None else (None, None)
        st = stats_pool.take(conv.out_channels) if self.training else None
        y = ops.conv2d_nhwc(x, w, k, k, stride, pad, in_scale=isc, in_shift=ish, relu_in=in_aff is not None, stats=st)
        return y, self._bn_affine(y, bn, st)

    def forward(self, x):
        dt = self.compute_dtype
        if getattr(self, "_external_sync", None) is not None:
            self._external_sync()
        pool = self._stats_pool(x.device) if self.training else None
        st = pool.take(64) if self.training else None
        blocks = [blk for li in range(4) for blk in getattr(self, f"layer{li + 1}")]
        a_aff = None
        if (self.stem_pool_fused and blocks[0].kind == "bottleneck" and blocks[0].downsample is not None
                and ops.stem_pool_supported(x.shape[0], x.shape[2], x.shape[3], dt)):
            a = ops.stem_conv7x7s2_pool(x.contiguous(), self._w(self.conv1, stem=True), self.bn1.weight.detach(), stats=st)
            a_aff = self._bn_affine(None, self.bn1, st, count=x.shape[0] * 128 * 128)
        else:
            y = ops.stem_conv7x7s2(x.contiguous(), self._w(self.conv1, stem=True), dt, stats=st)
            aff = self._bn_affine(y, self.bn1, st)
            a = ops.maxpool3x3s2(y, aff[0], aff[1])
        pending = None
        for bi, blk in enumerate(blocks):
            if blk.kind == "bottleneck":
                if pending is not None and isinstance(pending[0], str):
                    _, y2_p, a2_p, w3_p, al_p, idt_p, idaff_p = pending
                    st = pool.take(blk.conv1.out_channels) if self.training else None
                    a, y1 = ops.bottleneck_tail(y2_p, a2_p, w3_p, al_p, idt_p, idaff_p, self._w(blk.conv1), stats=st)
                    a1 = self._bn_affine(y1, blk.bn1, st)
                    pending = None
                elif pending is not None:
                    yl_p, al_p, idt_p, idaff_p = pending
                    a = torch.empty_like(yl_p)
                    st = pool.take(blk.conv1.out_channels) if self.training else None
                    y1 = ops.conv1x1_residual_in(yl_p, idt_p, self._w(blk.conv1), al_p[0], al_p[1],
                                                 None if idaff_p is None else idaff_p[0],
                                                 None if idaff_p is None else idaff_p[1], a_out=a, stats=st)
                    a1 = self._bn_affine(y1, blk.bn1, st)
                    pending = None
                else:
                    y1, a1 = self._conv_bn(a, blk.conv1, blk.bn1, pool, a_aff, apply="load")
                ap2 = "load" if self.bn_apply_3x3 == "auto" and (ops.conv_tile_choice(
                    y1.shape[0], y1.shape[1], y1.shape[2], y1.shape[3], blk.conv2.out_channels, 3, blk.stride, 1, y1.dtype, 1) == 9
                    or (blk.stride == 2 and blk.conv2.in_channels <= self.bn_load_s2)) else None
                wh = None
                if (self.conv_halo and blk.stride == 1 and y1.dtype == torch.bfloat16 and self.bn_apply_3x3 == "auto"
                        and ops.conv3x3_halo_supported(y1.shape[0], y1.shape[1], y1.shape[2], y1.shape[3], blk.conv2.out_channels)):
                    wh = self._w_halo(blk.conv2)
                if wh is not None:
                    st2 = pool.take(blk.conv2.out_channels) if self.training else None
                    y2 = ops.conv3x3_halo(y1, wh, a1[0], a1[1], relu_in=True, stats=st2)
                    a2 = self._bn_affine(y2, blk.bn2, st2)
                else:
                    y2, a2 = self._conv_bn(y1, blk.conv2, blk.bn2, pool, a1, blk.stride, 1, 3, apply=ap2)
                ap3 = self.bn_apply_1x1 if self.bn_apply_1x1 != "auto" else ("load" if blk.conv3.in_channels <= 128 or ops.conv_tile_choice(
                    y2.shape[0], y2.shape[1], y2.shape[2], y2.shape[3], blk.conv3.out_channels, 1, 1, 0, y2.dtype, 1) == 11 else "pass")
                nxt = blocks[bi + 1] if bi + 1 < len(blocks) else None
                recompute = (self.fuse_recompute and self.fuse_tail and nxt is not None and nxt.kind == "bottleneck" and y2.dtype == torch.bfloat16
                             and nxt.conv1.kernel_size == (1, 1) and nxt.conv1.stride == (1, 1)
                             and ops.bottleneck_tail_supported(y2.shape[0], y2.shape[1], y2.shape[2], y2.shape[3], nxt.conv1.out_channels))
                if recompute:
                    w3 = self._w(blk.conv3)
                    st3 = None
                    if self.training and self.recompute_stats == "gram":
                        bn3 = blk.bn3
                        yl, al = None, ops.conv1x1_gram_bn(y2, a2[0], a2[1], w3, bn3.weight, bn3.bias, bn3.running_mean, bn3.running_var,
                                                           pool.gram(y2.shape[-1]), BN_MOMENTUM, BN_EPS, num_batches_tracked=bn3.num_batches_tracked)
                    else:
                        if self.training:
                            st3 = pool.take(blk.conv3.out_channels)
                            ops.conv1x1_stats(y2, w3, a2[0], a2[1], st3)
                        yl, al = None, self._bn_affine(None, blk.bn3, st3, count=y2.numel() // y2.shape[-1])
                else:
                    yl, al = self._conv_bn(y2, blk.conv3, blk.bn3, pool, a2, apply=ap3)
            else:
                recompute = False
                y1, a1 = self._conv_bn(a, blk.conv1, blk.bn1, pool, None, blk.stride, 1, 3)
                yl, al = self._conv_bn(y1, blk.conv2, blk.bn2, pool, a1, 1, 1, 3)
            if blk.downsample is not None:
                idt, idaff = self._conv_bn(a, blk.downsample[0], blk.downsample[1], pool, a_aff, blk.stride, 0, 1, apply="load")
                a_aff = None
            else:
                idt, idaff = a, None
            nxt = blocks[bi + 1] if bi + 1 < len(blocks) else None
            if recompute:
                pending = ("re", y2, a2, w3, al, idt, idaff)
            elif self.fuse_tail and nxt is not None and nxt.kind == "bottleneck":
                pending = (yl, al, idt, idaff)
            elif nxt is None and self.fuse_pool and yl.shape[-1] % 4 == 0:
                if pool is not None:
                    pool.done()
                return self.fc(ops.bn_act_avgpool(yl, al[0], al[1], idt, None if idaff is None else idaff[0], None if idaff is None else idaff[1]))
            elif idaff is not None:
                a = ops.bn_act(yl, al[0], al[1], idt, idaff[0], idaff[1], relu=True)
            else:
                a = ops.bn_act(yl, al[0], al[1], idt, relu=True)
        if pool is not None:
            pool.done()
        return self.fc(ops.avgpool(a))

    def _stats_pool(self, device):
        p = getattr(self, "_pool", None)
        if p is None or p.buf.device != device:
            p = self._pool = _StatsPool(device, persistent=True)
        p.begin()
        return p


class _StatsPool:
    def __init__(self, device, channels=32768, persistent=False):
        self.S = ops.stat_shards()
        self.buf = torch.zeros(2 * self.S * 2 * channels, device=device, dtype=ops.STAT_DTYPE)
        self.off = 0
        self.persistent, self.clean = persistent, True
        self._gram = {}

    def gram(self, Cb):
        if Cb not in self._gram:
            self._gram[Cb] = ops.gram_buffers(Cb, self.buf.device)
        return self._gram[Cb]

    def begin(self):
        if not self.clean:
            self.buf.zero_()
            for g, _ in self._gram.values():
                g.zero_()
        self.off, self.clean = 0, False

    def done(self):
        self.clean = True

    def take(self, C):
        n = 2 * self.S * 2 * C
        if self.off + n > self.buf.numel():
            if self.persistent:
                raise RuntimeError("_StatsPool: persistent arena exhausted")
            self.buf = torch.zeros_like(self.buf)
            self.off = 0
        v = self.buf[self.off:self.off + n].view(2, self.S, 2, C)
        self.off += n
        self.high = max(getattr(self, "high", 0), self.off)
        return v


def resnet18(pretrained=False, **kw):
    return ResNetTrunk("resnet18", **kw)


def resnet50(pretrained=False, **kw):
    return ResNetTrunk("resnet50", **kw)
```

mhentropy_amd/switches.py:

```python
import os

SWITCHES = {
    "MHE_CONV_TILE": ("-1", "csrc/conv.hip", "force convolution variant k where the geometry admits it (tuning runs)"),
    "MHE_CONV_STREAM": ("1", "csrc/conv.hip", "0: no streaming 1x1 / row-streaming 3x3 kernels (variants 8 / 9)"),
    "MHE_CONV_WIDE": ("1", "csrc/conv.hip", "0: no resident-slab kernel (variant 11)"),
    "MHE_CONV_TAIL": ("1", "csrc/conv.hip", "0: no residual-tail kernel with transfer waves (variant 10)"),
    "MHE_CONV_P8H": ("1", "csrc/conv.hip", "0: no 256x128 phase-pipelined tile (variant 13)"),
    "MHE_CONV_HALO": ("1", "resnet.py, train.py", "0: 3x3 stride-1 units of layer2 / layer3 on the im2col kernels instead of the resident-tile kernel"),
    "MHE_BN_APPLY": ("pass", "resnet.py", "pass | load: where a producer's BatchNorm + ReLU is applied by default"),
    "MHE_BN_APPLY_1X1": ("auto", "resnet.py", "pass | load | auto for the 1x1 consumers"),
    "MHE_BN_APPLY_3X3": ("auto", "resnet.py", "pass | load | auto for the 3x3 consumers"),
    "MHE_BN_LOAD_S2": ("256", "resnet.py", "BatchNorm on the load of the stride-2 3x3 launches up to this many channels"),
    "MHE_FUSE_TAIL": ("1", "resnet.py", "0: block tails as separate bn_act passes"),
    "MHE_FUSE_RECOMPUTE": ("1", "resnet.py", "0: conv3 of layer1 / layer2 written and read back (forward-only path)"),
    "MHE_RECOMPUTE_STATS": ("gram", "resnet.py", "stream: bn3 statistics from the statistics-only launch instead of the Gram matrix"),
    "MHE_STEM_POOL": ("1", "resnet.py", "0: stem convolution and max pool as two kernels"),
    "MHE_FUSE_POOL": ("1", "resnet.py", "0: last block tail and average pool as two launches"),
    "MHE_GRAM_WGS_64": ("512", "csrc/conv_gram.hip", "workgroups of the 64-channel Gram launch"),
    "MHE_GRAM_WGS_128": ("256", "csrc/conv_gram.hip", "workgroups of the 128-channel Gram launch"),
    "MHE_FLOW_FRAG": ("1", "flows.py, train.py", "0: second-generation coupling-stack kernel (flow_ns.hip) instead of the fragment-streaming one"),
    "MHE_FLOW_W1_SETS": ("2", "csrc/flow_fwd.hip", "3: a third register set of layer-1 weight fragments (measured equal)"),
    "MHE_GLOW_FUSED": ("1", "glow.py, train_glow.py", "0: the Glow branch's sampling pass layer by layer (~60 launches) instead of the one-launch kernel"),
    "MHE_GLOW_REV_FUSED": ("1", "train_glow.py", "0: the Glow branch's reverse pass over the tape stage by stage instead of the one-launch chain (csrc/glow_rev.hip)"),
    "MHE_MANO_FOUR": ("1", "csrc/mano.hip", "0: one hypothesis per wavefront"),
    "MHE_LBS_MFMA": ("1", "body.py", "0: the body model's skinning with one thread per vertex (csrc/body.hip) instead of the matrix-core kernel (csrc/lbs_skin.hip)"),
    "MHE_MANO_SKIN_MFMA": ("1", "csrc/mano.hip", "0: full-mesh skinning with one thread per vertex (round 1) instead of the matrix-core kernel on bf16 pieces (csrc/mano_skin.hip)"),
    "MHE_TRAIN_RECOMPUTE": ("1", "train.py", "0: conv3 of layer1 / layer2 written by the train step's forward pass"),
    "MHE_CONV3_FOLD": ("1", "train.py", "0: conv3 + bn3 reversed by reading y3 (no Gram fold)"),
    "MHE_CONV3_FOLD_CAT": ("1", "train.py", "0: the fold's second product as a launch of its own"),
    "MHE_SHORTCUT_FOLD": ("1", "train.py", "0: layer1's shortcut reversed by the apply pass"),
    "MHE_STEM_BWD_TWO_PASS": ("1", "train.py", "0: the stem's scattered pool gradient written and read back"),
    "MHE_STEM_POOL_FUSED": ("1", "train.py", "0: stem BatchNorm + ReLU not folded into its max pool"),
    "MHE_STEM_POOLED_SUMS": ("1", "train.py", "0: the stem's BatchNorm-reverse sums from a walk over its full-resolution output"),
    "MHE_STEM_WGRAD_PAIRS": ("1", "train.py", "0: the stem's weight gradient over single pixels (3 channels padded to 8)"),
    "MHE_GATE_BITS": ("1", "train.py", "0: ReLU gates read from the block-wide tensors instead of their bits"),
    "MHE_CONV_HALO_DG": ("1", "train.py", "0: 3x3 data gradients on the im2col kernels"),
    "MHE_HALO_BN_ON_LOAD": ("0", "train.py", "1: the unit's BatchNorm reverse on the resident-tile data-gradient launch's load (measured equal)"),
    "MHE_BN_REDUCE_FUSED": ("1", "train.py", "0: BatchNorm-reverse sums in a pass of their own"),
    "MHE_BN_BWD_ON_LOAD": ("1", "train.py", "0: BatchNorm-reverse apply always as a pass"),
    "MHE_BN_BWD_ON_LOAD_MAXC": ("128", "train.py", "widest bottleneck whose conv3 reverse takes the apply on its operand load"),
    "MHE_BN_BWD_ON_LOAD_WIDE": ("1", "train.py", "0: layer3 / layer4's conv3 reverse without the apply on its load"),
    "MHE_BN_BWD_APPLY_WIDE": ("1", "csrc/trunk_bwd.hip", "0: 8-byte lanes in the apply pass"),
    "MHE_COND_BWD_BF16": ("1", "train.py", "0: the conditioning projections' reverse products on f32 operands"),
    "MHE_FLOW_WGRAD_GROUPED": ("1", "train.py", "0: one weight-gradient launch per coupling net"),
    "MHE_FLOW_REV_FUSED": ("1", "train.py", "0: the flow's reverse chain coupling by coupling"),
    "MHE_FLOW_RECOMPUTE": ("0", "train.py", "1: the reverse pass re-evaluates the flow nets instead of reading emitted activations"),
    "MHE_LAZY_FALLBACK_TABLES": ("1", "train.py", "0: the fallback operand layouts refreshed every step"),
    "MHE_POISON_STALE_TABLES": ("0", "train.py", "1 (debug): fallback operand layouts a repack leaves behind are filled with NaN"),
    "MHE_GATHER_AFFINE": ("1", "train.py", "0: the bf16 operand re-pack from one index per element instead of (base, stride, validity) per eight"),
    "MHE_WGRAD_MULTI": ("1", "train.py", "0: one weight-gradient launch per trunk layer instead of one multi-problem launch per gradient bucket and tile shape"),
    "MHE_WGRAD_MULTI_WGS": ("2048", "csrc/wgrad.hip", "workgroups a multi-problem launch of the 4-wave tiles aims at"),
    "MHE_WGRAD_MULTI_WGS_BIG": ("768", "csrc/wgrad.hip", "workgroups a multi-problem launch of the 256 x 256 tile aims at"),
    "MHE_WGRAD_W16": ("1", "csrc/wgrad.hip", "0: the 256 x 256 weight-gradient tile on eight waves of 64 x 128 instead of sixteen of 64 x 64"),
    "MHE_WGRAD_DMA": ("1", "csrc/wgrad.hip", "0: register-staged bf16 weight-gradient kernel"),
    "MHE_WGRAD_BIG": ("1", "csrc/wgrad.hip", "0: no 256x256 weight-gradient tile"),
    "MHE_WGRAD_XCD": ("1", "csrc/wgrad.hip", "0: weight-gradient tiles in grid order"),
    "MHE_WGRAD_WGS": ("512", "csrc/wgrad.hip", "target workgroup count of a split launch"),
    "MHE_WGRAD_MINCHUNK": ("512", "csrc/wgrad.hip", "shortest pixel slice of the bf16 kernels"),
    "MHE_WGRAD_SLABS": ("all", "csrc/wgrad.hip", "big: small layers add their tiles with f32 atomics (order-dependent sums)"),
    "MHE_WGRAD_F32MFMA": ("", "csrc/wgrad.hip", "set: bf16 operands through the f32 MFMA kernel"),
    "MHE_GRAD_EXCHANGE": ("f32", "dist.py", "bf16: gradient buckets exchanged as bf16 (all-to-all + all-gather, f32 accumulation) instead of an f32 all-reduce"),
    "MHE_DIST_FORCE": ("0", "dist.py", "1: issue every collective in a group of ONE rank (one-GPU rehearsal of the RCCL path)"),
    "MHE_BENCH_REHEARSE": ("0", "bench.py", "1: all ranks share cuda:0 and talk over gloo (development only)"),
}


def non_default(environ=None):
    env = os.environ if environ is None else environ
    return {k: env[k] for k, (default, _, _) in SWITCHES.items() if k in env and env[k] != default}


def markdown_table():
    rows = ["| variable | default | read by | non-default value selects |", "|---|---|---|---|"]
    rows += [f"| `{k}` | `{d or '(unset)'}` | `{w}` | {m} |" for k, (d, w, m) in SWITCHES.items()]
    return "\n".join(rows)


if __name__ == "__main__":
    print(markdown_table())
```

Before: 2.517 million hypotheses/s.

## Write block output only at even pixels before stride-2 downsample stages

Before a stride-2 stage whose shortcut samples one pixel in four, the previous block's fused tail kernel now writes its activation output only at even (row, col) pixels into a quarter-size buffer. The downsample 1x1 then runs as a stride-1 conv on that compact tensor. This is meant to cut activation write bandwidth and the strided shortcut read. It adds new kernel template variants and geometry checks, and it relies on the stride-2 conv1 path never reading the full-resolution output, which the forward appears to satisfy.

New measurement: 2.534 million hypotheses/s, median of 6. About the same (+0.7%).

```diff
diff --git a/include/mhe.h b/include/mhe.h
--- a/include/mhe.h
+++ b/include/mhe.h
@@ -245,6 +245,15 @@
                                   const void *w3, const float *bn3_scale, const float *bn3_shift, const void *identity,
                                   const float *id_scale, const float *id_shift, const void *w1, void *a_out, void *a_bits, void *y1,
                                   mhe_stat_t *stats, void *stream);
+int mhe_bottleneck_tail_even_supported(const mhe_conv_desc *d, int Cb);
+int mhe_bottleneck_tail_even_nhwc(const mhe_conv_desc *d, int Cb, const void *y2, const float *bn2_scale, const float *bn2_shift,
+                                  const void *w3, const float *bn3_scale, const float *bn3_shift, const void *identity,
+                                  const float *id_scale, const float *id_shift, const void *w1, void *a_out, void *a_bits, void *y1,
+                                  mhe_stat_t *stats, int a_even, void *stream);
+int mhe_conv1x1_residual_in_even_supported(const mhe_conv_desc *d);
+int mhe_conv1x1_residual_in_even_nhwc(const mhe_conv_desc *d, const void *x, const void *x2, const void *w, void *y,
+                                      const float *in_scale, const float *in_shift, const float *x2_scale,
+                                      const float *x2_shift, void *a_out, mhe_stat_t *stats, int a_even, void *stream);
 int mhe_conv2d_masked_bias_nhwc(const mhe_conv_desc *d, const void *x, const void *xcat, int cin2, const void *w, void *y,
                                 const void *residual, const void *mask, const float *bias, const void *bn_y0,
                                 const float *bn_mean_invstd0, mhe_stat_t *bn_stats0, void *stream);
diff --git a/mhentropy_amd/_lib.py b/mhentropy_amd/_lib.py
--- a/mhentropy_amd/_lib.py
+++ b/mhentropy_amd/_lib.py
@@ -129,6 +129,10 @@
     "mhe_conv_wgrad_batched_nhwc": (_i, [_p, _i, _p, _l, _p, _l, _p, _l, _i, _p, _sz, _p]),
     "mhe_conv2d_masked_bits_nhwc": (_i, [_p] * 14),
     "mhe_bottleneck_tail_bits_nhwc": (_i, [_p, _i] + [_p] * 15),
+    "mhe_bottleneck_tail_even_supported": (_i, [_p, _i]),
+    "mhe_bottleneck_tail_even_nhwc": (_i, [_p, _i] + [_p] * 14 + [_i, _p]),
+    "mhe_conv1x1_residual_in_even_supported": (_i, [C.POINTER(ConvDesc)]),
+    "mhe_conv1x1_residual_in_even_nhwc": (_i, [C.POINTER(ConvDesc)] + [_p] * 10 + [_i, _p]),
     "mhe_conv2d_masked_bias_nhwc": (_i, [_p, _p, _p, _i] + [_p] * 9),
     "mhe_conv3x3_halo_supported": (_i, [_i] * 5),
     "mhe_conv3x3_halo_pack_bf16": (_i, [_p, _p, _i, _i, _p]),
diff --git a/mhentropy_amd/csrc/conv.hip b/mhentropy_amd/csrc/conv.hip
--- a/mhentropy_amd/csrc/conv.hip
+++ b/mhentropy_amd/csrc/conv.hip
@@ -562,7 +562,7 @@
                       const float *in_shift, const float *out_scale, const float *out_shift, const void *residual,
                       mhe_stat_t *stats, const void *x2, const float *x2_scale, const float *x2_shift, void *a_out, void *stream,
                       const void *mask = nullptr, const struct BnRev *bn = nullptr, float *y32 = nullptr, const int *scatter = nullptr,
-                      const void *xcat = nullptr, int cin2 = 0, const void *mask_bits = nullptr);
+                      const void *xcat = nullptr, int cin2 = 0, const void *mask_bits = nullptr, int a_even = 0);
 struct BnRev { const void *y[2]; const float *mi[2]; mhe_stat_t *stats[2]; };
 
 extern "C" int mhe_conv2d_nhwc(const mhe_conv_desc *d, const void *x, const void *w, void *y, const float *in_scale,
@@ -585,6 +585,30 @@
     MHE_REQUIRE(d->KH == 1 && d->KW == 1 && d->stride == 1 && d->pad == 0, "mhe_conv1x1_residual_in_nhwc: 1x1 stride-1 only");
     MHE_REQUIRE((x2_scale == nullptr) == (x2_shift == nullptr), "mhe_conv1x1_residual_in_nhwc: x2_scale/x2_shift must come together");
     return conv_entry(d, x, w, y, in_scale, in_shift, nullptr, nullptr, nullptr, stats, x2, x2_scale, x2_shift, a_out, stream);
+}
+
+static bool residual_in_even_geometry(const mhe_conv_desc *d) {
+    if (!d || d->dtype != MHE_BF16 || d->B <= 0 || d->H <= 0 || d->W <= 0 || d->H % 2 || d->W % 2) return false;
+    mhe_conv_desc q = *d;
+    q.tile = 0;
+    return mhe_conv_tile_mode(&q, 2) == 10;
+}
+
+extern "C" int mhe_conv1x1_residual_in_even_supported(const mhe_conv_desc *d) { return residual_in_even_geometry(d) ? 1 : 0; }
+
+extern "C" int mhe_conv1x1_residual_in_even_nhwc(const mhe_conv_desc *d, const void *x, const void *x2, const void *w, void *y,
+                                                 const float *in_scale, const float *in_shift, const float *x2_scale,
+                                                 const float *x2_shift, void *a_out, mhe_stat_t *stats, int a_even, void *stream) {
+    if (!a_even) return mhe_conv1x1_residual_in_nhwc(d, x, x2, w, y, in_scale, in_shift, x2_scale, x2_shift, a_out, stats, stream);
+    MHE_REQUIRE(d && x2 && in_scale && in_shift && a_out, "mhe_conv1x1_residual_in_even_nhwc: x2, in_scale, in_shift and a_out are required");
+    MHE_REQUIRE(d->KH == 1 && d->KW == 1 && d->stride == 1 && d->pad == 0, "mhe_conv1x1_residual_in_even_nhwc: 1x1 stride-1 only");
+    MHE_REQUIRE((x2_scale == nullptr) == (x2_shift == nullptr), "mhe_conv1x1_residual_in_even_nhwc: x2_scale/x2_shift must come together");
+    MHE_REQUIRE(residual_in_even_geometry(d), "mhe_conv1x1_residual_in_even_nhwc: needs bf16, even H and W and a geometry the transfer-wave tail kernel takes "
+                "(H=%d W=%d Cin=%d Cout=%d)", d->H, d->W, d->Cin, d->Cout);
+    mhe_conv_desc q = *d;
+    q.tile = 0;
+    return conv_entry(&q, x, w, y, in_scale, in_shift, nullptr, nullptr, nullptr, stats, x2, x2_scale, x2_shift, a_out, stream, nullptr, nullptr, nullptr,
+                      nullptr, nullptr, 0, nullptr, 1);
 }
 
 extern "C" int mhe_conv1x1_cat_bias_nhwc(const mhe_conv_desc *d, const void *x, const void *xcat, int cin2, const void *w, void *y, const void *residual,
@@ -667,7 +691,7 @@
 static int conv_entry(const mhe_conv_desc *d, const void *x, const void *w, void *y, const float *in_scale,
                       const float *in_shift, const float *out_scale, const float *out_shift, const void *residual,
                       mhe_stat_t *stats, const void *x2, const float *x2_scale, const float *x2_shift, void *a_out, void *stream,
-                      const void *mask, const BnRev *bn, float *y32, const int *scatter, const void *xcat, int cin2, const void *mask_bits) {
+                      const void *mask, const BnRev *bn, float *y32, const int *scatter, const void *xcat, int cin2, const void *mask_bits, int a_even) {
     MHE_REQUIRE(d && x && w && (y || y32), "mhe_conv2d_nhwc: null pointer");
     MHE_REQUIRE(d->dtype == MHE_F32 || d->dtype == MHE_BF16, "mhe_conv2d_nhwc: dtype=%d", d->dtype);
     const int ce = elem_chunk(d->dtype), bke = 8 * ce;
@@ -697,6 +721,7 @@
     MHE_REQUIRE(M < (1ll << 31), "mhe_conv2d_nhwc: too many output pixels");
     p.M = (int)M;
     p.xcat = xcat; p.Cin2 = cin2; p.mask_bits = (const unsigned char *)mask_bits;
+    p.a_even = a_even ? 1 : 0;
     const int ktot = d->KH * d->KW * d->Cin + cin2;
     p.Kpad = (ktot + bke - 1) / bke * bke;
     p.relu_in = d->relu_in; p.relu_out = d->relu_out;
@@ -708,6 +733,8 @@
         p.y32 = y32;
         if (p.force < 0 || p.force > 4) p.force = p.Cout <= 64 ? 0 : 1;
     }
+    MHE_REQUIRE(!p.a_even || (d->dtype == MHE_BF16 && conv::tail_supports(p) && conv::choose_tile(p, true, true) == 10),
+                "mhe_conv2d_nhwc: a_out at even pixels needs the transfer-wave tail kernel (variant 10)");
     if (d->dtype == MHE_F32) return conv::launch_conv<float>(p, (hipStream_t)stream);
     return conv::launch_conv<u16>(p, (hipStream_t)stream);
 }
@@ -733,10 +760,11 @@
     return conv::launch_stream(p, (hipStream_t)stream);
 }
 
-extern "C" int mhe_bottleneck_tail_supported(const mhe_conv_desc *d, int Cb) {
+static int bottleneck_tail_geometry(const mhe_conv_desc *d, int Cb, int a_even) {
     if (!d || d->dtype != MHE_BF16) return 0;
     static const float dummy = 0.f;
     conv::Params p{};
+    p.H = d->H; p.W = d->W; p.a_even = a_even ? 1 : 0;
     p.x = p.x2 = p.w = p.w3 = p.y = p.a_out = (void *)&dummy; p.in_scale = p.in_shift = p.mid_scale = p.mid_shift = &dummy;
     p.Cin = d->Cin; p.Cout = d->Cout; p.KH = d->KH; p.KW = d->KW; p.stride = d->stride; p.pad = d->pad; p.Kpad = d->Cin;
     const long long M = (long long)d->B * d->H * d->W;
@@ -745,6 +773,9 @@
     return conv::fuse_supports(p, Cb) ? 1 : 0;
 }
 
+extern "C" int mhe_bottleneck_tail_supported(const mhe_conv_desc *d, int Cb) { return bottleneck_tail_geometry(d, Cb, 0); }
+extern "C" int mhe_bottleneck_tail_even_supported(const mhe_conv_desc *d, int Cb) { return bottleneck_tail_geometry(d, Cb, 1); }
+
 extern "C" int mhe_bottleneck_tail_nhwc(const mhe_conv_desc *d, int Cb, const void *y2, const float *bn2_scale, const float *bn2_shift,
                                         const void *w3, const float *bn3_scale, const float *bn3_shift, const void *identity,
                                         const float *id_scale, const float *id_shift, const void *w1, void *a_out, void *y1, mhe_stat_t *stats,
@@ -756,18 +787,28 @@
                                              const void *w3, const float *bn3_scale, const float *bn3_shift, const void *identity,
                                              const float *id_scale, const float *id_shift, const void *w1, void *a_out, void *a_bits, void *y1,
                                              mhe_stat_t *stats, void *stream) {
+    return mhe_bottleneck_tail_even_nhwc(d, Cb, y2, bn2_scale, bn2_shift, w3, bn3_scale, bn3_shift, identity, id_scale, id_shift, w1, a_out, a_bits, y1, stats, 0,
+                                         stream);
+}
+
+extern "C" int mhe_bottleneck_tail_even_nhwc(const mhe_conv_desc *d, int Cb, const void *y2, const float *bn2_scale, const float *bn2_shift,
+                                             const void *w3, const float *bn3_scale, const float *bn3_shift, const void *identity,
+                                             const float *id_scale, const float *id_shift, const void *w1, void *a_out, void *a_bits, void *y1,
+                                             mhe_stat_t *stats, int a_even, void *stream) {
     MHE_REQUIRE(d && y2 && bn2_scale && bn2_shift && w3 && bn3_scale && bn3_shift && identity && w1 && a_out && y1, "mhe_bottleneck_tail_nhwc: null pointer");
     MHE_REQUIRE(d->dtype == MHE_BF16, "mhe_bottleneck_tail_nhwc: bf16 storage only");
     MHE_REQUIRE((id_scale == nullptr) == (id_shift == nullptr), "mhe_bottleneck_tail_nhwc: id_scale/id_shift must come together");
     conv::Params p{};
     p.x = y2; p.in_scale = bn2_scale; p.in_shift = bn2_shift; p.w3 = w3; p.mid_scale = bn3_scale; p.mid_shift = bn3_shift;
     p.x2 = identity; p.x2_scale = id_scale; p.x2_shift = id_shift; p.w = w1; p.a_out = a_out; p.y = y1; p.stats = stats;
-    p.a_bits = (unsigned char *)a_bits;
+    p.a_bits = (unsigned char *)a_bits; p.a_even = a_even ? 1 : 0;
     p.B = d->B; p.H = d->H; p.W = d->W; p.Cin = d->Cin; p.Cout = d->Cout; p.KH = d->KH; p.KW = d->KW; p.stride = d->stride; p.pad = d->pad;
     p.Ho = d->H; p.Wo = d->W; p.Kpad = d->Cin; p.relu_in = 1; p.force = -1;
     const long long M = (long long)d->B * d->H * d->W;
     MHE_REQUIRE(M > 0 && M < (1ll << 31), "mhe_bottleneck_tail_nhwc: bad pixel count");
     p.M = (int)M;
+    MHE_REQUIRE(!a_even || (Cb == 64 && d->Cout == 128 && d->H % 2 == 0 && d->W % 2 == 0),
+                "mhe_bottleneck_tail_even_nhwc: a_out at even pixels needs Cb 64, Cout 128 and even H and W (Cb=%d Cout=%d H=%d W=%d)", Cb, d->Cout, d->H, d->W);
     MHE_REQUIRE(conv::fuse_supports(p, Cb), "mhe_bottleneck_tail_nhwc: needs Cin = 4 Cb, Cb 64 / 128, Cout 64 / 128, pixels %% 128 == 0 (Cin=%d Cb=%d Cout=%d M=%lld)",
                 d->Cin, Cb, d->Cout, M);
     return conv::launch_fuse(p, Cb, (hipStream_t)stream);
diff --git a/mhentropy_amd/csrc/conv_fuse.hip b/mhentropy_amd/csrc/conv_fuse.hip
--- a/mhentropy_amd/csrc/conv_fuse.hip
+++ b/mhentropy_amd/csrc/conv_fuse.hip
@@ -22,8 +22,8 @@
 }
 }
 
-template <int CB, int N2>
-__global__ __launch_bounds__(512) void bottleneck_tail_kernel(const Params p) {
+template <int CB, int N2, bool QA>
+__device__ __forceinline__ void bottleneck_tail_body(const Params &p) {
     using T = u16;
     constexpr int C = 4 * CB, NT = C / 64, KT1 = CB / 64;
     constexpr int R3S = KT1 * 64 * 8, R1S = N2 * 8;
@@ -46,7 +46,7 @@
     __syncthreads();
     const __amdgpu_buffer_rsrc_t y2g = rsrc_of(p.x, (size_t)p.M * CB * 2), idg = rsrc_of(p.x2, (size_t)p.M * C * 2);
     const __amdgpu_buffer_rsrc_t w3g = rsrc_of(p.w3, (size_t)C * CB * 2), w1g = rsrc_of(p.w, (size_t)N2 * C * 2);
-    const __amdgpu_buffer_rsrc_t ag = rsrc_of(p.a_out, (size_t)p.M * C * 2), yg = rsrc_of(p.y, (size_t)p.M * N2 * 2);
+    const __amdgpu_buffer_rsrc_t ag = rsrc_of(p.a_out, (size_t)(QA ? p.M / 4 : p.M) * C * 2), yg = rsrc_of(p.y, (size_t)p.M * N2 * 2);
     const __amdgpu_buffer_rsrc_t abg = rsrc_of(p.a_bits, (size_t)p.M * (C / 8));
     const int cc = t2 % CPR2, r0 = t2 / CPR2;
     const unsigned toffC = (unsigned)(rbase * C + s8 * 8) * 2u, toffB = (unsigned)(rbase * CB + s8 * 8) * 2u, toffY = (unsigned)(r0 * N2 + cc * 8) * 2u;
@@ -192,6 +192,14 @@
 #pragma unroll
             for (int j = 0; j < N2 / 32; ++j) *reinterpret_cast<u32x4 *>(dst + swz(rbase + 32 * j, s8)) = w1r[j];
         };
+        unsigned qoff[4];
+        auto even_rows = [&](int m0) __attribute__((always_inline)) {
+#pragma unroll
+            for (int j = 0; j < 4; ++j) {
+                const int e = even_pixel(m0 + rbase + 32 * j, p.W);
+                qoff[j] = e < 0 ? ~0u : (unsigned)(e * C + s8 * 8) * 2u;
+            }
+        };
         auto xform = [&](int m0, int t, const IdSet &st) __attribute__((always_inline)) {
             const uint4 *Ts = Tbuf + (t & 1) * FT;
             uint4 *As = Abuf + (t & 1) * FT;
@@ -220,7 +228,8 @@
                 }
                 const uint4 o = Chunk<T>::pack(v);
                 As[swz(row, s8)] = o;
-                bst(ag, toffC, (unsigned)(m0 + 32 * j) * (C * 2) + t * 128, o);
+                if constexpr (QA) { if (qoff[j] != ~0u) bst(ag, qoff[j], t * 128, o); }
+                else bst(ag, toffC, (unsigned)(m0 + 32 * j) * (C * 2) + t * 128, o);
                 const unsigned wds[4] = {o.x, o.y, o.z, o.w};
                 unsigned gb = 0;
 #pragma unroll
@@ -262,6 +271,7 @@
             const int Ln = L + (int)gridDim.x;
             const bool more = Ln < ntiles;
             const int m0n = more ? Ln * FPIX : m0;
+            if constexpr (QA) even_rows(m0);
             stage_a2();
             store_w3(0);
             load_w3(1);
@@ -305,7 +315,13 @@
     }
 }
 
+template <int CB, int N2>
+__global__ __launch_bounds__(512) void bottleneck_tail_kernel(const Params p) { bottleneck_tail_body<CB, N2, false>(p); }
+template <int CB, int N2>
+__global__ __launch_bounds__(512) void bottleneck_tail_even_kernel(const Params p) { bottleneck_tail_body<CB, N2, true>(p); }
+
 bool fuse_supports(const Params &p, int cb) {
+    if (p.a_even && !(cb == 64 && p.Cout == 128 && p.H > 0 && p.W > 0 && p.H % 2 == 0 && p.W % 2 == 0 && p.M % (p.H * p.W) == 0)) return false;
     return p.x && p.x2 && p.w && p.w3 && p.y && p.a_out && p.in_scale && p.in_shift && p.mid_scale && p.mid_shift &&
            (cb == 64 || cb == 128) && p.Cin == 4 * cb && (p.Cout == 64 || p.Cout == 128) && p.Kpad == p.Cin &&
            p.KH == 1 && p.KW == 1 && p.stride == 1 && p.pad == 0 && p.M % FPIX == 0 && p.M > 0;
@@ -314,6 +330,7 @@
 int launch_fuse(const Params &p, int cb, hipStream_t s) {
     const int ntiles = p.M / FPIX;
     const dim3 grid((unsigned)(ntiles < 256 ? ntiles : 256)), block(512);
+    if (p.a_even) { hipLaunchKernelGGL((bottleneck_tail_even_kernel<64, 128>), grid, block, 0, s, p); return check_launch("bottleneck_tail_even_kernel"); }
     if (cb == 64 && p.Cout == 64) hipLaunchKernelGGL((bottleneck_tail_kernel<64, 64>), grid, block, 0, s, p);
     else if (cb == 64 && p.Cout == 128) hipLaunchKernelGGL((bottleneck_tail_kernel<64, 128>), grid, block, 0, s, p);
     else if (cb == 128 && p.Cout == 64) hipLaunchKernelGGL((bottleneck_tail_kernel<128, 64>), grid, block, 0, s, p);
diff --git a/mhentropy_amd/csrc/conv_shared.h b/mhentropy_amd/csrc/conv_shared.h
--- a/mhentropy_amd/csrc/conv_shared.h
+++ b/mhentropy_amd/csrc/conv_shared.h
@@ -22,7 +22,13 @@
     const void *xcat; int Cin2;
     unsigned char *a_bits; const unsigned char *mask_bits;
     const float *rev_coef;
+    int a_even;
 };
+
+__device__ __forceinline__ int even_pixel(int m, int W) {
+    const unsigned r = (unsigned)m / (unsigned)W, w = (unsigned)m - r * (unsigned)W;
+    return ((r | w) & 1u) ? -1 : (int)((r >> 1) * ((unsigned)W >> 1) + (w >> 1));
+}
 
 __device__ __forceinline__ long out_pixel(const Params &p, int m) {
     if (m >= p.M) return -1l;
diff --git a/mhentropy_amd/csrc/conv_tail.hip b/mhentropy_amd/csrc/conv_tail.hip
--- a/mhentropy_amd/csrc/conv_tail.hip
+++ b/mhentropy_amd/csrc/conv_tail.hip
@@ -9,8 +9,8 @@
 
 }
 
-template <bool DG>
-__global__ __launch_bounds__(512) void conv_tail_kernel(const Params p) {
+template <bool DG, bool QA>
+__device__ __forceinline__ void conv_tail_body(const Params &p) {
     using T = u16;
     __shared__ uint4 lds[2 * T_STAGE];
     __shared__ float aff[4 * TMAXK];
@@ -46,6 +46,7 @@
 #pragma unroll
         for (int j = 0; j < 8; ++j) st.w[j] = *reinterpret_cast<const uint4 *>(wg + (size_t)(n0 + rbase + 32 * j) * p.Kpad + kc);
     };
+    int qpix[4];
     auto store_tile = [&](int t, const Set &st, int m0, T *ag) __attribute__((always_inline)) {
         uint4 *At = lds + (t & 1) * T_STAGE, *Wt = At + T_A;
         const int kc = t * TBK + s * 8;
@@ -73,7 +74,8 @@
             }
             const uint4 o = Chunk<T>::pack(v);
             At[swz(rbase + 32 * j, s)] = o;
-            if (ag) *reinterpret_cast<uint4 *>(ag + (size_t)(m0 + rbase + 32 * j) * K + kc) = o;
+            if constexpr (QA) { if (ag && qpix[j] >= 0) *reinterpret_cast<uint4 *>(ag + (size_t)qpix[j] * K + kc) = o; }
+            else if (ag) *reinterpret_cast<uint4 *>(ag + (size_t)(m0 + rbase + 32 * j) * K + kc) = o;
         }
 #pragma unroll
         for (int j = 0; j < 8; ++j) Wt[swz(rbase + 32 * j, s)] = st.w[j];
@@ -231,6 +233,10 @@
             tile_at(L, mt, ntile);
             const int m0 = mt * TBM, n0 = ntile * TBN;
             T *ag = p.a_out && ntile == 0 ? reinterpret_cast<T *>(p.a_out) : nullptr;
+            if constexpr (QA) {
+#pragma unroll
+                for (int j = 0; j < 4; ++j) qpix[j] = even_pixel(m0 + rbase + 32 * j, p.W);
+            }
             __syncthreads();
             store_tile(0, st0, m0, ag);
             if (2 < nk) load_tile(2, st0, m0, n0);
@@ -266,8 +272,12 @@
     }
 }
 
+template <bool DG>
+__global__ __launch_bounds__(512) void conv_tail_kernel(const Params p) { conv_tail_body<DG, false>(p); }
+__global__ __launch_bounds__(512) void conv_tail_even_kernel(const Params p) { conv_tail_body<false, true>(p); }
 
 bool tail_supports(const Params &p) {
+    if (p.a_even && !(p.a_out && !p.mask && p.H > 0 && p.W > 0 && p.H % 2 == 0 && p.W % 2 == 0 && p.M % (p.H * p.W) == 0)) return false;
     if (p.mask ? (p.stats != nullptr) : (p.residual != nullptr)) return false;
     return p.x2 && p.in_scale && !p.out_scale && !p.out_shift && !p.relu_out && !p.y32 && !p.os2 && !p.res_s2 &&
            p.KH == 1 && p.KW == 1 && p.stride == 1 && p.pad == 0 && p.Kpad == p.Cin && p.Cin % TBK == 0 && p.Cin >= 2 * TBK && p.Cin <= TMAXK &&
@@ -277,6 +287,7 @@
 int launch_tail(const Params &p, hipStream_t s) {
     const int ntiles = (p.M / TBM) * (p.Cout / TBN);
     const dim3 grid((unsigned)(ntiles < 256 ? ntiles : 256));
+    if (p.a_even) { hipLaunchKernelGGL(conv_tail_even_kernel, grid, dim3(512), 0, s, p); return check_launch("conv_tail_even_kernel"); }
     if (p.mask) hipLaunchKernelGGL(conv_tail_kernel<true>, grid, dim3(512), 0, s, p);
     else hipLaunchKernelGGL(conv_tail_kernel<false>, grid, dim3(512), 0, s, p);
     return check_launch("conv_tail_kernel");
diff --git a/mhentropy_amd/ops.py b/mhentropy_amd/ops.py
--- a/mhentropy_amd/ops.py
+++ b/mhentropy_amd/ops.py
@@ -683,8 +683,15 @@
     return bool(_lib.lib().mhe_bottleneck_tail_supported(C.byref(d), int(Cb)))
 
 
-def bottleneck_tail(y2, bn2, w3, bn3, identity, id_aff, w1, stats=None, want_bits=False):
+def bottleneck_tail_even_supported(B, H, W, Cb, Cout):
+    d = ConvDesc(B, H, W, 4 * Cb, Cout, 1, 1, 1, 0, BF16, 1, 0, 0, 0)
+    return bool(_lib.lib().mhe_bottleneck_tail_even_supported(C.byref(d), int(Cb)))
+
+
+def bottleneck_tail(y2, bn2, w3, bn3, identity, id_aff, w1, stats=None, want_bits=False, a_even=False, a_out=None):
     B, H, W, Cb = y2.shape
+    if a_even and (H % 2 or W % 2):
+        raise _lib.MheError(f"tail: a_even needs even H and W, got {H} x {W}")
     Cw, Cout = w3.shape[0], w1.shape[0]
     _chk(y2, torch.bfloat16, "tail.y2"); _chk(w3, torch.bfloat16, "tail.w3", (Cw, Cb)); _chk(w1, torch.bfloat16, "tail.w1", (Cout, Cw))
     _chk(identity, torch.bfloat16, "tail.identity", (B, H, W, Cw))
@@ -692,20 +699,25 @@
         _chk(sc, torch.float32, f"tail.{n}_scale", (c,)); _chk(sh, torch.float32, f"tail.{n}_shift", (c,))
     if stats is not None:
         _chk_stats(stats, "tail.stats", Cout)
-    a = torch.empty(B, H, W, Cw, device=y2.device, dtype=torch.bfloat16)
+    a_shape = (B, H // 2, W // 2, Cw) if a_even else (B, H, W, Cw)
+    a = a_out if a_out is not None else torch.empty(a_shape, device=y2.device, dtype=torch.bfloat16)
+    _chk(a, torch.bfloat16, "tail.a_out", a_shape)
     y1 = torch.empty(B, H, W, Cout, device=y2.device, dtype=torch.bfloat16)
     bits = torch.empty(B, H, W, Cw // 8, device=y2.device, dtype=torch.uint8) if want_bits else None
     d = ConvDesc(B, H, W, Cw, Cout, 1, 1, 1, 0, BF16, 1, 0, 0, 0)
     if TIMING:
         ev0, ev1 = torch.cuda.Event(enable_timing=True), torch.cuda.Event(enable_timing=True)
         ev0.record()
-    check(_lib.lib().mhe_bottleneck_tail_bits_nhwc(C.byref(d), Cb, _ptr(y2), _ptr(bn2[0]), _ptr(bn2[1]), _ptr(w3), _ptr(bn3[0]), _ptr(bn3[1]), _ptr(identity),
-                                                   _ptr(id_aff[0] if id_aff is not None else None), _ptr(id_aff[1] if id_aff is not None else None),
-                                                   _ptr(w1), _ptr(a), _ptr(bits), _ptr(y1), _ptr(stats), _stream()), "mhe_bottleneck_tail_bits_nhwc")
+    args = (C.byref(d), Cb, _ptr(y2), _ptr(bn2[0]), _ptr(bn2[1]), _ptr(w3), _ptr(bn3[0]), _ptr(bn3[1]), _ptr(identity),
+            _ptr(id_aff[0] if id_aff is not None else None), _ptr(id_aff[1] if id_aff is not None else None), _ptr(w1), _ptr(a), _ptr(bits), _ptr(y1), _ptr(stats))
+    if a_even:
+        check(_lib.lib().mhe_bottleneck_tail_even_nhwc(*args, 1, _stream()), "mhe_bottleneck_tail_even_nhwc")
+    else:
+        check(_lib.lib().mhe_bottleneck_tail_bits_nhwc(*args, _stream()), "mhe_bottleneck_tail_bits_nhwc")
     if TIMING:
         ev1.record()
         nbytes = 2 * (y2.numel() + identity.numel() + a.numel() + y1.numel() + w3.numel() + w1.numel())
-        KERNEL_TIMES.append(("mhe::conv::bottleneck_tail_kernel<%d, %d>" % (Cb, Cout), 2.0 * B * H * W * Cw * (Cb + Cout), ev0, ev1, nbytes))
+        KERNEL_TIMES.append(("mhe::conv::bottleneck_tail%s_kernel<%d, %d>" % ("_even" if a_even else "", Cb, Cout), 2.0 * B * H * W * Cw * (Cb + Cout), ev0, ev1, nbytes))
     return (a, y1, bits) if want_bits else (a, y1)
 
 
@@ -745,8 +757,15 @@
     return dx
 
 
-def conv1x1_residual_in(x, x2, w, in_scale, in_shift, x2_scale=None, x2_shift=None, a_out=None, stats=None, tile=0):
+def conv1x1_residual_in_even_supported(B, H, W, Cin, Cout, dt):
+    d = ConvDesc(B, H, W, Cin, Cout, 1, 1, 1, 0, dtype_code(dt), 1, 0, 0, 0)
+    return bool(_lib.lib().mhe_conv1x1_residual_in_even_supported(C.byref(d)))
+
+
+def conv1x1_residual_in(x, x2, w, in_scale, in_shift, x2_scale=None, x2_shift=None, a_out=None, stats=None, tile=0, a_even=False):
     B, H, W, Cin = x.shape
+    if a_even and (a_out is None or tile or H % 2 or W % 2):
+        raise _lib.MheError("conv_res: a_even needs a_out, even H and W and the launcher's own kernel choice")
     Cout = w.shape[0]
     dt = x.dtype
     _chk(x, dt, "conv_res.x"); _chk(x2, dt, "conv_res.x2", x.shape); _chk(w, dt, "conv_res.w")
@@ -754,7 +773,7 @@
     if x2_scale is not None:
         _chk(x2_scale, torch.float32, "conv_res.x2_scale", (Cin,)); _chk(x2_shift, torch.float32, "conv_res.x2_shift", (Cin,))
     if a_out is not None:
-        _chk(a_out, dt, "conv_res.a_out", x.shape)
+        _chk(a_out, dt, "conv_res.a_out", (B, H // 2, W // 2, Cin) if a_even else x.shape)
     if stats is not None:
         _chk_stats(stats, "conv_res.stats", Cout)
     y = torch.empty(B, H, W, Cout, device=x.device, dtype=dt)
@@ -762,14 +781,16 @@
     if TIMING:
         ev0, ev1 = torch.cuda.Event(enable_timing=True), torch.cuda.Event(enable_timing=True)
         ev0.record()
-    check(_lib.lib().mhe_conv1x1_residual_in_nhwc(C.byref(d), _ptr(x), _ptr(x2), _ptr(w), _ptr(y), _ptr(in_scale), _ptr(in_shift),
-                                                  _ptr(x2_scale), _ptr(x2_shift), _ptr(a_out), _ptr(stats), _stream()),
-          "mhe_conv1x1_residual_in_nhwc")
+    args = (C.byref(d), _ptr(x), _ptr(x2), _ptr(w), _ptr(y), _ptr(in_scale), _ptr(in_shift), _ptr(x2_scale), _ptr(x2_shift), _ptr(a_out), _ptr(stats))
+    if a_even:
+        check(_lib.lib().mhe_conv1x1_residual_in_even_nhwc(*args, 1, _stream()), "mhe_conv1x1_residual_in_even_nhwc")
+    else:
+        check(_lib.lib().mhe_conv1x1_residual_in_nhwc(*args, _stream()), "mhe_conv1x1_residual_in_nhwc")
     if TIMING:
         ev1.record()
         es = x.element_size()
         nbytes = es * (2 * x.numel() + y.numel() + w.numel() + (a_out.numel() if a_out is not None else 0))
-        name = _conv_kernel_name(d, dt, 2)
+        name = "mhe::conv::conv_tail_even_kernel" if a_even else _conv_kernel_name(d, dt, 2)
         KERNEL_TIMES.append((name, 2.0 * B * H * W * Cout * Cin, ev0, ev1, nbytes))
     return y
 
diff --git a/mhentropy_amd/resnet.py b/mhentropy_amd/resnet.py
--- a/mhentropy_amd/resnet.py
+++ b/mhentropy_amd/resnet.py
@@ -76,6 +76,7 @@
         self.recompute_stats = os.environ.get("MHE_RECOMPUTE_STATS", "gram")
         self.stem_pool_fused = os.environ.get("MHE_STEM_POOL", "1") == "1"
         self.fuse_pool = os.environ.get("MHE_FUSE_POOL", "1") == "1"
+        self.strided_a = os.environ.get("MHE_STRIDED_A", "1") == "1"
 
     def _w(self, conv, cin_pad=None, stem=False):
         p = conv.weight
@@ -108,14 +109,14 @@
         sc = bn.weight.detach() / torch.sqrt(bn.running_var + BN_EPS)
         return sc.contiguous(), (bn.bias.detach() - bn.running_mean * sc).contiguous()
 
-    def _conv_bn(self, x, conv, bn, stats_pool, in_aff=None, stride=1, pad=0, k=1, cin_pad=None, apply=None):
+    def _conv_bn(self, x, conv, bn, stats_pool, in_aff=None, stride=1, pad=0, k=1, cin_pad=None, apply=None, tile=0):
         w = self._w(conv, cin_pad)
         if in_aff is not None and (apply or self.bn_apply) == "pass":
             x = ops.bn_act(x, in_aff[0], in_aff[1], relu=True, out=x)
             in_aff = None
         isc, ish = in_aff if in_aff is not None else (None, None)
         st = stats_pool.take(conv.out_channels) if self.training else None
-        y = ops.conv2d_nhwc(x, w, k, k, stride, pad, in_scale=isc, in_shift=ish, relu_in=in_aff is not None, stats=st)
+        y = ops.conv2d_nhwc(x, w, k, k, stride, pad, in_scale=isc, in_shift=ish, relu_in=in_aff is not None, stats=st, tile=tile)
         return y, self._bn_affine(y, bn, st)
 
     def forward(self, x):
@@ -136,20 +137,26 @@
             a = ops.maxpool3x3s2(y, aff[0], aff[1])
         pending = None
         for bi, blk in enumerate(blocks):
+            a_even = False
             if blk.kind == "bottleneck":
+                want_even = self.strided_a and pending is not None and blk.downsample is not None and blk.stride == 2
                 if pending is not None and isinstance(pending[0], str):
                     _, y2_p, a2_p, w3_p, al_p, idt_p, idaff_p = pending
                     st = pool.take(blk.conv1.out_channels) if self.training else None
-                    a, y1 = ops.bottleneck_tail(y2_p, a2_p, w3_p, al_p, idt_p, idaff_p, self._w(blk.conv1), stats=st)
+                    a_even = want_even and ops.bottleneck_tail_even_supported(y2_p.shape[0], y2_p.shape[1], y2_p.shape[2], y2_p.shape[3],
+                                                                              blk.conv1.out_channels)
+                    a, y1 = ops.bottleneck_tail(y2_p, a2_p, w3_p, al_p, idt_p, idaff_p, self._w(blk.conv1), stats=st, a_even=a_even)
                     a1 = self._bn_affine(y1, blk.bn1, st)
                     pending = None
                 elif pending is not None:
                     yl_p, al_p, idt_p, idaff_p = pending
-                    a = torch.empty_like(yl_p)
+                    Bp, Hp, Wp, Cp = yl_p.shape
+                    a_even = want_even and ops.conv1x1_residual_in_even_supported(Bp, Hp, Wp, Cp, blk.conv1.out_channels, yl_p.dtype)
+                    a = yl_p.new_empty(Bp, Hp // 2, Wp // 2, Cp) if a_even else torch.empty_like(yl_p)
                     st = pool.take(blk.conv1.out_channels) if self.training else None
                     y1 = ops.conv1x1_residual_in(yl_p, idt_p, self._w(blk.conv1), al_p[0], al_p[1],
                                                  None if idaff_p is None else idaff_p[0],
-                                                 None if idaff_p is None else idaff_p[1], a_out=a, stats=st)
+                                                 None if idaff_p is None else idaff_p[1], a_out=a, stats=st, a_even=a_even)
                     a1 = self._bn_affine(y1, blk.bn1, st)
                     pending = None
                 else:
@@ -191,7 +198,11 @@
                 recompute = False
                 y1, a1 = self._conv_bn(a, blk.conv1, blk.bn1, pool, None, blk.stride, 1, 3)
                 yl, al = self._conv_bn(y1, blk.conv2, blk.bn2, pool, a1, 1, 1, 3)
-            if blk.downsample is not None:
+            if blk.downsample is not None and a_even:
+                ds = blk.downsample[0]
+                v = ops.conv_tile_choice(a.shape[0], 2 * a.shape[1], 2 * a.shape[2], ds.in_channels, ds.out_channels, 1, 2, 0, a.dtype)
+                idt, idaff = self._conv_bn(a, ds, blk.downsample[1], pool, None, 1, 0, 1, tile=v + 1)
+            elif blk.downsample is not None:
                 idt, idaff = self._conv_bn(a, blk.downsample[0], blk.downsample[1], pool, a_aff, blk.stride, 0, 1, apply="load")
                 a_aff = None
             else:
diff --git a/mhentropy_amd/switches.py b/mhentropy_amd/switches.py
--- a/mhentropy_amd/switches.py
+++ b/mhentropy_amd/switches.py
@@ -16,6 +16,7 @@
     "MHE_RECOMPUTE_STATS": ("gram", "resnet.py", "stream: bn3 statistics from the statistics-only launch instead of the Gram matrix"),
     "MHE_STEM_POOL": ("1", "resnet.py", "0: stem convolution and max pool as two kernels"),
     "MHE_FUSE_POOL": ("1", "resnet.py", "0: last block tail and average pool as two launches"),
+    "MHE_STRIDED_A": ("1", "resnet.py", "0: the block output before a stride-2 stage written at full resolution (its shortcut reads one pixel in four)"),
     "MHE_GRAM_WGS_64": ("512", "csrc/conv_gram.hip", "workgroups of the 64-channel Gram launch"),
     "MHE_GRAM_WGS_128": ("256", "csrc/conv_gram.hip", "workgroups of the 128-channel Gram launch"),
     "MHE_FLOW_FRAG": ("1", "flows.py, train.py", "0: second-generation coupling-stack kernel (flow_ns.hip) instead of the fragment-streaming one"),
```
